# colmap/privacy_preserving_sfm

Measured on AMD Instinct MI355X. Metric: BA iterations/sec + RANSAC hypotheses/sec, 500 cams / 200k line obs, higher is better.
Workload: dtype f64; 1 GPU; configs[2]: 500 cams / 200k line obs full BA (K1+K2+K3, MFMA Schur solve) on 1xMI355X; cams=500, points=25000, obs=200000, camera_model=SIMPLE_RADIAL, reduced_system=3000, successful_steps=2561, lm_chunk=10, submodels=1, exchange=none (independent sub-models), linear_solver=cholesky (one launch: chain workgroup + task list), cholesky_fallbacks=0

## Files before the change

privacy_preserving_sfm_amd/csrc/ba_covariance.hip:

```cpp
#include <algorithm>
#include <cmath>
#include <cstring>
#include <vector>

#include "ba_impl.hpp"
#include "resource_pool.hpp"

namespace ppsfm {

typedef double cov_v4 __attribute__((ext_vector_type(4)));
constexpr int kTile = 64;

__device__ __forceinline__ cov_v4 CovMfma64(const double (&a)[16], const double (&b)[16], cov_v4 acc) {
  cov_v4 p1 = (cov_v4){0.0, 0.0, 0.0, 0.0}, p2 = p1, p3 = p1;
#pragma unroll
  for (int kk = 0; kk < 4; ++kk) {
    acc = __builtin_amdgcn_mfma_f64_16x16x4f64(a[kk], b[kk], acc, 0, 0, 0);
    p1 = __builtin_amdgcn_mfma_f64_16x16x4f64(a[4 + kk], b[4 + kk], p1, 0, 0, 0);
    p2 = __builtin_amdgcn_mfma_f64_16x16x4f64(a[8 + kk], b[8 + kk], p2, 0, 0, 0);
    p3 = __builtin_amdgcn_mfma_f64_16x16x4f64(a[12 + kk], b[12 + kk], p3, 0, 0, 0);
  }
  return (acc + p1) + (p2 + p3);
}
__device__ __forceinline__ void CovLoad16(const double* __restrict__ p, double (&v)[16]) {
  const double2* q = reinterpret_cast<const double2*>(p);
#pragma unroll
  for (int i = 0; i < 8; ++i) { const double2 t = q[i]; v[2 * i] = t.x; v[2 * i + 1] = t.y; }
}

__global__ __launch_bounds__(256) void k_tri_inverse(const double* __restrict__ L, int ld, int T, const double* __restrict__ Minv, const uint8_t* __restrict__ nz, double* Zt) {
  __shared__ double P[kTile * 17];
  const int j = (int)blockIdx.x >> 2, strip = (int)blockIdx.x & 3;
  const int tid = threadIdx.x, w = tid >> 6, l = tid & 63, lr = l & 15, g = l >> 4;
  double* zcol = Zt + ((size_t)j * kTile + 16 * strip) * ld;
  for (int idx = tid; idx < kTile * 16; idx += 256) {
    const int cc = idx >> 6, rr = idx & 63, gcol = 16 * strip + cc;
    zcol[(size_t)cc * ld + (size_t)j * kTile + rr] = rr >= gcol ? Minv[(size_t)j * kTile * kTile + rr * kTile + gcol] : 0.0;
  }
  __syncthreads();
  for (int k = j + 1; k < T; ++k) {
    cov_v4 acc = (cov_v4){0.0, 0.0, 0.0, 0.0};
    for (int m = j; m < k; ++m) {
      if (nz && !nz[(size_t)k * T + m]) continue;
      double av[16], bv[16];
      CovLoad16(L + ((size_t)k * kTile + 16 * w + lr) * ld + (size_t)m * kTile + 16 * g, av);
      CovLoad16(zcol + (size_t)lr * ld + (size_t)m * kTile + 16 * g, bv);
      acc = CovMfma64(av, bv, acc);
    }
#pragma unroll
    for (int i = 0; i < 4; ++i) P[(16 * w + g + 4 * i) * 17 + lr] = acc[i];
    __syncthreads();
    double av[16], bv[16];
    CovLoad16(Minv + (size_t)k * kTile * kTile + (size_t)(16 * w + lr) * kTile + 16 * g, av);
#pragma unroll
    for (int kk = 0; kk < 16; ++kk) {
      if (16 * g + kk > 16 * w + lr) av[kk] = 0.0;
      bv[kk] = P[(16 * g + kk) * 17 + lr];
    }
    const cov_v4 d = CovMfma64(av, bv, (cov_v4){0.0, 0.0, 0.0, 0.0});
#pragma unroll
    for (int i = 0; i < 4; ++i) zcol[(size_t)lr * ld + (size_t)k * kTile + 16 * w + g + 4 * i] = -d[i];
    __syncthreads();
  }
}

__global__ __launch_bounds__(256) void k_cov_pose_blocks(const int32_t* __restrict__ pairs, const int32_t* __restrict__ spos, const double* __restrict__ scale_c,
                                                         const double* __restrict__ Zt, int N, int n, double* __restrict__ out) {
  __shared__ double red[4][36];
  const int pr = blockIdx.x, tid = threadIdx.x;
  const int pi = pairs[2 * pr], pj = pairs[2 * pr + 1];
  const int ci = spos[6 * pi], cj = spos[6 * pj];
  const double* zi = Zt + (size_t)ci * N;
  const double* zj = Zt + (size_t)cj * N;
  double acc[36];
#pragma unroll
  for (int i = 0; i < 36; ++i) acc[i] = 0.0;
  for (int k = max(ci, cj) + tid; k < n; k += 256) {
    double a[6], b[6];
#pragma unroll
    for (int x = 0; x < 6; ++x) { a[x] = zi[(size_t)x * N + k]; b[x] = zj[(size_t)x * N + k]; }
#pragma unroll
    for (int x = 0; x < 6; ++x)
#pragma unroll
      for (int y = 0; y < 6; ++y) acc[6 * x + y] += a[x] * b[y];
  }
#pragma unroll
  for (int i = 0; i < 36; ++i) acc[i] = WaveSum(acc[i]);
  if ((tid & 63) == 0) {
#pragma unroll
    for (int i = 0; i < 36; ++i) red[tid >> 6][i] = acc[i];
  }
  __syncthreads();
  if (tid < 36) {
    const double v = ((red[0][tid] + red[1][tid]) + red[2][tid]) + red[3][tid];
    out[36 * (size_t)pr + tid] = scale_c[6 * pi + tid / 6] * scale_c[6 * pj + tid % 6] * v;
  }
}

struct CovPointArgs {
  int C, n, N;
  const int32_t *pt_start, *pt_obs, *obs_pose, *obs_cam, *spos, *intr_off, *intr_nv;
  const uint8_t* point_const;
  const double *rec, *JkS , *Vinv, *scale_p, *Zt;
};
constexpr int kCovChunk = 64;

__global__ __launch_bounds__(256) void k_cov_points(CovPointArgs a, const int32_t* __restrict__ ids, double* __restrict__ out) {
  __shared__ int s_kmin, s_col[kCovChunk], s_nv[kCovChunk], s_colI[kCovChunk][kCamStride];
  __shared__ double s_B[kCovChunk][18], s_BI[kCovChunk][3 * kCamStride], red[4][6];
  const int tid = threadIdx.x;
  const int p = ids[blockIdx.x];
  if (a.point_const[p]) {
    if (tid < 9) out[9 * (size_t)blockIdx.x + tid] = 0.0;
    return;
  }
  const int begin = a.pt_start[p], end = a.pt_start[p + 1];
  if (tid == 0) s_kmin = a.n;
  __syncthreads();
  for (int e = begin + tid; e < end; e += 256) {
    const int o = a.pt_obs[e];
    int kmin = a.spos[6 * a.obs_pose[o]];
    if (a.JkS) {
      const int cam = a.obs_cam[o] >> 4, off = a.intr_off[cam];
      if (off >= 0) for (int c = 0; c < a.intr_nv[cam]; ++c) kmin = min(kmin, a.spos[6 * a.C + off + c]);
    }
    atomicMin(&s_kmin, kmin);
  }
  __syncthreads();
  const int kmin = s_kmin;
  const int nchunks = (end - begin + kCovChunk - 1) / kCovChunk;
  double acc[6] = {0.0, 0.0, 0.0, 0.0, 0.0, 0.0};
  for (int k0 = kmin; k0 < a.n; k0 += 256) {
    const int k = k0 + tid;
    const bool live = k < a.n;
    double y0 = 0.0, y1 = 0.0, y2 = 0.0;
    for (int ch = 0; ch < nchunks; ++ch) {
      const int cnt = min(kCovChunk, end - begin - kCovChunk * ch);
      if (nchunks > 1 || k0 == kmin) {
        __syncthreads();
        if (tid < cnt) {
          const int o = a.pt_obs[begin + kCovChunk * ch + tid];
          const double* t = RecT(a.rec, (size_t)o);
          const double* jp = RecJ(a.rec, (size_t)o);
          s_col[tid] = a.spos[6 * a.obs_pose[o]];
#pragma unroll
          for (int x = 0; x < 6; ++x)
#pragma unroll
            for (int c = 0; c < 3; ++c) s_B[tid][3 * x + c] = jp[x] * t[c] + jp[6 + x] * t[3 + c];
          int nv = 0;
          if (a.JkS) {
            const int cam = a.obs_cam[o] >> 4, off = a.intr_off[cam];
            if (off >= 0) {
              nv = a.intr_nv[cam];
              const double* jk = a.JkS + (size_t)2 * kCamStride * o;
              for (int x = 0; x < nv; ++x) {
                s_colI[tid][x] = a.spos[6 * a.C + off + x];
#pragma unroll
                for (int c = 0; c < 3; ++c) s_BI[tid][3 * x + c] = jk[x] * t[c] + jk[kCamStride + x] * t[3 + c];
              }
            }
          }
          s_nv[tid] = nv;
        }
        __syncthreads();
      }
      if (live) {
        for (int q = 0; q < cnt; ++q) {
          const double* z = a.Zt + (size_t)s_col[q] * a.N + k;
#pragma unroll
          for (int x = 0; x < 6; ++x) {
            const double zz = z[(size_t)x * a.N];
            y0 += zz * s_B[q][3 * x]; y1 += zz * s_B[q][3 * x + 1]; y2 += zz * s_B[q][3 * x + 2];
          }
          const int nv = s_nv[q];
          for (int x = 0; x < nv; ++x) {
            const double zz = a.Zt[(size_t)s_colI[q][x] * a.N + k];
            y0 += zz * s_BI[q][3 * x]; y1 += zz * s_BI[q][3 * x + 1]; y2 += zz * s_BI[q][3 * x + 2];
          }
        }
      }
    }
    acc[0] += y0 * y0; acc[1] += y0 * y1; acc[2] += y0 * y2; acc[3] += y1 * y1; acc[4] += y1 * y2; acc[5] += y2 * y2;
  }
#pragma unroll
  for (int i = 0; i < 6; ++i) acc[i] = WaveSum(acc[i]);
  if ((tid & 63) == 0) {
#pragma unroll
    for (int i = 0; i < 6; ++i) red[tid >> 6][i] = acc[i];
  }
  __syncthreads();
  if (tid < 9) {
    const int r = tid / 3, c = tid % 3;
    const int lo = min(r, c), hi = max(r, c);
    const int sym = lo == 0 ? hi : (lo == 1 ? 2 + hi : 5);
    const double yy = ((red[0][sym] + red[1][sym]) + red[2][sym]) + red[3][sym];
    out[9 * (size_t)blockIdx.x + tid] = a.scale_p[3 * p + r] * a.scale_p[3 * p + c] * a.Vinv[6 * (size_t)p + sym] + yy;
  }
}

namespace {
struct CovBuffers {
  hipStream_t stream = nullptr;
  std::vector<void*> blocks;
  CholeskyState* chol = nullptr;
  template <typename T> int Alloc(T** p, size_t count) { const int rc = HandleAlloc(p, count); if (rc == PP_OK && *p) blocks.push_back(*p); return rc; }
  ~CovBuffers() {
    if (stream) (void)hipStreamSynchronize(stream);
    if (chol) CholeskyDestroy(chol);
    for (void* b : blocks) PoolDeviceFree(b);
  }
};
struct BufferSwap {
  pp_ba_impl* h;
  double *S, *scale_c, *scale_p, *diag_c, *diag_p, *Vinv, *vb;
  int32_t* d_flag;
  explicit BufferSwap(pp_ba_impl* hh) : h(hh), S(hh->S), scale_c(hh->scale_c), scale_p(hh->scale_p), diag_c(hh->diag_c), diag_p(hh->diag_p), Vinv(hh->Vinv), vb(hh->vb), d_flag(hh->d_flag) {}
  ~BufferSwap() { h->S = S; h->scale_c = scale_c; h->scale_p = scale_p; h->diag_c = diag_c; h->diag_p = diag_p; h->Vinv = Vinv; h->vb = vb; h->d_flag = d_flag; }
};
}

}

using namespace ppsfm;

extern "C" int pp_ba_covariance(pp_ba_handle h, const pp_ba_options* o, int32_t num_pose_pairs, const int32_t* pose_i, const int32_t* pose_j, double* pose_cov,
                                int32_t num_points, const int32_t* point_ids, double* point_cov, pp_ba_covariance_info* info) try {
  PP_REQUIRE(h && o, "pp_ba_covariance: null handle or options");
  PP_REQUIRE(num_pose_pairs >= 0 && num_points >= 0, "pp_ba_covariance: negative count");
  PP_REQUIRE(num_pose_pairs == 0 || (pose_i && pose_j && pose_cov), "pp_ba_covariance: %d pose pairs without their arrays", (int)num_pose_pairs);
  PP_REQUIRE(num_points == 0 || (point_ids && point_cov), "pp_ba_covariance: %d points without their arrays", (int)num_points);
  for (int32_t q = 0; q < num_pose_pairs; ++q)
    PP_REQUIRE(pose_i[q] >= 0 && pose_i[q] < h->C && pose_j[q] >= 0 && pose_j[q] < h->C, "pp_ba_covariance: pose pair %d = (%d, %d) is out of range (%d images)", (int)q,
               (int)pose_i[q], (int)pose_j[q], (int)h->C);
  for (int32_t q = 0; q < num_points; ++q)
    PP_REQUIRE(point_ids[q] >= 0 && point_ids[q] < h->P, "pp_ba_covariance: point %d = %d is out of range (%d points)", (int)q, (int)point_ids[q], (int)h->P);
  PP_REQUIRE(!h->iterative, "pp_ba_covariance: an iterative (ITERATIVE_SCHUR) handle never forms the reduced camera system the covariance is taken from - create "
             "the handle with pp_ba_problem_desc::linear_solver = PP_LINEAR_SOLVER_DIRECT (or PPSFM_BA_LINEAR_SOLVER=direct)");
  PP_REQUIRE(!BaInGroup(h), "pp_ba_covariance: the handle is attached to a group (pp_ba_set_allreduce / pp_ba_set_communicator) and holds one shard of the points - "
             "detach it, or take the covariance from a handle that holds the whole problem");
  if (info) std::memset(info, 0, sizeof(*info));
  PP_HIP_TRY(hipSetDevice(h->device));
  int rc;
  if ((rc = BaEnsureJacobianBuffers(h, 0, h->NI > 0 ? 1 : 0))) return rc;
  if ((rc = BaEnsureSolverBuffers(h))) return rc;
  hipStream_t s = h->stream;
  const int N = h->N, n = h->n_red, T = N / kTile;
  const size_t NN = (size_t)N * N;

  CovBuffers buf;
  buf.stream = s;
  double *S2 = nullptr, *Linv2 = nullptr, *Lfac2 = nullptr, *x2 = nullptr, *scale_c2 = nullptr, *scale_p2 = nullptr, *diag_c2 = nullptr, *diag_p2 = nullptr, *Vinv2 = nullptr,
         *vb2 = nullptr, *Zt = nullptr, *d_pose = nullptr, *d_point = nullptr;
  int32_t *flag2 = nullptr, *d_pairs = nullptr, *d_ids = nullptr;
  Switches sw = h->sw;
  sw.chol_small = false;
  {
    std::lock_guard<std::recursive_mutex> setup_lock(DeviceSetupMutex());
    if ((rc = buf.Alloc(&S2, NN)) || (rc = buf.Alloc(&Linv2, CholeskyWorkspaceDoubles(N))) || (rc = buf.Alloc(&x2, (size_t)N)) || (rc = buf.Alloc(&flag2, 4)) ||
        (rc = buf.Alloc(&scale_c2, (size_t)n)) || (rc = buf.Alloc(&scale_p2, 3 * (size_t)h->P)) || (rc = buf.Alloc(&diag_c2, (size_t)n)) ||
        (rc = buf.Alloc(&diag_p2, 3 * (size_t)h->P)) || (rc = buf.Alloc(&Vinv2, 6 * (size_t)h->P)) || (rc = buf.Alloc(&vb2, 3 * (size_t)h->P)) || (rc = buf.Alloc(&Zt, NN)) ||
        (rc = buf.Alloc(&d_pose, 36 * (size_t)num_pose_pairs)) || (rc = buf.Alloc(&d_point, 9 * (size_t)num_points)) || (rc = buf.Alloc(&d_pairs, 2 * (size_t)num_pose_pairs)) ||
        (rc = buf.Alloc(&d_ids, (size_t)num_points)))
      return rc;
    buf.chol = CholeskyCreate(sw);
    CholeskyDisableGraph(buf.chol);
    if (CholeskyNeedsFactorArray(buf.chol, N) && !CholeskyColumnsOnly(h->chol) && (rc = buf.Alloc(&Lfac2, NN))) return rc;
    PP_HIP_TRY(hipMemsetAsync(S2, 0, sizeof(double) * NN, s));
    if (Lfac2) PP_HIP_TRY(hipMemsetAsync(Lfac2, 0, sizeof(double) * NN, s));
    PP_HIP_TRY(hipMemsetAsync(Zt, 0, sizeof(double) * NN, s));
    PP_HIP_TRY(hipMemsetAsync(flag2, 0, 4 * sizeof(int32_t), s));
    const CholeskySystem sys{S2, N, n, Linv2, Lfac2, x2, flag2, s};
    const bool sparse = h->sparse_tiles && !h->tile_nz.empty();
    if ((rc = CholeskyBind(buf.chol, sys, sparse ? h->tile_nz.data() : nullptr))) return rc;
    if (CholeskyColumnsOnly(h->chol)) (void)CholeskyFallBackToColumns(buf.chol);
  }
  if (num_pose_pairs > 0) {
    std::vector<int32_t> pairs(2 * (size_t)num_pose_pairs);
    const bool perm = !h->pose_new_of_old.empty();
    for (int32_t q = 0; q < num_pose_pairs; ++q) {
      pairs[2 * (size_t)q] = perm ? h->pose_new_of_old[pose_i[q]] : pose_i[q];
      pairs[2 * (size_t)q + 1] = perm ? h->pose_new_of_old[pose_j[q]] : pose_j[q];
    }
    PP_HIP_TRY(hipMemcpyAsync(d_pairs, pairs.data(), sizeof(int32_t) * pairs.size(), hipMemcpyHostToDevice, s));
    PP_HIP_TRY(hipStreamSynchronize(s));
  }
  if (num_points > 0) PP_HIP_TRY(hipMemcpyAsync(d_ids, point_ids, sizeof(int32_t) * (size_t)num_points, hipMemcpyHostToDevice, s));
  PP_HIP_TRY(hipEventRecord(h->ev0, s));

  int32_t flag = 0;
  {
    BufferSwap swap(h);
    h->S = S2; h->scale_c = scale_c2; h->scale_p = scale_p2; h->diag_c = diag_c2; h->diag_p = diag_p2; h->Vinv = Vinv2; h->vb = vb2; h->d_flag = flag2;
    for (int attempt = 0; attempt < 2; ++attempt) {
      if ((rc = BaAssembleUndamped(h, o, attempt == 0))) return rc;
      if ((rc = CholeskySolve(buf.chol))) return rc;
      PP_HIP_TRY(hipMemcpyAsync(&flag, flag2, sizeof(int32_t), hipMemcpyDeviceToHost, s));
      PP_HIP_TRY(hipStreamSynchronize(s));
      if (!(flag & 4) || (flag & 3) || attempt == 1 || !CholeskyFallBackToColumns(buf.chol)) break;
      PP_HIP_TRY(hipMemsetAsync(flag2, 0, sizeof(int32_t), s));
      PP_HIP_TRY(hipMemsetAsync(S2, 0, sizeof(double) * NN, s));
    }
  }
  if (flag & 7) {
    SetLastError("pp_ba_covariance: the undamped reduced camera system is not positive definite (%s) - a free gauge, or a point seen along one direction only, has no covariance",
                 (flag & 2) ? "a point block is singular" : (flag & 1) ? "non-positive pivot" : "the factorisation did not finish");
    return PP_ERR_NUMERIC;
  }
  const double* Minv = nullptr;
  const uint8_t* nz = nullptr;
  const double* L = CholeskyFactor(buf.chol, &Minv, &nz);
  if (!L) { SetLastError("pp_ba_covariance: the factorisation left no factor in memory"); return PP_ERR_INTERNAL; }
  hipLaunchKernelGGL(k_tri_inverse, dim3(4 * T), dim3(256), 0, s, L, N, T, Minv, nz, Zt);
  if (num_pose_pairs > 0)
    hipLaunchKernelGGL(k_cov_pose_blocks, dim3(num_pose_pairs), dim3(256), 0, s, (const int32_t*)d_pairs, (const int32_t*)h->spos, (const double*)scale_c2, (const double*)Zt, N, n, d_pose);
  if (num_points > 0) {
    CovPointArgs a;
    a.C = h->C; a.n = n; a.N = N;
    a.pt_start = h->pt_start; a.pt_obs = h->pt_obs; a.obs_pose = h->obs_pose; a.obs_cam = h->obs_cam; a.spos = h->spos; a.intr_off = h->intr_off; a.intr_nv = h->intr_nv;
    a.point_const = h->point_const; a.rec = h->JpS; a.JkS = h->NI > 0 ? h->JkS_intr : nullptr; a.Vinv = Vinv2; a.scale_p = scale_p2; a.Zt = Zt;
    hipLaunchKernelGGL(k_cov_points, dim3(num_points), dim3(256), 0, s, a, (const int32_t*)d_ids, d_point);
  }
  PP_HIP_TRY(hipGetLastError());
  PP_HIP_TRY(hipEventRecord(h->ev1, s));
  if (num_pose_pairs > 0) PP_HIP_TRY(hipMemcpyAsync(pose_cov, d_pose, sizeof(double) * 36 * (size_t)num_pose_pairs, hipMemcpyDeviceToHost, s));
  if (num_points > 0) PP_HIP_TRY(hipMemcpyAsync(point_cov, d_point, sizeof(double) * 9 * (size_t)num_points, hipMemcpyDeviceToHost, s));
  PP_HIP_TRY(hipStreamSynchronize(s));
  if (info) {
    float ms = 0;
    PP_HIP_TRY(hipEventElapsedTime(&ms, h->ev0, h->ev1));
    info->n = n; info->path = CholeskyLinsolve(buf.chol); info->device_ms = ms;
  }
  return PP_OK;
} PP_API_CATCH("pp_ba_covariance")
```

privacy_preserving_sfm_amd/csrc/ba_eval.hip:

```cpp
#include <algorithm>
#include <chrono>
#include <cstdlib>
#include <cmath>
#include <cstring>
#include <numeric>
#include <thread>

#include "ba_impl.hpp"
#include "resource_pool.hpp"
#include "line_residual.hpp"

namespace ppsfm {

struct EvalArgs {
  int64_t M;
  const double *la, *lb, *lc;
  const int32_t *obs_pose, *obs_point, *obs_cam;
  const double *poses, *points, *intr;
  double *r, *Jpose, *Jpoint, *Jcam;
  const int32_t* cam_col;
  int cam_stride;
  double* partials;
  int loss_type;
  double loss_scale;
};

__device__ __forceinline__ void BlockPartialSum(double v, double* partials) {
  __shared__ double wsum[4];
  v = WaveSum(v);
  const int wave = threadIdx.x >> 6;
  if ((threadIdx.x & 63) == 0) wsum[wave] = v;
  __syncthreads();
  if (threadIdx.x == 0) partials[blockIdx.x] = (wsum[0] + wsum[1]) + (wsum[2] + wsum[3]);
}

template <int MODE, bool WANT_CAM, bool LOSS_CORRECT>
__global__ __launch_bounds__(256) void k_line_eval(EvalArgs a) {
  constexpr int JW = MODE == 2 ? 14 : 12;
  __shared__ __attribute__((aligned(16))) double sJp[MODE == 0 ? 2 : 256 * JW];
  __shared__ __attribute__((aligned(16))) double sJx[MODE == 0 ? 2 : 256 * 6];
  const int tid = threadIdx.x;
  const int64_t o0 = (int64_t)blockIdx.x * 256;
  const int64_t o = o0 + tid;
  double half_rho = 0.0;
  if (o < a.M) {
    const int c = a.obs_pose[o], p = a.obs_point[o], ck = a.obs_cam[o];
    const double la = a.la[o], lb = a.lb[o], lc = a.lc[o];
    const int model = ck & 15;
    const double* cam = a.intr + (size_t)kCamStride * (ck >> 4);
    const double* pose = a.poses + (size_t)7 * c;
    const double q[4] = {pose[0], pose[1], pose[2], pose[3]};
    const double t[3] = {pose[4], pose[5], pose[6]};
    const double X[3] = {a.points[3 * (size_t)p], a.points[3 * (size_t)p + 1], a.points[3 * (size_t)p + 2]};
    if (MODE == 0) {
      double r[2];
      LineResidualOnly(model, cam, q, t, X, la, lb, lc, r);
      double rho0, rho1;
      LossRho(a.loss_type, a.loss_scale, r[0] * r[0] + r[1] * r[1], &rho0, &rho1);
      half_rho = 0.5 * rho0;
      if (a.r) { a.r[2 * o] = r[0]; a.r[2 * o + 1] = r[1]; }
    } else {
      LineObsJac J;
      LineResidualJacobian<MODE == 2>(model, cam, q, t, X, la, lb, lc, &J);
      double rho0, rho1;
      LossRho(a.loss_type, a.loss_scale, J.r[0] * J.r[0] + J.r[1] * J.r[1], &rho0, &rho1);
      half_rho = 0.5 * rho0;
      const double sr = LOSS_CORRECT ? sqrt(rho1) : 1.0;
      double2* r2 = reinterpret_cast<double2*>(a.r);
      r2[o] = make_double2(sr * J.r[0], sr * J.r[1]);
      double2* jp = reinterpret_cast<double2*>(sJp + JW * tid);
      if (MODE == 1) {
        jp[0] = make_double2(sr * J.Jrot[0], sr * J.Jrot[1]);
        jp[1] = make_double2(sr * J.Jrot[2], sr * J.Jt[0]);
        jp[2] = make_double2(sr * J.Jt[1], sr * J.Jt[2]);
        jp[3] = make_double2(sr * J.Jrot[3], sr * J.Jrot[4]);
        jp[4] = make_double2(sr * J.Jrot[5], sr * J.Jt[3]);
        jp[5] = make_double2(sr * J.Jt[4], sr * J.Jt[5]);
      } else {
        jp[0] = make_double2(sr * J.Jq[0], sr * J.Jq[1]);
        jp[1] = make_double2(sr * J.Jq[2], sr * J.Jq[3]);
        jp[2] = make_double2(sr * J.Jt[0], sr * J.Jt[1]);
        jp[3] = make_double2(sr * J.Jt[2], sr * J.Jq[4]);
        jp[4] = make_double2(sr * J.Jq[5], sr * J.Jq[6]);
        jp[5] = make_double2(sr * J.Jq[7], sr * J.Jt[3]);
        jp[6] = make_double2(sr * J.Jt[4], sr * J.Jt[5]);
      }
      double2* jx = reinterpret_cast<double2*>(sJx + 6 * tid);
      jx[0] = make_double2(sr * J.JX[0], sr * J.JX[1]);
      jx[1] = make_double2(sr * J.JX[2], sr * J.JX[3]);
      jx[2] = make_double2(sr * J.JX[4], sr * J.JX[5]);
      if (WANT_CAM) {
        double jl[2 * kCamStride];
#pragma unroll
        for (int i = 0; i < 2 * kCamStride; ++i) jl[i] = 0.0;
        LineResidualCameraJacobian(model, cam, q, t, X, la, lb, lc, jl, kCamStride);
        if (LOSS_CORRECT) {
#pragma unroll
          for (int i = 0; i < 2 * kCamStride; ++i) jl[i] *= sr;
        }
        if (a.cam_col) {
          const int W = a.cam_stride;
          double* jc = a.Jcam + (size_t)2 * W * o;
          double2* z = reinterpret_cast<double2*>(jc);
          for (int i = 0; i < W; ++i) z[i] = make_double2(0.0, 0.0);
          const int32_t* col = a.cam_col + (size_t)kCamStride * (ck >> 4);
#pragma unroll
          for (int i = 0; i < kCamStride; ++i) { const int cc = col[i]; if (cc >= 0) { jc[cc] = jl[i]; jc[W + cc] = jl[kCamStride + i]; } }
        } else {
          double2* jc = reinterpret_cast<double2*>(a.Jcam + (size_t)2 * kCamStride * o);
#pragma unroll
          for (int i = 0; i < kCamStride; ++i) jc[i] = make_double2(jl[2 * i], jl[2 * i + 1]);
        }
      }
    }
  }
  if (MODE != 0) {
    __syncthreads();
    const int64_t left = a.M - o0;
    const int nobs = left < 256 ? (int)left : 256;
    {
      const int n2 = nobs * JW / 2;
      double2* dst = reinterpret_cast<double2*>(a.Jpose + (size_t)JW * o0);
      const double2* src = reinterpret_cast<const double2*>(sJp);
#pragma unroll
      for (int it = 0; it < (256 * JW / 2 + 255) / 256; ++it) {
        const int idx = it * 256 + tid;
        if (idx < n2) { const double2 v = src[idx]; __builtin_nontemporal_store(v.x, &dst[idx].x); __builtin_nontemporal_store(v.y, &dst[idx].y); }
      }
    }
    {
      const int n2 = nobs * 3;
      double2* dst = reinterpret_cast<double2*>(a.Jpoint + (size_t)6 * o0);
      const double2* src = reinterpret_cast<const double2*>(sJx);
#pragma unroll
      for (int it = 0; it < 3; ++it) {
        const int idx = it * 256 + tid;
        if (idx < n2) { const double2 v = src[idx]; __builtin_nontemporal_store(v.x, &dst[idx].x); __builtin_nontemporal_store(v.y, &dst[idx].y); }
      }
    }
  }
  BlockPartialSum(half_rho, a.partials);
}

__global__ __launch_bounds__(256) void k_sum_partials(const double* partials, int n, double* out) {
  __shared__ double sh[256];
  double acc = 0.0;
  for (int i = threadIdx.x; i < n; i += 256) acc += partials[i];
  sh[threadIdx.x] = acc;
  __syncthreads();
  for (int s = 128; s > 0; s >>= 1) {
    if ((int)threadIdx.x < s) sh[threadIdx.x] += sh[threadIdx.x + s];
    __syncthreads();
  }
  if (threadIdx.x == 0) *out = sh[0];
}

static EvalArgs MakeArgs(pp_ba_impl* h, const double* poses, const double* points, const double* intr = nullptr) {
  EvalArgs a;
  a.M = h->M; a.la = h->la; a.lb = h->lb; a.lc = h->lc;
  a.obs_pose = h->obs_pose; a.obs_point = h->obs_point; a.obs_cam = h->obs_cam;
  a.poses = poses; a.points = points; a.intr = intr ? intr : h->intr;
  a.r = h->r; a.Jpose = h->Jpose; a.Jpoint = h->Jpoint; a.Jcam = h->Jcam; a.cam_col = nullptr; a.cam_stride = kCamStride;
  a.partials = h->partials; a.loss_type = h->loss_type; a.loss_scale = h->loss_scale;
  return a;
}

int BaEnsureJacobianBuffers(pp_ba_impl* h, int jac_mode, int want_cam) {
  const int width = jac_mode == 1 ? 14 : 12;
  if (!h->Jpose || h->jpose_width < width) {
    if (h->Jpose) PoolDeviceFree(h->Jpose);
    h->Jpose = nullptr;
    int rc = HandleAlloc(&h->Jpose, (size_t)h->M * width);
    if (rc) return rc;
    h->jpose_width = width;
  }
  if (want_cam && !h->Jcam) {
    int rc = HandleAlloc(&h->Jcam, (size_t)h->M * 2 * kCamStride);
    if (rc) return rc;
  }
  return PP_OK;
}

int LaunchEval(pp_ba_impl* h, int jac_mode, int want_cam, bool loss_correct, const double* poses, const double* points,
               double* cost_slot, bool compact_cam) {
  EvalArgs a = MakeArgs(h, poses, points);
  if (want_cam) {
    h->jcam_compact = compact_cam && h->NI > 0;
    if (h->jcam_compact) { a.cam_col = h->intr_col; a.cam_stride = h->jcam_stride; }
  }
  const int grid = h->num_partials;
  hipStream_t s = h->stream;
  if (jac_mode == 0) {
    if (want_cam) { if (loss_correct) hipLaunchKernelGGL((k_line_eval<1, true, true>), dim3(grid), dim3(256), 0, s, a); else hipLaunchKernelGGL((k_line_eval<1, true, false>), dim3(grid), dim3(256), 0, s, a); }
    else { if (loss_correct) hipLaunchKernelGGL((k_line_eval<1, false, true>), dim3(grid), dim3(256), 0, s, a); else hipLaunchKernelGGL((k_line_eval<1, false, false>), dim3(grid), dim3(256), 0, s, a); }
  } else {
    if (want_cam) hipLaunchKernelGGL((k_line_eval<2, true, false>), dim3(grid), dim3(256), 0, s, a);
    else hipLaunchKernelGGL((k_line_eval<2, false, false>), dim3(grid), dim3(256), 0, s, a);
  }
  if (cost_slot) hipLaunchKernelGGL(k_sum_partials, dim3(1), dim3(256), 0, s, h->partials, grid, cost_slot);
  PP_HIP_TRY(hipGetLastError());
  return PP_OK;
}

int LaunchCostOnly(pp_ba_impl* h, const double* poses, const double* points, const double* intr, double* cost_slot) {
  EvalArgs a = MakeArgs(h, poses, points, intr);
  a.r = nullptr;
  const int grid = h->num_partials;
  hipLaunchKernelGGL((k_line_eval<0, false, false>), dim3(grid), dim3(256), 0, h->stream, a);
  if (cost_slot) hipLaunchKernelGGL(k_sum_partials, dim3(1), dim3(256), 0, h->stream, h->partials, grid, cost_slot);
  PP_HIP_TRY(hipGetLastError());
  return PP_OK;
}

static int LaunchResidualsOnly(pp_ba_impl* h, const double* poses, const double* points, double* cost_slot) {
  EvalArgs a = MakeArgs(h, poses, points);
  const int grid = h->num_partials;
  hipLaunchKernelGGL((k_line_eval<0, false, false>), dim3(grid), dim3(256), 0, h->stream, a);
  if (cost_slot) hipLaunchKernelGGL(k_sum_partials, dim3(1), dim3(256), 0, h->stream, h->partials, grid, cost_slot);
  PP_HIP_TRY(hipGetLastError());
  return PP_OK;
}

}

using namespace ppsfm;

extern "C" {

int pp_ba_destroy(pp_ba_handle h) try {
  if (!h) return PP_OK;
  (void)hipSetDevice(h->device);
  void* bufs[] = {h->la, h->lb, h->lc, h->obs_cam, h->obs_pose, h->obs_point, h->pose_camera, h->camera_model, h->pose_const,
                  h->tvec_mask, h->point_const, h->pt_start, h->pt_obs, h->pose_start, h->pose_obs, h->pair_start,
                  h->pair_ij, h->pair_entries, h->poses, h->points, h->intr, h->poses_c, h->points_c, h->r, h->Jpose,
                  h->Jpoint, h->Jcam, h->partials, h->U, h->gc, h->V, h->gp, h->Vinv, h->vb, h->scale_c, h->scale_p,
                  h->diag_c, h->diag_p, h->S, h->Linv, h->Lfac, h->step_c, h->step_p, h->scal, h->JpS, h->Q, h->norm_part,
                  h->intr_c, h->cam_np, h->intr_off, h->intr_nv, h->intr_col, h->cam_start, h->cam_obs, h->gen_pair, h->gen_pair_chunk, h->gen_chunk,
                  h->gen_multi, h->gen_grp_start, h->gen_grp_obs, h->gen_L, h->kk_entries, h->kk_pair, h->kk_pair_chunk, h->kk_chunk, h->kk_multi, h->kk_partial, h->gen_entries, h->isum_chunk, h->isum_cam_chunk, h->gen_partial, h->isum_partial, h->cnI, h->JkS_intr, h->Spack, h->nz_tile_list,
                  h->small_chunk, h->small_pair_chunk, h->small_partials, h->spos, h->step_s, h->attach_slot};
  if (h->stream) (void)hipStreamSynchronize(h->stream);
  for (void* b : bufs) if (b) PoolDeviceFree(b);
  CholeskyDestroy(h->chol);
  PcgFreeBuffers(h);
  for (int i = 0; i < 8; ++i) if (h->tev[i]) PoolEventRelease(h->tev[i], true);
  for (int i = 0; i < 2; ++i) if (h->tev_eval[i]) PoolEventRelease(h->tev_eval[i], true);
  if (h->h_scal) PoolPinnedFree(h->h_scal);
  { void* pins[] = {h->pin_r, h->pin_jpose, h->pin_jpoint, h->pin_jcam}; for (void* b : pins) if (b) (void)hipHostFree(b); }
  if (h->ev_readback) PoolEventRelease(h->ev_readback, false);
  if (h->ev0) PoolEventRelease(h->ev0, true);
  if (h->ev1) PoolEventRelease(h->ev1, true);
  if (h->stream) PoolStreamRelease(h->stream);
  delete h;
  return PP_OK;
} PP_API_CATCH("pp_ba_destroy")

int pp_ba_create(const pp_ba_problem_desc* d, int device, pp_ba_handle* out) try {
  PP_REQUIRE(d && out, "pp_ba_create: null argument");
  *out = nullptr;
  PP_REQUIRE(d->num_poses > 0 && d->num_points > 0 && d->num_cameras > 0 && d->num_obs > 0,
             "pp_ba_create: empty problem (poses %d, points %d, cameras %d, obs %lld)", d->num_poses, d->num_points,
             d->num_cameras, (long long)d->num_obs);
  PP_REQUIRE(d->lines && d->obs_pose && d->obs_point && d->pose_camera && d->camera_model, "pp_ba_create: null array");
  PP_REQUIRE(d->loss_type >= 0 && d->loss_type <= 2 && d->loss_scale >= 0, "pp_ba_create: bad loss");
  PP_REQUIRE(d->num_obs < (int64_t)1 << 31, "pp_ba_create: more than 2^31 observations");
  PP_REQUIRE(d->ordering >= PP_ORDERING_DEFAULT && d->ordering <= PP_ORDERING_AUTO, "pp_ba_create: unknown ordering %d", d->ordering);
  const int C = d->num_poses, P = d->num_points, K = d->num_cameras;
  const int64_t M = d->num_obs;
  PP_REQUIRE(K < (1 << 26), "pp_ba_create: too many intrinsics blocks");
  for (int k = 0; k < K; ++k) PP_REQUIRE(CameraNumParams(d->camera_model[k]) > 0, "pp_ba_create: unknown camera model %d", d->camera_model[k]);
  for (int c = 0; c < C; ++c) PP_REQUIRE(d->pose_camera[c] >= 0 && d->pose_camera[c] < K, "pp_ba_create: pose_camera[%d] out of range", c);
  for (int64_t o = 0; o < M; ++o) {
    PP_REQUIRE(d->obs_pose[o] >= 0 && d->obs_pose[o] < C && d->obs_point[o] >= 0 && d->obs_point[o] < P,
               "pp_ba_create: observation %lld indexes out of range", (long long)o);
    const double nrm = std::sqrt(d->lines[3 * o] * d->lines[3 * o] + d->lines[3 * o + 1] * d->lines[3 * o + 1]);
    PP_REQUIRE(std::fabs(nrm - 1.0) <= 1e-6, "pp_ba_create: line %lld is not normalised (|(a,b)| = %.9g)", (long long)o, nrm);
  }
  std::vector<int32_t> intr_off(K, -1), intr_nv(K, 0), intr_col((size_t)K * kCamStride, -1);
  int nv_widest = 0;
  int NI = 0;
  if (d->camera_const_mask) {
    std::vector<char> cam_used(K, 0);
    for (int c = 0; c < C; ++c) cam_used[d->pose_camera[c]] = 1;
    for (int k = 0; k < K; ++k) {
      if (!cam_used[k]) continue;
      const int np = CameraNumParams(d->camera_model[k]);
      int nv = 0;
      for (int j = 0; j < np; ++j) if (!((d->camera_const_mask[k] >> j) & 1)) intr_col[(size_t)k * kCamStride + j] = nv++;
      if (nv > 0) { intr_off[k] = NI; intr_nv[k] = nv; NI += nv; } nv_widest = std::max(nv_widest, nv);
    }
  }
  int ndev = 0;
  PP_HIP_TRY(hipGetDeviceCount(&ndev));
  PP_REQUIRE(device >= 0 && device < ndev, "pp_ba_create: device %d of %d", device, ndev);
  PP_HIP_TRY(hipSetDevice(device));

  const auto t_create0 = std::chrono::steady_clock::now();
  const ppsfm::Switches sw = ppsfm::ReadSwitches();
  const bool create_dbg = sw.create_debug;
  auto lap = [&, last = t_create0](const char* what) mutable {
    if (!create_dbg) return;
    const auto now = std::chrono::steady_clock::now();
    fprintf(stderr, "ppsfm: create %-34s %.3f ms\n", what, std::chrono::duration<double, std::milli>(now - last).count());
    last = now;
  };
  pp_ba_impl* h = new pp_ba_impl();
  OnUnwind unwind{[&] { pp_ba_destroy(h); }};
  h->sw = sw;
  h->chol = CholeskyCreate(sw);
  h->structure_from_covisibility = d->covisibility != nullptr;
  h->device = device; h->C = C; h->P = P; h->K = K; h->M = M;
  h->loss_type = d->loss_type; h->loss_scale = d->loss_scale;
  h->NI = NI; h->n_red = 6 * C + NI; h->intrinsics_variable = NI > 0;
  h->jcam_stride = std::max(2, (nv_widest + 1) & ~1);
  h->iterative = ppsfm::WillIterate(d, sw.ba_linear_solver);
  const bool iterative = h->iterative;
  int rc = PP_OK;
#define TRY(x) do { rc = (x); if (rc) { pp_ba_destroy(h); return rc; } } while (0)
#define TRYH(x) do { hipError_t e_ = (x); if (e_ != hipSuccess) { SetLastError("%s: %s", #x, hipGetErrorString(e_)); pp_ba_destroy(h); return PP_ERR_HIP; } } while (0)
  TRY(PoolStreamAcquire(&h->stream));
  TRY(PoolEventAcquire(&h->ev0, true));
  TRY(PoolEventAcquire(&h->ev1, true));
  hipStream_t s = h->stream;
  lap("handle, stream, events");

  std::vector<uint8_t> point_const(P, 0);
  if (d->point_const) std::memcpy(point_const.data(), d->point_const, P);
  std::vector<int32_t> pt_start(P + 1, 0), pt_obs(M);
  for (int64_t o = 0; o < M; ++o) pt_start[d->obs_point[o] + 1]++;
  for (int p = 0; p < P; ++p) pt_start[p + 1] += pt_start[p];
  {
    std::vector<int32_t> fp(pt_start.begin(), pt_start.end() - 1);
    for (int64_t o = 0; o < M; ++o) pt_obs[fp[d->obs_point[o]]++] = (int32_t)o;
  }
  lap("CSR by point");
  bool lists_on_device = !iterative && PairListsOnDeviceEligible(C, M, sw.ba_pair_lists);
  std::vector<uint64_t> graph_bits;
  double graph_ms = 0;
  if (lists_on_device) {
// ... 309 lines not shown
          size_t b = a;
          while (b < ko.size() && ko[b].first == ko[a].first) ++b;
          grps.push_back({ko[a].first, p, (int32_t)flat.size(), (int32_t)(flat.size() + (b - a))});
          for (size_t t = a; t < b; ++t) flat.push_back(ko[t].second);
          a = b;
        }
      }
      std::stable_sort(grps.begin(), grps.end(), [](const Grp& a, const Grp& b) { return a.k < b.k; });
      const size_t G = grps.size();
      dl.entries.assign(G + 1 + flat.size(), 0);
      { size_t pos = 0; for (size_t g = 0; g < G; ++g) { dl.entries[g] = (int32_t)pos; for (int32_t e = grps[g].e0; e < grps[g].e1; ++e) dl.entries[G + 1 + pos++] = flat[e]; } dl.entries[G] = (int32_t)pos; }
      dl.num_groups = (int64_t)G;
      dl.pair_chunk.push_back(0);
      size_t g = 0;
      for (int k = 0; k < K; ++k) {
        if (intr_off[k] < 0) continue;
        const int pair_id = (int)(dl.pair.size() / 4);
        dl.pair.push_back(6 * C + intr_off[k]); dl.pair.push_back(intr_nv[k]); dl.pair.push_back(6 * C + intr_off[k]); dl.pair.push_back(intr_nv[k] | (1 << 8));
        while (g < G && grps[g].k < k) ++g;
        size_t g0 = g; int64_t nobs = 0;
        for (; g < G && grps[g].k == k; ++g) {
          nobs += grps[g].e1 - grps[g].e0;
          if (nobs >= 320) { dl.chunk.push_back(pair_id); dl.chunk.push_back((int32_t)g0); dl.chunk.push_back((int32_t)(g + 1)); g0 = g + 1; nobs = 0; }
        }
        if (g0 < g) { dl.chunk.push_back(pair_id); dl.chunk.push_back((int32_t)g0); dl.chunk.push_back((int32_t)g); }
        dl.pair_chunk.push_back((int32_t)(dl.chunk.size() / 3));
      }
    };
    auto finish_diag = [&](DiagLists& dl) {
      const int64_t np = (int64_t)(dl.pair.size() / 4);
      for (int64_t pr = 0; pr < np; ++pr) if (dl.pair_chunk[pr + 1] - dl.pair_chunk[pr] != 1) dl.multi.push_back((int32_t)pr);
    };
    if (iterative) {
      DiagLists dl;
      build_diag(dl);
      gen_entries = dl.entries; gen_pair = dl.pair; gen_pair_chunk = dl.pair_chunk; gen_chunk = dl.chunk; h->gen_num_groups = dl.num_groups;
    } else if (h->intr_wide_nv > 0) {
      gen_pair_chunk.push_back(0);
    } else {
    struct GEntry { int64_t key; int32_t oi, oj; };
    std::vector<GEntry> ge;
    std::vector<int32_t> grp_start(1, 0), grp_obs;
    std::vector<int32_t> grp_cam;
    {
      std::vector<std::pair<int32_t, int32_t>> ko;
      for (int p = 0; p < P; ++p) {
        ko.clear();
        for (int e = pt_start[p]; e < pt_start[p + 1]; ++e) {
          const int32_t o = pt_obs[e]; const int k = in_pose_camera[in_obs_pose[o]];
          if (intr_off[k] >= 0) ko.push_back({k, o});
        }
        std::stable_sort(ko.begin(), ko.end(), [](const auto& a, const auto& b) { return a.first < b.first; });
        const size_t first_group = grp_cam.size();
        for (size_t a = 0; a < ko.size();) {
          size_t b = a;
          while (b < ko.size() && ko[b].first == ko[a].first) ++b;
          grp_cam.push_back(ko[a].first);
          for (size_t t = a; t < b; ++t) grp_obs.push_back(ko[t].second);
          grp_start.push_back((int32_t)grp_obs.size());
          a = b;
        }
        for (size_t g = first_group; g < grp_cam.size(); ++g) {
          const int ka = grp_cam[g];
          for (int f = pt_start[p]; f < pt_start[p + 1]; ++f) {
            const int32_t oj = pt_obs[f]; const int cj = in_obs_pose[oj]; const int kb = in_pose_camera[cj];
            const bool same = kb == ka;
            if (point_const[p] && !same) continue;
            const int32_t code = oj | (same ? (int32_t)0x80000000 : 0);
            if (!pose_const[cj]) ge.push_back({((int64_t)ka * 2 + 0) * (int64_t)(C + K) + cj, (int32_t)g, code});
            if (intr_off[kb] >= 0 && kb < ka) ge.push_back({((int64_t)ka * 2 + 1) * (int64_t)(C + K) + kb, (int32_t)g, code});
          }
        }
      }
    }
    h->gen_num_groups = (int64_t)grp_cam.size();
    gen_grp_start = grp_start; gen_grp_obs = grp_obs;
    build_diag(kk); finish_diag(kk);
    std::sort(ge.begin(), ge.end(), [](const GEntry& a, const GEntry& b) {
      if (a.key != b.key) return a.key < b.key;
      if (a.oi != b.oi) return a.oi < b.oi;
      return (a.oj & 0x7fffffff) < (b.oj & 0x7fffffff);
    });
    {
      std::vector<char> has_obs(K, 0);
      for (int64_t o = 0; o < M; ++o) has_obs[in_pose_camera[in_obs_pose[o]]] = 1;
      (void)has_obs;
      std::sort(ge.begin(), ge.end(), [](const GEntry& a, const GEntry& b) {
        if (a.key != b.key) return a.key < b.key;
        if (a.oi != b.oi) return a.oi < b.oi;
        return a.oj < b.oj;
      });
    }
    gen_entries.resize(2 * ge.size());
    gen_pair_chunk.push_back(0);
    size_t e = 0;
    while (e < ge.size()) {
      size_t f = e;
      while (f < ge.size() && ge[f].key == ge[e].key) ++f;
      const int64_t key = ge[e].key;
      const int col = (int)(key % (C + K)), kind = (int)((key / (C + K)) & 1), ka = (int)(key / (C + K) / 2);
      const int pair_id = (int)(gen_pair.size() / 4);
      gen_pair.push_back(6 * C + intr_off[ka]); gen_pair.push_back(intr_nv[ka]);
      if (kind == 0) { gen_pair.push_back(6 * col); gen_pair.push_back(6); }
      else { gen_pair.push_back(6 * C + intr_off[col]); gen_pair.push_back(intr_nv[col] | (1 << 8)); }
      if (ge[e].oi >= 0)
        for (size_t c0 = e; c0 < f; c0 += kGenChunk) { gen_chunk.push_back(pair_id); gen_chunk.push_back((int32_t)c0); gen_chunk.push_back((int32_t)std::min(c0 + kGenChunk, f)); }
      gen_pair_chunk.push_back((int32_t)(gen_chunk.size() / 3));
      for (size_t g = e; g < f; ++g) { gen_entries[2 * g] = ge[g].oi; gen_entries[2 * g + 1] = ge[g].oj; }
      e = f;
    }
    }
    h->gen_num_pairs = (int64_t)(gen_pair.size() / 4); h->gen_num_chunks = (int64_t)(gen_chunk.size() / 3);
    for (int64_t pr = 0; pr < h->gen_num_pairs; ++pr) if (gen_pair_chunk[pr + 1] - gen_pair_chunk[pr] != 1) gen_multi.push_back((int32_t)pr);
    h->gen_num_multi = (int64_t)gen_multi.size();
    h->isum_num_chunks = (int64_t)(isum_chunk.size() / 3);
  }

  lap("chunks, intrinsics lists");
  const auto t_create3 = std::chrono::steady_clock::now();
  TRY(HandleAlloc(&h->la, M)); TRY(HandleAlloc(&h->lb, M)); TRY(HandleAlloc(&h->lc, M));
  if (!arrays_on_device) { TRY(HandleAlloc(&h->obs_pose, M)); TRY(HandleAlloc(&h->obs_point, M)); }
  TRY(HandleAlloc(&h->obs_cam, M));
  TRY(HandleAlloc(&h->pose_camera, C)); TRY(HandleAlloc(&h->camera_model, K));
  if (!arrays_on_device) { TRY(HandleAlloc(&h->pose_const, C)); TRY(HandleAlloc(&h->point_const, P)); TRY(HandleAlloc(&h->pt_start, P + 1)); TRY(HandleAlloc(&h->pt_obs, M)); }
  TRY(HandleAlloc(&h->tvec_mask, C));
  TRY(HandleAlloc(&h->pose_start, C + 1)); TRY(HandleAlloc(&h->pose_obs, M));
  TRY(HandleAlloc(&h->pair_start, pair_start.size())); TRY(HandleAlloc(&h->pair_ij, std::max<size_t>(pair_ij.size(), 2)));
  if (!h->pair_entries) TRY(HandleAlloc(&h->pair_entries, std::max<size_t>(pair_entries.size(), 2)));
  TRY(HandleAlloc(&h->poses, (size_t)7 * C)); TRY(HandleAlloc(&h->points, (size_t)3 * P)); TRY(HandleAlloc(&h->intr, (size_t)kCamStride * K));
  TRY(HandleAlloc(&h->poses_c, (size_t)7 * C)); TRY(HandleAlloc(&h->points_c, (size_t)3 * P)); TRY(HandleAlloc(&h->intr_c, (size_t)kCamStride * K));
  TRY(HandleAlloc(&h->cam_np, K));
  TRY(HandleAlloc(&h->intr_off, K)); TRY(HandleAlloc(&h->intr_nv, K)); TRY(HandleAlloc(&h->intr_col, (size_t)K * kCamStride));
  if (NI > 0) {
    TRY(HandleAlloc(&h->cam_start, K + 1)); TRY(HandleAlloc(&h->cam_obs, M));
    TRY(HandleAlloc(&h->gen_pair, std::max<size_t>(gen_pair.size(), 4))); TRY(HandleAlloc(&h->gen_pair_chunk, gen_pair_chunk.size()));
    TRY(HandleAlloc(&h->gen_chunk, gen_chunk.size())); TRY(HandleAlloc(&h->gen_entries, std::max<size_t>(gen_entries.size(), 2)));
    TRY(HandleAlloc(&h->gen_multi, std::max<size_t>(gen_multi.size(), 1)));
    if (!iterative) {
      h->kk_num_groups = kk.num_groups; h->kk_num_pairs = (int64_t)(kk.pair.size() / 4); h->kk_num_chunks = (int64_t)(kk.chunk.size() / 3); h->kk_num_multi = (int64_t)kk.multi.size();
      TRY(HandleAlloc(&h->kk_entries, std::max<size_t>(kk.entries.size(), 1))); TRY(HandleAlloc(&h->kk_pair, std::max<size_t>(kk.pair.size(), 1)));
      TRY(HandleAlloc(&h->kk_pair_chunk, std::max<size_t>(kk.pair_chunk.size(), 1))); TRY(HandleAlloc(&h->kk_chunk, std::max<size_t>(kk.chunk.size(), 1)));
      TRY(HandleAlloc(&h->kk_multi, std::max<size_t>(kk.multi.size(), 1))); TRY(HandleAlloc(&h->kk_partial, 144 * std::max<size_t>((size_t)h->kk_num_chunks, 1)));
      TRY(Upload(h->kk_entries, kk.entries.data(), kk.entries.size(), s)); TRY(Upload(h->kk_pair, kk.pair.data(), kk.pair.size(), s));
      TRY(Upload(h->kk_pair_chunk, kk.pair_chunk.data(), kk.pair_chunk.size(), s)); TRY(Upload(h->kk_chunk, kk.chunk.data(), kk.chunk.size(), s));
      TRY(Upload(h->kk_multi, kk.multi.data(), kk.multi.size(), s));
      TRY(HandleAlloc(&h->gen_grp_start, std::max<size_t>(gen_grp_start.size(), 1))); TRY(HandleAlloc(&h->gen_grp_obs, std::max<size_t>(gen_grp_obs.size(), 1)));
      TRY(HandleAlloc(&h->gen_L, 36 * std::max<size_t>((size_t)h->gen_num_groups, 1)));
    }
    TRY(HandleAlloc(&h->isum_chunk, isum_chunk.size())); TRY(HandleAlloc(&h->isum_cam_chunk, isum_cam_chunk.size()));
    TRY(HandleAlloc(&h->gen_partial, (size_t)std::max<int64_t>(h->gen_num_chunks, 1) * 144)); TRY(HandleAlloc(&h->isum_partial, (size_t)std::max<int64_t>(h->isum_num_chunks, 1) * 24));
    TRY(HandleAlloc(&h->cnI, (size_t)NI)); TRY(HandleAlloc(&h->JkS_intr, (size_t)M * 2 * kCamStride));
    TRYH(hipMemsetAsync(h->JkS_intr, 0, sizeof(double) * (size_t)M * 2 * kCamStride, s));
  }
  TRY(HandleAlloc(&h->r, (size_t)2 * M)); TRY(HandleAlloc(&h->Jpoint, (size_t)6 * M));
  h->num_partials = CeilDiv(M, 256);
  h->partials_stride = std::max(std::max(h->num_partials, 4096), CeilDiv(4 * (int64_t)P, 256));
  TRY(HandleAlloc(&h->partials, 2 * (size_t)h->partials_stride));
  TRY(HandleAlloc(&h->scal, kNumScalars + 1));
  h->d_flag = reinterpret_cast<int32_t*>(h->scal + kNumScalars - 1);
  TRY(PoolPinnedAlloc(reinterpret_cast<void**>(&h->h_scal), sizeof(double) * 3 * kNumScalars));
  std::memset(h->h_scal, 0, sizeof(double) * 3 * kNumScalars);
  if (hipHostGetDevicePointer(reinterpret_cast<void**>(&h->h_scal_dev), h->h_scal, 0) != hipSuccess) { h->h_scal_dev = nullptr; (void)hipGetLastError(); }
  TRYH(hipMemsetAsync(h->scal, 0, sizeof(double) * (kNumScalars + 1), s));

  TRY(Upload(h->la, la.data(), M, s)); TRY(Upload(h->lb, lb.data(), M, s)); TRY(Upload(h->lc, lc.data(), M, s));
  if (!arrays_on_device) { TRY(Upload(h->obs_pose, in_obs_pose, M, s)); TRY(Upload(h->obs_point, d->obs_point, M, s)); }
  TRY(Upload(h->obs_cam, obs_cam.data(), M, s));
  TRY(Upload(h->pose_camera, in_pose_camera, C, s)); TRY(Upload(h->camera_model, d->camera_model, K, s));
  if (!arrays_on_device) { TRY(Upload(h->pose_const, pose_const.data(), C, s)); TRY(Upload(h->point_const, point_const.data(), P, s)); }
  TRY(Upload(h->tvec_mask, tvec_mask.data(), C, s));
  {
    int neff = 0;
    for (int c = 0; c < C; ++c) if (!pose_const[c]) neff += 6 - __builtin_popcount(tvec_mask[c] & 7);
    for (int p = 0; p < P; ++p) if (!point_const[p]) neff += 3;
    h->num_effective_pose_point = neff;
  }
  if (!arrays_on_device) { TRY(Upload(h->pt_start, pt_start.data(), P + 1, s)); TRY(Upload(h->pt_obs, pt_obs.data(), M, s)); }
  TRY(Upload(h->pose_start, pose_start.data(), C + 1, s)); TRY(Upload(h->pose_obs, pose_obs.data(), M, s));
  TRY(Upload(h->pair_start, pair_start.data(), pair_start.size(), s));
  TRY(Upload(h->pair_ij, pair_ij.data(), pair_ij.size(), s));
  if (!lists_on_device) TRY(Upload(h->pair_entries, pair_entries.data(), pair_entries.size(), s));
  { std::vector<int32_t> np(K); for (int k = 0; k < K; ++k) np[k] = CameraNumParams(d->camera_model[k]); TRY(Upload(h->cam_np, np.data(), K, s)); TRYH(hipStreamSynchronize(s)); }
  TRY(HandleAlloc(&h->spos, std::max<size_t>(h->spos_host.size(), 1))); TRY(Upload(h->spos, h->spos_host.data(), h->spos_host.size(), s));
  TRY(Upload(h->intr_off, intr_off.data(), K, s)); TRY(Upload(h->intr_nv, intr_nv.data(), K, s)); TRY(Upload(h->intr_col, intr_col.data(), intr_col.size(), s));
  if (NI > 0) {
    TRY(Upload(h->cam_start, cam_start.data(), K + 1, s)); TRY(Upload(h->cam_obs, cam_obs.data(), M, s));
    TRY(Upload(h->gen_pair, gen_pair.data(), gen_pair.size(), s)); TRY(Upload(h->gen_pair_chunk, gen_pair_chunk.data(), gen_pair_chunk.size(), s));
    TRY(Upload(h->gen_chunk, gen_chunk.data(), gen_chunk.size(), s)); TRY(Upload(h->gen_entries, gen_entries.data(), gen_entries.size(), s));
    TRY(Upload(h->gen_multi, gen_multi.data(), gen_multi.size(), s));
    if (!iterative) { TRY(Upload(h->gen_grp_start, gen_grp_start.data(), gen_grp_start.size(), s)); TRY(Upload(h->gen_grp_obs, gen_grp_obs.data(), gen_grp_obs.size(), s)); }
    TRY(Upload(h->isum_chunk, isum_chunk.data(), isum_chunk.size(), s)); TRY(Upload(h->isum_cam_chunk, isum_cam_chunk.data(), isum_cam_chunk.size(), s));
  }
  if (want_chunks) {
    TRY(HandleAlloc(&h->small_chunk, std::max<size_t>(small_chunk.size(), 3))); TRY(HandleAlloc(&h->small_pair_chunk, small_pair_chunk.size()));
    TRY(HandleAlloc(&h->small_partials, 36 * std::max<size_t>((size_t)h->small_num_chunks, 1)));
    TRY(Upload(h->small_chunk, small_chunk.data(), small_chunk.size(), s)); TRY(Upload(h->small_pair_chunk, small_pair_chunk.data(), small_pair_chunk.size(), s));
  }
  TRYH(hipStreamSynchronize(s));
#undef TRY
#undef TRYH
  {
    const auto t_create4 = std::chrono::steady_clock::now();
    auto ms = [](std::chrono::steady_clock::time_point a, std::chrono::steady_clock::time_point b) { return std::chrono::duration<double, std::milli>(b - a).count(); };
    h->create_ms[0] = ordering_ms; h->create_ms[1] = ms(t_create0, t_create2) - ordering_ms; h->create_ms[2] = ms(t_create2, t_create3);
    h->create_ms[3] = ms(t_create3, t_create4); h->create_ms[4] = 0; h->create_ms[5] = ms(t_create0, t_create4);
  }
  *out = h;
  return PP_OK;
} PP_API_CATCH("pp_ba_create")

int pp_ba_get_create_profile(pp_ba_handle h, double* ms) try {
  PP_REQUIRE(h && ms, "pp_ba_get_create_profile: null argument");
  for (int i = 0; i < 6; ++i) ms[i] = h->create_ms[i];
  ms[4] = CholeskyPlanMs(h->chol);
  return PP_OK;
} PP_API_CATCH("pp_ba_get_create_profile")

int pp_ba_covisibility(const pp_ba_problem_desc* d, uint8_t* out) try {
  PP_REQUIRE(d && out && d->obs_pose && d->obs_point, "pp_ba_covisibility: null argument");
  const int C = d->num_poses, P = d->num_points;
  const int64_t M = d->num_obs;
  PP_REQUIRE(C > 0 && P > 0 && M >= 0, "pp_ba_covisibility: empty problem");
  if (d->camera_const_mask) {
    PP_REQUIRE(d->pose_camera && d->camera_model && d->num_cameras > 0, "pp_ba_covisibility: camera_const_mask without pose_camera / camera_model");
    for (int k = 0; k < d->num_cameras; ++k) PP_REQUIRE(CameraNumParams(d->camera_model[k]) > 0, "pp_ba_covisibility: unknown camera model %d", d->camera_model[k]);
    for (int c = 0; c < C; ++c) PP_REQUIRE(d->pose_camera[c] >= 0 && d->pose_camera[c] < d->num_cameras, "pp_ba_covisibility: pose_camera[%d] out of range", c);
  }
  for (int64_t o = 0; o < M; ++o)
    PP_REQUIRE(d->obs_pose[o] >= 0 && d->obs_pose[o] < C && d->obs_point[o] >= 0 && d->obs_point[o] < P, "pp_ba_covisibility: observation %lld indexes out of range", (long long)o);
  std::memset(out, 0, (size_t)C * C);
  std::vector<int32_t> ps(P + 1, 0), po(M);
  for (int64_t o = 0; o < M; ++o) ps[d->obs_point[o] + 1]++;
  for (int p = 0; p < P; ++p) ps[p + 1] += ps[p];
  { std::vector<int32_t> f(ps.begin(), ps.end() - 1); for (int64_t o = 0; o < M; ++o) po[f[d->obs_point[o]]++] = d->obs_pose[o]; }
  const uint8_t* fixed = (d->camera_const_mask && ppsfm::PrivateIntrinsicsColumns(d, ppsfm::ReadSwitches().ba_intr_layout) > 0) ? nullptr : d->pose_const;
  for (int p = 0; p < P; ++p) {
    if (d->point_const && d->point_const[p]) continue;
    for (int a = ps[p]; a < ps[p + 1]; ++a) {
      const int ca = po[a];
      if (fixed && fixed[ca]) continue;
      for (int b = ps[p]; b < a; ++b) {
        const int cb = po[b];
        if (cb == ca || (fixed && fixed[cb])) continue;
        out[(size_t)ca * C + cb] = 1; out[(size_t)cb * C + ca] = 1;
      }
    }
  }
  return PP_OK;
} PP_API_CATCH("pp_ba_covisibility")

int pp_ba_set_parameters(pp_ba_handle h, const double* poses, const double* points, const double* intr) try {
  PP_REQUIRE(h, "pp_ba_set_parameters: null handle");
  PP_HIP_TRY(hipSetDevice(h->device));
  std::vector<double> staged;
  if (poses && !h->pose_new_of_old.empty()) {
    staged.resize((size_t)7 * h->C);
    for (int c = 0; c < h->C; ++c) std::memcpy(&staged[(size_t)7 * h->pose_new_of_old[c]], poses + (size_t)7 * c, 7 * sizeof(double));
    poses = staged.data();
  }
  if (poses && (int)h->host_pose_const.size() == h->C)
    for (int c = 0; c < h->C; ++c) {
      const double* q = poses + (size_t)7 * c;
      const double n2 = q[0] * q[0] + q[1] * q[1] + q[2] * q[2] + q[3] * q[3];
      PP_REQUIRE(h->host_pose_const[c] || !(std::fabs(n2 - 1.0) > 1e-6),
                 "pp_ba_set_parameters: the quaternion of a variable pose is not of unit length (|q|^2 = %.9g at internal image %d); normalise it as "
                 "BundleAdjuster::AddImageToProblem does (Image::NormalizeQvec)", n2, c);
    }
  if (poses) { int rc = Upload(h->poses, poses, (size_t)7 * h->C, h->stream); if (rc) return rc; }
  if (points) { int rc = Upload(h->points, points, (size_t)3 * h->P, h->stream); if (rc) return rc; }
  if (intr) { int rc = Upload(h->intr, intr, (size_t)kCamStride * h->K, h->stream); if (rc) return rc; }
  PP_HIP_TRY(hipStreamSynchronize(h->stream));
  return PP_OK;
} PP_API_CATCH("pp_ba_set_parameters")

int pp_ba_get_parameters(pp_ba_handle h, double* poses, double* points, double* intr) try {
  PP_REQUIRE(h, "pp_ba_get_parameters: null handle");
  PP_HIP_TRY(hipSetDevice(h->device));
  std::vector<double> staged;
  const bool perm = poses && !h->pose_new_of_old.empty();
  if (perm) staged.resize((size_t)7 * h->C);
  if (poses) { int rc = Download(perm ? staged.data() : poses, h->poses, (size_t)7 * h->C, h->stream); if (rc) return rc; }
  if (points) { int rc = Download(points, h->points, (size_t)3 * h->P, h->stream); if (rc) return rc; }
  if (intr) { int rc = Download(intr, h->intr, (size_t)kCamStride * h->K, h->stream); if (rc) return rc; }
  PP_HIP_TRY(hipStreamSynchronize(h->stream));
  if (perm) for (int c = 0; c < h->C; ++c) std::memcpy(poses + (size_t)7 * c, &staged[(size_t)7 * h->pose_new_of_old[c]], 7 * sizeof(double));
  return PP_OK;
} PP_API_CATCH("pp_ba_get_parameters")

int pp_ba_eval(pp_ba_handle h, int jac_mode, int want_cam, double* residuals_out, double* jpose_out, double* jpoint_out,
               double* jcam_out, double* cost_out) try {
  PP_REQUIRE(h, "pp_ba_eval: null handle");
  PP_REQUIRE(jac_mode == 0 || jac_mode == 1, "pp_ba_eval: jac_mode must be 0 (tangent) or 1 (ambient)");
  PP_HIP_TRY(hipSetDevice(h->device));
  int rc = BaEnsureJacobianBuffers(h, jac_mode, want_cam || jcam_out != nullptr);
  if (rc) return rc;
  const int cam = (want_cam || jcam_out) ? 1 : 0;
  rc = LaunchEval(h, jac_mode, cam, false, h->poses, h->points, h->scal + kCost);
  if (rc) return rc;
  const int width = jac_mode == 1 ? 14 : 12;
  if (residuals_out) { rc = Download(residuals_out, h->r, (size_t)2 * h->M, h->stream); if (rc) return rc; }
  if (jpose_out) { rc = Download(jpose_out, h->Jpose, (size_t)width * h->M, h->stream); if (rc) return rc; }
  if (jpoint_out) { rc = Download(jpoint_out, h->Jpoint, (size_t)6 * h->M, h->stream); if (rc) return rc; }
  if (jcam_out) { rc = Download(jcam_out, h->Jcam, (size_t)2 * kCamStride * h->M, h->stream); if (rc) return rc; }
  if (cost_out) { rc = Download(cost_out, h->scal + kCost, 1, h->stream); if (rc) return rc; }
  PP_HIP_TRY(hipStreamSynchronize(h->stream));
  return PP_OK;
} PP_API_CATCH("pp_ba_eval")

int pp_ba_eval_host_view(pp_ba_handle h, int jac_mode, int want_cam, int want_jacobians, const double** residuals, const double** jpose,
                         const double** jpoint, const double** jcam, double* cost_out) try {
  PP_REQUIRE(h && residuals, "pp_ba_eval_host_view: null argument");
  PP_REQUIRE(jac_mode == 0 || jac_mode == 1, "pp_ba_eval_host_view: jac_mode must be 0 (tangent) or 1 (ambient)");
  PP_HIP_TRY(hipSetDevice(h->device));
  const int cam = want_cam ? 1 : 0, width = jac_mode == 1 ? 14 : 12;
  int rc = BaEnsureJacobianBuffers(h, jac_mode, cam);
  if (rc) return rc;
  const size_t M = (size_t)h->M;
  if (!h->pin_r) PP_HIP_TRY(hipHostMalloc(reinterpret_cast<void**>(&h->pin_r), sizeof(double) * 2 * M));
  if (want_jacobians) {
    if (h->pin_jpose && h->pin_width < width) { (void)hipHostFree(h->pin_jpose); h->pin_jpose = nullptr; }
    if (!h->pin_jpose) { PP_HIP_TRY(hipHostMalloc(reinterpret_cast<void**>(&h->pin_jpose), sizeof(double) * width * M)); h->pin_width = width; }
    if (!h->pin_jpoint) PP_HIP_TRY(hipHostMalloc(reinterpret_cast<void**>(&h->pin_jpoint), sizeof(double) * 6 * M));
    if (cam && !h->pin_jcam) PP_HIP_TRY(hipHostMalloc(reinterpret_cast<void**>(&h->pin_jcam), sizeof(double) * 2 * kCamStride * M));
  }
  if (want_jacobians) rc = LaunchEval(h, jac_mode, cam, false, h->poses, h->points, h->scal + kCost);
  else rc = LaunchResidualsOnly(h, h->poses, h->points, h->scal + kCost);
  if (rc) return rc;
  rc = Download(h->pin_r, h->r, 2 * M, h->stream); if (rc) return rc;
  if (want_jacobians) {
    rc = Download(h->pin_jpose, h->Jpose, (size_t)width * M, h->stream); if (rc) return rc;
    rc = Download(h->pin_jpoint, h->Jpoint, 6 * M, h->stream); if (rc) return rc;
    if (cam) { rc = Download(h->pin_jcam, h->Jcam, (size_t)2 * kCamStride * M, h->stream); if (rc) return rc; }
  }
  if (cost_out) { rc = Download(cost_out, h->scal + kCost, 1, h->stream); if (rc) return rc; }
  PP_HIP_TRY(hipStreamSynchronize(h->stream));
  *residuals = h->pin_r;
  if (jpose) *jpose = want_jacobians ? h->pin_jpose : nullptr;
  if (jpoint) *jpoint = want_jacobians ? h->pin_jpoint : nullptr;
  if (jcam) *jcam = (want_jacobians && cam) ? h->pin_jcam : nullptr;
  return PP_OK;
} PP_API_CATCH("pp_ba_eval_host_view")

int pp_ba_eval_device(pp_ba_handle h, int jac_mode, int want_cam, int repeat, float* ms_per_launch) try {
  PP_REQUIRE(h && repeat > 0, "pp_ba_eval_device: bad argument");
  PP_REQUIRE(jac_mode == 0 || jac_mode == 1, "pp_ba_eval_device: jac_mode must be 0 or 1");
  PP_HIP_TRY(hipSetDevice(h->device));
  int rc = BaEnsureJacobianBuffers(h, jac_mode, want_cam);
  if (rc) return rc;
  PP_HIP_TRY(hipEventRecord(h->ev0, h->stream));
  for (int i = 0; i < repeat; ++i) {
    rc = LaunchEval(h, jac_mode, want_cam, false, h->poses, h->points, nullptr);
    if (rc) return rc;
  }
  PP_HIP_TRY(hipEventRecord(h->ev1, h->stream));
  PP_HIP_TRY(hipEventSynchronize(h->ev1));
  float ms = 0;
  PP_HIP_TRY(hipEventElapsedTime(&ms, h->ev0, h->ev1));
  if (ms_per_launch) *ms_per_launch = ms / repeat;
  return PP_OK;
} PP_API_CATCH("pp_ba_eval_device")

}
```

privacy_preserving_sfm_amd/csrc/ba_impl.hpp:

```cpp
#pragma once
#include <mutex>
#include <functional>
#include <vector>

#include "common.hpp"
#include "switches.hpp"

namespace ppsfm {

constexpr int kRecStride = 24;
#ifdef __HIPCC__
__device__ __forceinline__ const double* RecT(const double* rec, size_t o) { return rec + kRecStride * o; }
__device__ __forceinline__ const double* RecJ(const double* rec, size_t o) { return rec + kRecStride * o + 6; }
__device__ __forceinline__ const double* RecX(const double* rec, size_t o) { return rec + kRecStride * o + 18; }
#endif
int SymbolicTileFill(int T, uint8_t* nz);
int CholeskyChainSteps(int T, const uint8_t* nz, const Switches& sw, int* chains = nullptr);
int CholeskyPlanSteps(int T, const uint8_t* nz, const Switches& sw, int* chains = nullptr);
struct ImageOrdering { std::vector<int32_t> old_of_new, new_of_old; int nnz_natural = -1, nnz_ordered = -1, chains = 0, chain_steps = 0; bool dense_exit = false; double plan_ms = 0; };
ImageOrdering ChooseImageOrdering(const pp_ba_problem_desc* d, int NI, const Switches& sw, const uint64_t* graph_bits = nullptr);
bool OrderingReadsObservations(const pp_ba_problem_desc* d, int NI, const Switches& sw);
bool WillIterate(const pp_ba_problem_desc* d, LinearSolverSwitch sw);
int CountVariableIntrinsics(const pp_ba_problem_desc* d);
bool PairListsOnDeviceEligible(int C, int64_t M, PairListsSwitch sw);
int BuildPairListsOnDevice(int C, int64_t M, const int32_t* d_pt_start, const int32_t* d_pt_obs, const int32_t* d_obs_pose, const int32_t* d_obs_point,
                           const uint8_t* d_pose_const, const uint8_t* d_point_const, hipStream_t s, int32_t** entries_out, int64_t* num_entries,
                           std::vector<int32_t>* pair_start, std::vector<int32_t>* pair_ij, bool* fallback);
void BuildPairListsOnHost(int C, int P, int64_t M, const int32_t* pt_start, const int32_t* pt_obs, const int32_t* obs_pose, const uint8_t* list_const,
                          const uint8_t* point_const, int threads, const std::function<void(const char*)>& lap, int64_t* total_entries,
                          std::vector<int32_t>* pair_start, std::vector<int32_t>* pair_ij, std::vector<int32_t>* pair_entries);
int CoVisibilityOnDevice(int C, int64_t M, const int32_t* d_pt_start, const int32_t* d_pt_obs, const int32_t* d_obs_pose, const int32_t* d_obs_point,
                         const uint8_t* d_pose_const, const uint8_t* d_point_const, hipStream_t s, std::vector<uint64_t>* bits);
int PrivateIntrinsicsColumns(const pp_ba_problem_desc* d, IntrLayout layout);
}

namespace ppsfm {
struct PcgState { double rho, Q0, norm_b, alpha; int32_t iter, done, status, pad_; };
struct CholeskyState;
}

struct pp_ba_impl {
  ppsfm::Switches sw;
  int device = 0;
  hipStream_t stream = nullptr;
  hipEvent_t ev0 = nullptr, ev1 = nullptr;

  int32_t C = 0, P = 0, K = 0;
  int64_t M = 0;
  int32_t loss_type = 0;
  double loss_scale = 1.0;
  bool intrinsics_variable = false;

  double *la = nullptr, *lb = nullptr, *lc = nullptr;
  int32_t *obs_pose = nullptr, *obs_point = nullptr, *obs_cam = nullptr, *pose_camera = nullptr, *camera_model = nullptr;
  uint8_t *pose_const = nullptr, *tvec_mask = nullptr, *point_const = nullptr;
  std::vector<uint8_t> host_pose_const;
  int32_t *pt_start = nullptr, *pt_obs = nullptr, *pose_start = nullptr, *pose_obs = nullptr;
  int64_t num_pairs = 0, num_entries = 0;
  bool pairs_complete = false;
  std::vector<uint8_t> tile_nz;
  int num_nz_tiles = 0;
  bool sparse_tiles = false;
  int32_t* nz_tile_list = nullptr;
  std::vector<int32_t> pose_old_of_new, pose_new_of_old;
  int nnz_tiles_natural = -1, nnz_tiles_ordered = -1;
  int32_t* spos = nullptr;
  std::vector<int32_t> spos_host;
  bool spos_identity = true;
  int jcam_stride = 2;
  bool jcam_compact = false;
  int intr_wide_nv = 0;
  double* step_s = nullptr;
  double* attach_slot = nullptr;
  bool structure_from_covisibility = false;
  int structure_chains = -1, structure_steps = -1;
  double create_ms[6] = {0, 0, 0, 0, 0, 0};
  int32_t *pair_start = nullptr, *pair_ij = nullptr, *pair_entries = nullptr;

  int32_t NI = 0;
  int32_t n_red = 0;
  int32_t *intr_off = nullptr, *intr_nv = nullptr;
  int32_t* intr_col = nullptr;
  int32_t *cam_start = nullptr, *cam_obs = nullptr;
  int32_t* cam_np = nullptr;
  int64_t gen_num_pairs = 0, gen_num_chunks = 0, isum_num_chunks = 0;
  int32_t *gen_pair = nullptr, *gen_pair_chunk = nullptr, *gen_chunk = nullptr, *gen_entries = nullptr;
  int32_t *gen_grp_start = nullptr, *gen_grp_obs = nullptr; double* gen_L = nullptr;
  int32_t *kk_entries = nullptr, *kk_pair = nullptr, *kk_pair_chunk = nullptr, *kk_chunk = nullptr, *kk_multi = nullptr; double* kk_partial = nullptr;
  int64_t kk_num_groups = 0, kk_num_pairs = 0, kk_num_chunks = 0, kk_num_multi = 0;
  int32_t* gen_multi = nullptr; int64_t gen_num_multi = 0;
  int64_t gen_num_groups = 0;
  int32_t *isum_chunk = nullptr, *isum_cam_chunk = nullptr;
  double *gen_partial = nullptr, *isum_partial = nullptr, *cnI = nullptr, *JkS_intr = nullptr;

  double *poses = nullptr, *points = nullptr, *intr = nullptr;
  double *poses_c = nullptr, *points_c = nullptr, *intr_c = nullptr;

  double *r = nullptr, *Jpose = nullptr, *Jpoint = nullptr, *Jcam = nullptr;
  int jpose_width = 0;
  double* partials = nullptr;
  int num_partials = 0, partials_stride = 0, trial_partials = 0;
  double *pin_r = nullptr, *pin_jpose = nullptr, *pin_jpoint = nullptr, *pin_jcam = nullptr;
  int pin_width = 0;

  double *U = nullptr, *gc = nullptr, *V = nullptr, *gp = nullptr, *Vinv = nullptr, *vb = nullptr;
  double *scale_c = nullptr, *scale_p = nullptr, *diag_c = nullptr, *diag_p = nullptr;
  double *S = nullptr, *Linv = nullptr, *Lfac = nullptr, *step_c = nullptr, *step_p = nullptr;
  double *JpS = nullptr, *Q = nullptr, *norm_part = nullptr;
  int32_t N = 0;
  double* scal = nullptr;
  double* h_scal = nullptr;
  int num_effective_pose_point = 0;
  unsigned long long ticket_seq = 0;
  double* h_scal_dev = nullptr;
  hipEvent_t ev_readback = nullptr;
  int32_t* d_flag = nullptr;

  std::vector<double> trace;
  double timings_ms[PP_BA_T_COUNT] = {0};
  int32_t timing_calls[PP_BA_T_COUNT] = {0};

  bool iterative = false;
  double *pcg_Sd = nullptr, *pcg_binv = nullptr, *pcg_b = nullptr, *pcg_r = nullptr, *pcg_z = nullptr, *pcg_p = nullptr, *pcg_q = nullptr, *pcg_a = nullptr,
         *pcg_dot = nullptr, *pcg_part = nullptr;
  ppsfm::PcgState *pcg_state = nullptr, *pcg_state_host = nullptr;
  double *pcg_tk = nullptr, *pcg_w = nullptr, *pcg_Scomp = nullptr, *pcg_binvI = nullptr;
  void *pcg_pt_entry = nullptr, *pcg_pose_entry = nullptr;
  int linear_solver_iterations = 0;
  int32_t pcg_ticket = 0;
  int pcg_last_iterations = 0;

  bool pairs_chunked = false;
  int32_t *small_chunk = nullptr, *small_pair_chunk = nullptr;
  int small_num_chunks = 0;
  double* small_partials = nullptr;

  pp_allreduce_fn allreduce = nullptr;
  void* allreduce_ctx = nullptr;
  int32_t group_rank = 0, group_size = 1;
  struct pp_comm_impl* comm = nullptr;
  int64_t Spack_cap = 0;
  double* Spack = nullptr;
  hipEvent_t tev[8] = {nullptr};
  hipEvent_t tev_eval[2] = {nullptr, nullptr};
  ppsfm::CholeskyState* chol = nullptr;
};

namespace ppsfm {
enum Scalar { kCost = 0, kCostCand = 1, kModelChange = 2, kGradMax = 3, kStepNorm2 = 4, kXNorm2 = 5, kTicketSlot = 6 , kNumScalars = 8 };

int BaEnsureJacobianBuffers(pp_ba_impl* h, int jac_mode, int want_cam);
int LaunchEval(pp_ba_impl* h, int jac_mode, int want_cam, bool loss_correct, const double* poses, const double* points,
               double* cost_slot, bool compact_cam = false);
int LaunchCostOnly(pp_ba_impl* h, const double* poses, const double* points, const double* intr, double* cost_slot);
constexpr int kGenChunk = 32;
constexpr int kIsumChunk = 2048;
int IntrSumsAfterEval(pp_ba_impl* h);
int IntrScale(pp_ba_impl* h, int jacobi);
int IntrDiagonal(pp_ba_impl* h, double dmin, double dmax);
int IntrScaledJacobians(pp_ba_impl* h);
int IntrAssemble(pp_ba_impl* h, double inv_radius, int add_diagonal);
inline size_t CholeskyWorkspaceDoubles(int N) { return (size_t)(4 * (N / 64) + 3) * 64 * 64 + 8192 + (size_t)(N / 128 + 1) * 5 * 64 * 64; }
std::recursive_mutex& DeviceSetupMutex();
struct CholeskySystem { double* S; int N, rhs_row; double *Linv_ws, *Lfac, *x; int32_t* flag; hipStream_t stream; };
CholeskyState* CholeskyCreate(const Switches& sw);
void CholeskyDestroy(CholeskyState* st);
bool CholeskyNeedsFactorArray(const CholeskyState* st, int N);
int CholeskyBind(CholeskyState* st, const CholeskySystem& sys, const uint8_t* tile_nz, bool* map_changed = nullptr);
int CholeskySolve(CholeskyState* st);
bool CholeskyFallBackToColumns(CholeskyState* st);
void CholeskyDisableGraph(CholeskyState* st);
int CholeskyLinsolve(const CholeskyState* st);
int CholeskyFallbacks(const CholeskyState* st);
double CholeskyPlanMs(const CholeskyState* st);
bool CholeskyColumnsOnly(const CholeskyState* st);
const double* CholeskyFactor(const CholeskyState* st, const double** diag_inverses, const uint8_t** tile_map);
int BaEnsureSolverBuffers(pp_ba_impl* h);
int BaAssembleUndamped(pp_ba_impl* h, const pp_ba_options* o, bool evaluate);
bool BaInGroup(const pp_ba_impl* h);
int BaGroupReduce(pp_ba_impl* h, double* ptr, int64_t count, int op);
int PcgEnsureBuffers(pp_ba_impl* h);
void PcgFreeBuffers(pp_ba_impl* h);
int PcgSolve(pp_ba_impl* h, double radius, int max_iterations, double eta, int* iterations);
#ifdef __HIPCC__
__device__ __forceinline__ void LossRho(int type, double scale, double s, double* rho0, double* rho1) {
  if (type == PP_LOSS_TRIVIAL) { *rho0 = s; *rho1 = 1.0; return; }
  const double b = scale * scale, c = 1.0 / b;
  const double sum = 1.0 + s * c;
  if (type == PP_LOSS_SOFT_L1) {
    const double tmp = sqrt(sum);
    *rho0 = 2.0 * b * (tmp - 1.0);
    *rho1 = fmax(2.2250738585072014e-308, 1.0 / tmp);
  } else {
    *rho0 = b * log(sum);
    *rho1 = fmax(2.2250738585072014e-308, 1.0 / sum);
  }
}

#endif

}
```

privacy_preserving_sfm_amd/csrc/ba_solver.hip:

```cpp
#include <atomic>
#include <chrono>
#include <cmath>
#include <cstdlib>
#include <cstring>
#include <thread>

#include "ba_impl.hpp"
#include "lm_policy.hpp"
#include "resource_pool.hpp"
#include "line_residual.hpp"
#include "rccl_comm.hpp"

namespace ppsfm {

constexpr double kBig = 1e100;

struct Jrow {
  double jp[12];
  double jx[6];
};

__device__ __forceinline__ void LoadJp(const double* __restrict__ Jpose, int o, double jp[12]) {
  const double2* p = reinterpret_cast<const double2*>(Jpose + (size_t)12 * o);
#pragma unroll
  for (int i = 0; i < 6; ++i) { const double2 v = p[i]; jp[2 * i] = v.x; jp[2 * i + 1] = v.y; }
}
__device__ __forceinline__ void LoadJx(const double* __restrict__ Jpoint, int o, double jx[6]) {
  const double2* p = reinterpret_cast<const double2*>(Jpoint + (size_t)6 * o);
#pragma unroll
  for (int i = 0; i < 3; ++i) { const double2 v = p[i]; jx[2 * i] = v.x; jx[2 * i + 1] = v.y; }
}

__device__ __forceinline__ void PoseReduceBody(int c, const int32_t* __restrict__ pose_start, const int32_t* __restrict__ pose_obs,
                                               const double* __restrict__ Jpose, const double* __restrict__ r,
                                               double* __restrict__ U, double* __restrict__ gc) {
  __shared__ double red[4][27];
  const int lane = threadIdx.x & 63, wv = threadIdx.x >> 6;
  double u[21], g[6];
#pragma unroll
  for (int i = 0; i < 21; ++i) u[i] = 0.0;
#pragma unroll
  for (int i = 0; i < 6; ++i) g[i] = 0.0;
  auto add = [&](const double (&jp)[12], double r0, double r1) {
    int idx = 0;
#pragma unroll
    for (int a = 0; a < 6; ++a) {
      g[a] += jp[a] * r0 + jp[6 + a] * r1;
#pragma unroll
      for (int b = a; b < 6; ++b) u[idx++] += jp[a] * jp[b] + jp[6 + a] * jp[6 + b];
    }
  };
  const int begin = pose_start[c], end = pose_start[c + 1];
  if (end - begin <= 256) {
    const int e = begin + (int)threadIdx.x;
    if (e < end) {
      const int o = pose_obs[e];
      double jp[12];
      LoadJp(Jpose, o, jp);
      add(jp, r[2 * (size_t)o], r[2 * (size_t)o + 1]);
    }
  } else {
    for (int e = begin + (int)threadIdx.x; e < end; e += 512) {
      const bool two = e + 256 < end;
      const int o = pose_obs[e], o2 = pose_obs[two ? e + 256 : e];
      double jp[12], jq[12];
      LoadJp(Jpose, o, jp);
      LoadJp(Jpose, o2, jq);
      const double r0 = r[2 * (size_t)o], r1 = r[2 * (size_t)o + 1];
      const double w = two ? 1.0 : 0.0;
      const double q0 = w * r[2 * (size_t)o2], q1 = w * r[2 * (size_t)o2 + 1];
#pragma unroll
      for (int i = 0; i < 12; ++i) jq[i] *= w;
      add(jp, r0, r1);
      add(jq, q0, q1);
    }
  }
#pragma unroll
  for (int i = 0; i < 21; ++i) u[i] = WaveSumDpp(u[i]);
#pragma unroll
  for (int i = 0; i < 6; ++i) g[i] = WaveSumDpp(g[i]);
  if (lane == 0) {
#pragma unroll
    for (int i = 0; i < 21; ++i) red[wv][i] = u[i];
#pragma unroll
    for (int i = 0; i < 6; ++i) red[wv][21 + i] = g[i];
  }
  __syncthreads();
  if (threadIdx.x < 27) {
    const int i = threadIdx.x;
    const double v = ((red[0][i] + red[1][i]) + red[2][i]) + red[3][i];
    if (i >= 21) {
      gc[6 * (size_t)c + (i - 21)] = v;
    } else {
      int a = 0, rem = i;
      while (rem >= 6 - a) { rem -= 6 - a; ++a; }
      const int b = a + rem;
      U[36 * (size_t)c + 6 * a + b] = v; U[36 * (size_t)c + 6 * b + a] = v;
    }
  }
}

__device__ __forceinline__ void PointReduceBody(int gid, int P, const int32_t* __restrict__ pt_start, const int32_t* __restrict__ pt_obs,
                                                const double* __restrict__ Jpoint, const double* __restrict__ r,
                                                double* __restrict__ V, double* __restrict__ gp) {
  const int p = gid >> 2, q = gid & 3;
  double v[6] = {0, 0, 0, 0, 0, 0}, g[3] = {0, 0, 0};
  if (p < P) {
    for (int e = pt_start[p] + q; e < pt_start[p + 1]; e += 4) {
      const int o = pt_obs[e];
      double jx[6];
      LoadJx(Jpoint, o, jx);
      const double r0 = r[2 * (size_t)o], r1 = r[2 * (size_t)o + 1];
      v[0] += jx[0] * jx[0] + jx[3] * jx[3]; v[1] += jx[0] * jx[1] + jx[3] * jx[4]; v[2] += jx[0] * jx[2] + jx[3] * jx[5];
      v[3] += jx[1] * jx[1] + jx[4] * jx[4]; v[4] += jx[1] * jx[2] + jx[4] * jx[5]; v[5] += jx[2] * jx[2] + jx[5] * jx[5];
      g[0] += jx[0] * r0 + jx[3] * r1; g[1] += jx[1] * r0 + jx[4] * r1; g[2] += jx[2] * r0 + jx[5] * r1;
    }
  }
#pragma unroll
  for (int i = 0; i < 6; ++i) { v[i] += __shfl_xor(v[i], 1, 64); v[i] += __shfl_xor(v[i], 2, 64); }
#pragma unroll
  for (int i = 0; i < 3; ++i) { g[i] += __shfl_xor(g[i], 1, 64); g[i] += __shfl_xor(g[i], 2, 64); }
  if (p >= P || q != 0) return;
#pragma unroll
  for (int i = 0; i < 6; ++i) V[6 * (size_t)p + i] = v[i];
#pragma unroll
  for (int i = 0; i < 3; ++i) gp[3 * (size_t)p + i] = g[i];
}

__global__ __launch_bounds__(256) void k_reduce(int C, int P, const int32_t* __restrict__ pose_start, const int32_t* __restrict__ pose_obs,
                                                const int32_t* __restrict__ pt_start, const int32_t* __restrict__ pt_obs, const double* __restrict__ Jpose,
                                                const double* __restrict__ Jpoint, const double* __restrict__ r, double* __restrict__ U,
                                                double* __restrict__ gc, double* __restrict__ V, double* __restrict__ gp) {
  if ((int)blockIdx.x < C) PoseReduceBody(blockIdx.x, pose_start, pose_obs, Jpose, r, U, gc);
  else PointReduceBody(((int)blockIdx.x - C) * 256 + threadIdx.x, P, pt_start, pt_obs, Jpoint, r, V, gp);
}

__global__ __launch_bounds__(256) void k_jacobi_scale(int C, int P, const double* __restrict__ U, const double* __restrict__ V,
                                                      const uint8_t* __restrict__ pose_const, const uint8_t* __restrict__ tvec_mask,
                                                      const uint8_t* __restrict__ point_const, int jacobi, double* __restrict__ scale_c,
                                                      double* __restrict__ scale_p) {
  const int i = blockIdx.x * 256 + threadIdx.x;
  if (i < 6 * C) {
    const int c = i / 6, j = i % 6;
    const bool fixed = pose_const[c] || (j >= 3 && ((tvec_mask[c] >> (j - 3)) & 1));
    const double n2 = U[36 * (size_t)c + 7 * j];
    scale_c[i] = fixed ? 0.0 : (jacobi ? 1.0 / (1.0 + sqrt(n2)) : 1.0);
  }
  if (i < 3 * P) {
    const int p = i / 3, j = i % 3;
    const int di = j == 0 ? 0 : (j == 1 ? 3 : 5);
    const double n2 = V[6 * (size_t)p + di];
    scale_p[i] = point_const[p] ? 0.0 : (jacobi ? 1.0 / (1.0 + sqrt(n2)) : 1.0);
  }
}

__global__ __launch_bounds__(256) void k_lm_diagonal(int C, int P, const double* __restrict__ U, const double* __restrict__ V,
                                                     const double* __restrict__ scale_c, const double* __restrict__ scale_p, double dmin,
                                                     double dmax, double* __restrict__ diag_c, double* __restrict__ diag_p) {
  const int i = blockIdx.x * 256 + threadIdx.x;
  if (i < 6 * C) {
    const int c = i / 6, j = i % 6;
    const double s = scale_c[i];
    diag_c[i] = fmin(fmax(s * s * U[36 * (size_t)c + 7 * j], dmin), dmax);
  }
  if (i < 3 * P) {
    const int p = i / 3, j = i % 3;
    const int di = j == 0 ? 0 : (j == 1 ? 3 : 5);
    const double s = scale_p[i];
    diag_p[i] = fmin(fmax(s * s * V[6 * (size_t)p + di], dmin), dmax);
  }
}

__device__ __forceinline__ double PointBlockInverse(const double* __restrict__ v, double s0, double s1, double s2, double d0, double d1, double d2,
                                                    double inv_radius, double (&vi)[6]) {
  const double a = s0 * s0 * v[0] + d0 * inv_radius, b = s0 * s1 * v[1], c = s0 * s2 * v[2];
  const double d = s1 * s1 * v[3] + d1 * inv_radius, e = s1 * s2 * v[4];
  const double f = s2 * s2 * v[5] + d2 * inv_radius;
  const double c00 = d * f - e * e, c01 = c * e - b * f, c02 = b * e - c * d;
  const double det = a * c00 + b * c01 + c * c02;
  const double id = 1.0 / det;
  vi[0] = c00 * id; vi[1] = c01 * id; vi[2] = c02 * id;
  vi[3] = (a * f - c * c) * id; vi[4] = (b * c - a * e) * id; vi[5] = (a * d - b * b) * id;
  return det;
}
__device__ __forceinline__ double LmDiagonalEntry(double scale, double jtj, double dmin, double dmax) { return fmin(fmax(scale * scale * jtj, dmin), dmax); }

template <bool kWithDiagonal>
__device__ __forceinline__ void PointPrepareBody(int block, int P, const double* __restrict__ V, const double* __restrict__ gp,
                                                 const double* __restrict__ scale_p, double* __restrict__ diag_p,
                                                 const uint8_t* __restrict__ point_const, double inv_radius,
                                                 double* __restrict__ Vinv, double* __restrict__ vb, int32_t* __restrict__ flag,
                                                 int C, const double* __restrict__ U, const double* __restrict__ scale_c, double dmin, double dmax,
                                                 double* __restrict__ diag_c) {
  const int p = block * 256 + threadIdx.x;
  if (kWithDiagonal) {
    if (p < 6 * C) {
      const int c = p / 6, j = p % 6;
      diag_c[p] = LmDiagonalEntry(scale_c[p], U[36 * (size_t)c + 7 * j], dmin, dmax);
    }
    if (p < P) {
#pragma unroll
      for (int j = 0; j < 3; ++j) {
        const int di = j == 0 ? 0 : (j == 1 ? 3 : 5);
        diag_p[3 * p + j] = LmDiagonalEntry(scale_p[3 * p + j], V[6 * (size_t)p + di], dmin, dmax);
      }
    }
  }
  if (p >= P) return;
  double* vi = Vinv + 6 * (size_t)p;
  double* vbp = vb + 3 * (size_t)p;
  if (point_const[p]) {
#pragma unroll
    for (int i = 0; i < 6; ++i) vi[i] = 0.0;
    vbp[0] = vbp[1] = vbp[2] = 0.0;
    return;
  }
  const double s0 = scale_p[3 * p], s1 = scale_p[3 * p + 1], s2 = scale_p[3 * p + 2];
  double w[6];
  const double det = PointBlockInverse(V + 6 * (size_t)p, s0, s1, s2, diag_p[3 * p], diag_p[3 * p + 1], diag_p[3 * p + 2], inv_radius, w);
  if (!(det > 0.0) || !isfinite(det)) { atomicOr(flag, 2); }
#pragma unroll
  for (int i = 0; i < 6; ++i) vi[i] = w[i];
  const double b0 = -s0 * gp[3 * p], b1 = -s1 * gp[3 * p + 1], b2 = -s2 * gp[3 * p + 2];
  vbp[0] = w[0] * b0 + w[1] * b1 + w[2] * b2;
  vbp[1] = w[1] * b0 + w[3] * b1 + w[4] * b2;
  vbp[2] = w[2] * b0 + w[4] * b1 + w[5] * b2;
}

struct SchurArgs {
  int C, N, rhs_row;
  const int32_t *pose_start, *pose_obs, *obs_point;
  const double *Jpose, *Jpoint, *U, *gc, *Vinv, *vb, *scale_c, *scale_p, *diag_c;
  double inv_radius;
  double* S;
  int add_diagonal;
  double* Sd = nullptr;
  double* rhs_out = nullptr;
  const int32_t* spos = nullptr;
};

template <bool kWithDiagonal>
__device__ __forceinline__ void ObsPrepareBody(int block, int64_t M, const int32_t* __restrict__ obs_pose, const int32_t* __restrict__ obs_point,
                                               const double* __restrict__ Jpose, const double* __restrict__ Jpoint,
                                               const double* __restrict__ V, const double* __restrict__ diag_p, const uint8_t* __restrict__ point_const,
                                               double inv_radius, double dmin, double dmax, const double* __restrict__ scale_c,
                                               const double* __restrict__ scale_p, double* __restrict__ rec) {
  __shared__ __attribute__((aligned(16))) double sR[256 * kRecStride];
  const int tid = threadIdx.x;
  const int64_t o0 = (int64_t)block * 256, o = o0 + tid;
  if (o < M) {
    const int c = obs_pose[o], p = obs_point[o];
    double jp[12], jx[6];
    LoadJp(Jpose, (int)o, jp);
    LoadJx(Jpoint, (int)o, jx);
    double2* jo = reinterpret_cast<double2*>(sR + kRecStride * tid + 6);
#pragma unroll
    for (int i = 0; i < 6; ++i) {
      const int j0 = (2 * i) % 6, j1 = (2 * i + 1) % 6;
      jo[i] = make_double2(jp[2 * i] * scale_c[6 * c + j0], jp[2 * i + 1] * scale_c[6 * c + j1]);
    }
    const double s0 = scale_p[3 * p], s1 = scale_p[3 * p + 1], s2 = scale_p[3 * p + 2];
    double vi[6] = {0.0, 0.0, 0.0, 0.0, 0.0, 0.0};
    if (!point_const[p]) {
      const double* v = V + 6 * (size_t)p;
      double d0, d1, d2;
      if (kWithDiagonal) { d0 = LmDiagonalEntry(s0, v[0], dmin, dmax); d1 = LmDiagonalEntry(s1, v[3], dmin, dmax); d2 = LmDiagonalEntry(s2, v[5], dmin, dmax); }
      else { d0 = diag_p[3 * p]; d1 = diag_p[3 * p + 1]; d2 = diag_p[3 * p + 2]; }
      (void)PointBlockInverse(v, s0, s1, s2, d0, d1, d2, inv_radius, vi);
    }
    const double v00 = vi[0] * s0 * s0, v01 = vi[1] * s0 * s1, v02 = vi[2] * s0 * s2, v11 = vi[3] * s1 * s1, v12 = vi[4] * s1 * s2,
                 v22 = vi[5] * s2 * s2;
    double t[6];
#pragma unroll
    for (int r = 0; r < 2; ++r) {
      t[3 * r + 0] = jx[3 * r] * v00 + jx[3 * r + 1] * v01 + jx[3 * r + 2] * v02;
      t[3 * r + 1] = jx[3 * r] * v01 + jx[3 * r + 1] * v11 + jx[3 * r + 2] * v12;
      t[3 * r + 2] = jx[3 * r] * v02 + jx[3 * r + 1] * v12 + jx[3 * r + 2] * v22;
    }
    double2* to = reinterpret_cast<double2*>(sR + kRecStride * tid);
    double2* xo = reinterpret_cast<double2*>(sR + kRecStride * tid + 18);
    to[0] = make_double2(t[0], t[1]); to[1] = make_double2(t[2], t[3]); to[2] = make_double2(t[4], t[5]);
    xo[0] = make_double2(jx[0], jx[1]); xo[1] = make_double2(jx[2], jx[3]); xo[2] = make_double2(jx[4], jx[5]);
  }
  __syncthreads();
  const int64_t left = M - o0;
  const int n2 = (left < 256 ? (int)left : 256) * (kRecStride / 2);
  double2* dr = reinterpret_cast<double2*>(rec + (size_t)kRecStride * o0);
  const double2* sr = reinterpret_cast<const double2*>(sR);
#pragma unroll
  for (int it = 0; it < kRecStride / 2; ++it) {
    const int idx = it * 256 + tid;
    if (idx < n2) dr[idx] = sr[idx];
  }
}

template <bool kWithDiagonal>
__global__ __launch_bounds__(256) void k_prepare(int point_blocks, int P, const double* __restrict__ V, const double* __restrict__ gp, const double* __restrict__ scale_p,
                                                 double* __restrict__ diag_p, const uint8_t* __restrict__ point_const, double inv_radius, double* __restrict__ Vinv,
                                                 double* __restrict__ vb, int32_t* __restrict__ flag, int C, const double* __restrict__ U,
                                                 const double* __restrict__ scale_c, double dmin, double dmax, double* __restrict__ diag_c, int64_t M,
                                                 const int32_t* __restrict__ obs_pose, const int32_t* __restrict__ obs_point, const double* __restrict__ Jpose,
                                                 const double* __restrict__ Jpoint, double* __restrict__ rec, int obs_blocks, double* __restrict__ zS, int zN,
                                                 const int32_t* __restrict__ ztiles) {
  if ((int)blockIdx.x < point_blocks)
    PointPrepareBody<kWithDiagonal>(blockIdx.x, P, V, gp, scale_p, diag_p, point_const, inv_radius, Vinv, vb, flag, C, U, scale_c, dmin, dmax, diag_c);
  else if ((int)blockIdx.x < point_blocks + obs_blocks)
    ObsPrepareBody<kWithDiagonal>((int)blockIdx.x - point_blocks, M, obs_pose, obs_point, Jpose, Jpoint, V, diag_p, point_const, inv_radius, dmin, dmax, scale_c, scale_p, rec);
  else {
    const int zt = (int)blockIdx.x - point_blocks - obs_blocks;
    const int ti = ztiles[2 * zt], tj = ztiles[2 * zt + 1];
    double2* base = reinterpret_cast<double2*>(zS + (size_t)ti * 64 * zN + (size_t)tj * 64);
    for (int idx = threadIdx.x; idx < 64 * 32; idx += 256) base[(size_t)(idx >> 5) * (zN / 2) + (idx & 31)] = make_double2(0.0, 0.0);
  }
}

__device__ __forceinline__ void SchurSelfRhsBody(const SchurArgs& a, const double* __restrict__ rec, int c) {
  __shared__ double red[4][27];
  const int lane = threadIdx.x & 63, wv = threadIdx.x >> 6;
  if (c == 0 && threadIdx.x < 64 && !a.Sd) {
    const int j = a.rhs_row + threadIdx.x;
    if (j < a.N) {
      if (threadIdx.x > 0) a.S[(size_t)j * a.N + j] = 1.0;
      else if (a.add_diagonal) a.S[(size_t)j * a.N + j] = kBig;
    }
  }
  double u[21], acc[6];
#pragma unroll
  for (int i = 0; i < 21; ++i) u[i] = 0.0;
#pragma unroll
  for (int i = 0; i < 6; ++i) acc[i] = 0.0;
  for (int e = a.pose_start[c] + (int)threadIdx.x; e < a.pose_start[c + 1]; e += 256) {
    const int o = a.pose_obs[e];
    const int p = a.obs_point[o];
    double jp[12], q[12];
    {
      const double2* p = reinterpret_cast<const double2*>(RecT(rec, (size_t)o));
#pragma unroll
      for (int i = 0; i < 3; ++i) { const double2 v = p[i]; q[2 * i] = v.x; q[2 * i + 1] = v.y; }
#pragma unroll
      for (int i = 0; i < 6; ++i) { const double2 v = p[3 + i]; jp[2 * i] = v.x; jp[2 * i + 1] = v.y; }
#pragma unroll
      for (int i = 0; i < 3; ++i) { const double2 v = p[9 + i]; q[6 + 2 * i] = v.x; q[6 + 2 * i + 1] = v.y; }
    }
    const double g00 = q[0] * q[6] + q[1] * q[7] + q[2] * q[8], g01 = q[0] * q[9] + q[1] * q[10] + q[2] * q[11];
    const double g10 = q[3] * q[6] + q[4] * q[7] + q[5] * q[8], g11 = q[3] * q[9] + q[4] * q[10] + q[5] * q[11];
    int idx = 0;
#pragma unroll
    for (int x = 0; x < 6; ++x) {
      const double h0 = jp[x] * g00 + jp[6 + x] * g10, h1 = jp[x] * g01 + jp[6 + x] * g11;
#pragma unroll
      for (int y = x; y < 6; ++y) u[idx++] += h0 * jp[y] + h1 * jp[6 + y];
    }
    const double w0 = a.scale_p[3 * p] * a.vb[3 * (size_t)p], w1 = a.scale_p[3 * p + 1] * a.vb[3 * (size_t)p + 1],
                 w2 = a.scale_p[3 * p + 2] * a.vb[3 * (size_t)p + 2];
    const double t0 = q[6] * w0 + q[7] * w1 + q[8] * w2, t1 = q[9] * w0 + q[10] * w1 + q[11] * w2;
#pragma unroll
    for (int j = 0; j < 6; ++j) acc[j] += jp[j] * t0 + jp[6 + j] * t1;
  }
#pragma unroll
  for (int i = 0; i < 21; ++i) u[i] = WaveSumDpp(u[i]);
#pragma unroll
  for (int i = 0; i < 6; ++i) acc[i] = WaveSumDpp(acc[i]);
  if (lane == 0) {
#pragma unroll
    for (int i = 0; i < 21; ++i) red[wv][i] = u[i];
#pragma unroll
    for (int i = 0; i < 6; ++i) red[wv][21 + i] = acc[i];
  }
  __syncthreads();
  if (threadIdx.x < 27) {
    const int i = threadIdx.x;
    const double sum = ((red[0][i] + red[1][i]) + red[2][i]) + red[3][i];
    if (i >= 21) {
      const int j = i - 21;
      const double s = a.scale_c[6 * c + j];
      const double own = a.add_diagonal ? -s * a.gc[6 * (size_t)c + j] : 0.0;
      if (a.Sd) a.rhs_out[6 * (size_t)c + j] = own - sum;
      else a.S[(size_t)a.rhs_row * a.N + a.spos[6 * c] + j] = own - sum;
    } else {
      int x = 0, rem = i;
      while (rem >= 6 - x) { rem -= 6 - x; ++x; }
      const int y = x + rem;
      const double sa = a.scale_c[6 * c + x], sb = a.scale_c[6 * c + y];
      double v = 0.0;
      if (a.add_diagonal) {
        v = sa * sb * a.U[36 * (size_t)c + 6 * x + y];
        if (x == y) v = (sa == 0.0) ? 1.0 : v + a.diag_c[6 * c + x] * a.inv_radius;
      }
      v -= sum;
      if (a.Sd) { a.Sd[36 * (size_t)c + 6 * x + y] = v; a.Sd[36 * (size_t)c + 6 * y + x] = v; }
      else {
        const int sp = a.spos[6 * c];
        a.S[(size_t)(sp + x) * a.N + sp + y] = v;
        a.S[(size_t)(sp + y) * a.N + sp + x] = v;
      }
    }
  }
}

template <bool kStore>
__device__ __forceinline__ void SchurPairsBody(const SchurArgs& a, const double* __restrict__ rec,
                                               int64_t num_pairs, const int32_t* __restrict__ pair_start,
                                               const int32_t* __restrict__ pair_ij, const int32_t* __restrict__ pair_entries, int64_t block) {
  const int lane = threadIdx.x & 63;
  const int slot = lane / 6, ar = lane % 6;
  const int64_t wave = block * 4 + (threadIdx.x >> 6);
  const int64_t pr = wave * 10 + slot;
  if (slot >= 10 || pr >= num_pairs) return;
  const int bi = pair_ij[2 * pr], bj = pair_ij[2 * pr + 1];
  const int e0 = pair_start[2 * pr], e1 = pair_start[2 * pr + 1];
  double acc[6] = {0, 0, 0, 0, 0, 0};
  int2 next = e0 < e1 ? *reinterpret_cast<const int2*>(pair_entries + 2 * (size_t)e0) : make_int2(0, 0);
  for (int e = e0; e < e1; ++e) {
    const int2 oo = next;
    if (e + 1 < e1) next = *reinterpret_cast<const int2*>(pair_entries + 2 * (size_t)(e + 1));
    const double2* qi = reinterpret_cast<const double2*>(RecT(rec, (size_t)oo.x));
    const double2* qj = reinterpret_cast<const double2*>(RecX(rec, (size_t)oo.y));
    const double2* pj = reinterpret_cast<const double2*>(RecJ(rec, (size_t)oo.y));
    const double2 t0 = qi[0], t1 = qi[1], t2 = qi[2];
    const double2 x0 = qj[0], x1 = qj[1], x2 = qj[2];
    const double pi0 = RecJ(rec, (size_t)oo.x)[ar], pi1 = RecJ(rec, (size_t)oo.x)[6 + ar];
    const double g00 = t0.x * x0.x + t0.y * x0.y + t1.x * x1.x, g01 = t0.x * x1.y + t0.y * x2.x + t1.x * x2.y;
    const double g10 = t1.y * x0.x + t2.x * x0.y + t2.y * x1.x, g11 = t1.y * x1.y + t2.x * x2.x + t2.y * x2.y;
    const double h0 = pi0 * g00 + pi1 * g10, h1 = pi0 * g01 + pi1 * g11;
    const double2 j0 = pj[0], j1 = pj[1], j2 = pj[2], j3 = pj[3], j4 = pj[4], j5 = pj[5];
    acc[0] += h0 * j0.x + h1 * j3.x; acc[1] += h0 * j0.y + h1 * j3.y;
    acc[2] += h0 * j1.x + h1 * j4.x; acc[3] += h0 * j1.y + h1 * j4.y;
    acc[4] += h0 * j2.x + h1 * j5.x; acc[5] += h0 * j2.y + h1 * j5.y;
  }
  double2* dst = reinterpret_cast<double2*>(a.S + (size_t)(a.spos[6 * bi] + ar) * a.N + a.spos[6 * bj]);
  double2 d0 = make_double2(0.0, 0.0), d1 = d0, d2 = d0;
  if (!kStore) { d0 = dst[0]; d1 = dst[1]; d2 = dst[2]; }
  d0.x -= acc[0]; d0.y -= acc[1]; d1.x -= acc[2]; d1.y -= acc[3]; d2.x -= acc[4]; d2.y -= acc[5];
  dst[0] = d0; dst[1] = d1; dst[2] = d2;
}

__global__ __launch_bounds__(256) void k_schur_self_rhs(SchurArgs a, const double* __restrict__ rec) {
  SchurSelfRhsBody(a, rec, blockIdx.x);
}
template <bool kStore>
__global__ __launch_bounds__(256) void k_schur_pairs(SchurArgs a, const double* __restrict__ rec, int64_t num_pairs,
                                                     const int32_t* __restrict__ pair_start, const int32_t* __restrict__ pair_ij,
                                                     const int32_t* __restrict__ pair_entries) {
  SchurPairsBody<kStore>(a, rec, num_pairs, pair_start, pair_ij, pair_entries, blockIdx.x);
}
__global__ __launch_bounds__(256) void k_schur_blocks(SchurArgs a, const double* __restrict__ rec, int64_t num_pairs,
                                                      const int32_t* __restrict__ pair_start, const int32_t* __restrict__ pair_ij,
                                                      const int32_t* __restrict__ pair_entries) {
  if ((int)blockIdx.x < a.C) SchurSelfRhsBody(a, rec, blockIdx.x);
  else SchurPairsBody<true>(a, rec, num_pairs, pair_start, pair_ij, pair_entries, (int64_t)blockIdx.x - a.C);
}

template <int NV>
__global__ __launch_bounds__(256) void k_schur_wide_self(SchurArgs a, const double* __restrict__ rec, const double* __restrict__ JkS,
                                                         const int32_t* __restrict__ pose_camera, const int32_t* __restrict__ intr_off) {
  constexpr int W = 6 + NV, NU = W * (W + 1) / 2;
  __shared__ double red[4][NU + W];
  const int c = blockIdx.x;
  const int lane = threadIdx.x & 63, wv = threadIdx.x >> 6;
  if (c == 0 && threadIdx.x < 64) {
    const int j = a.rhs_row + threadIdx.x;
    if (j < a.N) {
      if (threadIdx.x > 0) a.S[(size_t)j * a.N + j] = 1.0;
      else if (a.add_diagonal) a.S[(size_t)j * a.N + j] = kBig;
    }
  }
  double u[NU], acc[W];
#pragma unroll
  for (int i = 0; i < NU; ++i) u[i] = 0.0;
#pragma unroll
  for (int i = 0; i < W; ++i) acc[i] = 0.0;
  for (int e = a.pose_start[c] + (int)threadIdx.x; e < a.pose_start[c + 1]; e += 256) {
    const int o = a.pose_obs[e];
    const int p = a.obs_point[o];
    double j0[W], j1[W], q[12];
    {
      const double2* r2 = reinterpret_cast<const double2*>(RecT(rec, (size_t)o));
#pragma unroll
      for (int i = 0; i < 3; ++i) { const double2 v = r2[i]; q[2 * i] = v.x; q[2 * i + 1] = v.y; }
#pragma unroll
      for (int i = 0; i < 3; ++i) { const double2 v = r2[3 + i]; j0[2 * i] = v.x; j0[2 * i + 1] = v.y; }
#pragma unroll
      for (int i = 0; i < 3; ++i) { const double2 v = r2[6 + i]; j1[2 * i] = v.x; j1[2 * i + 1] = v.y; }
#pragma unroll
      for (int i = 0; i < 3; ++i) { const double2 v = r2[9 + i]; q[6 + 2 * i] = v.x; q[6 + 2 * i + 1] = v.y; }
      const double2* k2 = reinterpret_cast<const double2*>(JkS + (size_t)2 * kCamStride * o);
#pragma unroll
      for (int i = 0; i < NV / 2; ++i) { const double2 v0 = k2[i], v1 = k2[kCamStride / 2 + i]; j0[6 + 2 * i] = v0.x; j0[7 + 2 * i] = v0.y; j1[6 + 2 * i] = v1.x; j1[7 + 2 * i] = v1.y; }
    }
    const double g00 = q[0] * q[6] + q[1] * q[7] + q[2] * q[8], g01 = q[0] * q[9] + q[1] * q[10] + q[2] * q[11];
    const double g10 = q[3] * q[6] + q[4] * q[7] + q[5] * q[8], g11 = q[3] * q[9] + q[4] * q[10] + q[5] * q[11];
    int idx = 0;
#pragma unroll
    for (int x = 0; x < W; ++x) {
      const double h0 = j0[x] * g00 + j1[x] * g10, h1 = j0[x] * g01 + j1[x] * g11;
      const double d0 = h0 - j0[x], d1 = h1 - j1[x];
#pragma unroll
      for (int y = x; y < W; ++y) u[idx++] += (y < 6) ? h0 * j0[y] + h1 * j1[y] : d0 * j0[y] + d1 * j1[y];
    }
    const double w0 = a.scale_p[3 * p] * a.vb[3 * (size_t)p], w1 = a.scale_p[3 * p + 1] * a.vb[3 * (size_t)p + 1],
                 w2 = a.scale_p[3 * p + 2] * a.vb[3 * (size_t)p + 2];
    const double t0 = q[6] * w0 + q[7] * w1 + q[8] * w2, t1 = q[9] * w0 + q[10] * w1 + q[11] * w2;
#pragma unroll
    for (int j = 0; j < W; ++j) acc[j] += j0[j] * t0 + j1[j] * t1;
  }
#pragma unroll
  for (int i = 0; i < NU; ++i) u[i] = WaveSumDpp(u[i]);
#pragma unroll
  for (int i = 0; i < W; ++i) acc[i] = WaveSumDpp(acc[i]);
  if (lane == 0) {
#pragma unroll
    for (int i = 0; i < NU; ++i) red[wv][i] = u[i];
#pragma unroll
    for (int i = 0; i < W; ++i) red[wv][NU + i] = acc[i];
  }
  __syncthreads();
  if (threadIdx.x < NU + W) {
    const int i = threadIdx.x;
    const double sum = ((red[0][i] + red[1][i]) + red[2][i]) + red[3][i];
    const int sp = a.spos[6 * c];
    const int ioff = 6 * a.C + intr_off[pose_camera[c]];
    if (i >= NU) {
      const int j = i - NU;
      const int v = j < 6 ? 6 * c + j : ioff + j - 6;
      const double own = a.add_diagonal ? -a.scale_c[v] * a.gc[v] : 0.0;
      a.S[(size_t)a.rhs_row * a.N + sp + j] = own - sum;
    } else {
      int x = 0, rem = i;
      while (rem >= W - x) { rem -= W - x; ++x; }
      const int y = x + rem;
      double v = 0.0;
      if (a.add_diagonal) {
        if (y < 6) {
          const double sa = a.scale_c[6 * c + x], sb = a.scale_c[6 * c + y];
          v = sa * sb * a.U[36 * (size_t)c + 6 * x + y];
          if (x == y) v = (sa == 0.0) ? 1.0 : v + a.diag_c[6 * c + x] * a.inv_radius;
        } else if (x == y) v = a.diag_c[ioff + x - 6] * a.inv_radius;
      }
      v -= sum;
      a.S[(size_t)(sp + x) * a.N + sp + y] = v;
      a.S[(size_t)(sp + y) * a.N + sp + x] = v;
    }
  }
}
template <int NV, bool kStore>
__global__ __launch_bounds__(256) void k_schur_wide_pairs(SchurArgs a, const double* __restrict__ rec, const double* __restrict__ JkS, int64_t num_pairs,
                                                          const int32_t* __restrict__ pair_start, const int32_t* __restrict__ pair_ij,
                                                          const int32_t* __restrict__ pair_entries) {
  constexpr int W = 6 + NV, kSlots = 64 / W;
  const int lane = threadIdx.x & 63;
  const int slot = lane / W, ar = lane % W;
  const int64_t wave = (int64_t)blockIdx.x * 4 + (threadIdx.x >> 6);
  const int64_t pr = wave * kSlots + slot;
  if (slot >= kSlots || pr >= num_pairs) return;
  const int bi = pair_ij[2 * pr], bj = pair_ij[2 * pr + 1];
  const int e0 = pair_start[2 * pr], e1 = pair_start[2 * pr + 1];
  double acc[W];
#pragma unroll
  for (int i = 0; i < W; ++i) acc[i] = 0.0;
  int2 next = e0 < e1 ? *reinterpret_cast<const int2*>(pair_entries + 2 * (size_t)e0) : make_int2(0, 0);
  for (int e = e0; e < e1; ++e) {
    const int2 oo = next;
    if (e + 1 < e1) next = *reinterpret_cast<const int2*>(pair_entries + 2 * (size_t)(e + 1));
    const double2* qi = reinterpret_cast<const double2*>(RecT(rec, (size_t)oo.x));
    const double2* qj = reinterpret_cast<const double2*>(RecX(rec, (size_t)oo.y));
    const double2* pj = reinterpret_cast<const double2*>(RecJ(rec, (size_t)oo.y));
    const double2* kj = reinterpret_cast<const double2*>(JkS + (size_t)2 * kCamStride * oo.y);
    const double2 t0 = qi[0], t1 = qi[1], t2 = qi[2];
    const double2 x0 = qj[0], x1 = qj[1], x2 = qj[2];
    const double* ri = ar < 6 ? RecJ(rec, (size_t)oo.x) + ar : JkS + (size_t)2 * kCamStride * oo.x + (ar - 6);
    const double pi0 = ri[0], pi1 = ri[ar < 6 ? 6 : kCamStride];
    const double g00 = t0.x * x0.x + t0.y * x0.y + t1.x * x1.x, g01 = t0.x * x1.y + t0.y * x2.x + t1.x * x2.y;
    const double g10 = t1.y * x0.x + t2.x * x0.y + t2.y * x1.x, g11 = t1.y * x1.y + t2.x * x2.x + t2.y * x2.y;
    const double h0 = pi0 * g00 + pi1 * g10, h1 = pi0 * g01 + pi1 * g11;
    const double2 j0 = pj[0], j1 = pj[1], j2 = pj[2], j3 = pj[3], j4 = pj[4], j5 = pj[5];
    acc[0] += h0 * j0.x + h1 * j3.x; acc[1] += h0 * j0.y + h1 * j3.y;
    acc[2] += h0 * j1.x + h1 * j4.x; acc[3] += h0 * j1.y + h1 * j4.y;
    acc[4] += h0 * j2.x + h1 * j5.x; acc[5] += h0 * j2.y + h1 * j5.y;
#pragma unroll
    for (int b = 0; b < NV / 2; ++b) {
      const double2 k0 = kj[b], k1 = kj[kCamStride / 2 + b];
      acc[6 + 2 * b] += h0 * k0.x + h1 * k1.x; acc[7 + 2 * b] += h0 * k0.y + h1 * k1.y;
    }
  }
  double2* dst = reinterpret_cast<double2*>(a.S + (size_t)(a.spos[6 * bi] + ar) * a.N + a.spos[6 * bj]);
#pragma unroll
  for (int b = 0; b < W / 2; ++b) { double2 d = kStore ? make_double2(0.0, 0.0) : dst[b]; d.x -= acc[2 * b]; d.y -= acc[2 * b + 1]; dst[b] = d; }
}

__device__ __forceinline__ void SchurChunksBody(const double* __restrict__ rec, int num_chunks, const int32_t* __restrict__ chunk, const int32_t* __restrict__ pair_entries,
                                                double* __restrict__ partials, int64_t block) {
  const int lane = threadIdx.x & 63;
  const int slot = lane / 6, ar = lane % 6;
  const int64_t ch = (block * 4 + (threadIdx.x >> 6)) * 10 + slot;
  if (slot >= 10 || ch >= num_chunks) return;
  const int e0 = chunk[3 * ch + 1], e1 = chunk[3 * ch + 2];
  double acc[6] = {0, 0, 0, 0, 0, 0};
  int2 next = e0 < e1 ? *reinterpret_cast<const int2*>(pair_entries + 2 * (size_t)e0) : make_int2(0, 0);
  for (int e = e0; e < e1; ++e) {
    const int2 oo = next;
    if (e + 1 < e1) next = *reinterpret_cast<const int2*>(pair_entries + 2 * (size_t)(e + 1));
    const double2* qi = reinterpret_cast<const double2*>(RecT(rec, (size_t)oo.x));
    const double2* qj = reinterpret_cast<const double2*>(RecX(rec, (size_t)oo.y));
    const double2* pj = reinterpret_cast<const double2*>(RecJ(rec, (size_t)oo.y));
    const double2 t0 = qi[0], t1 = qi[1], t2 = qi[2];
    const double2 x0 = qj[0], x1 = qj[1], x2 = qj[2];
    const double pi0 = RecJ(rec, (size_t)oo.x)[ar], pi1 = RecJ(rec, (size_t)oo.x)[6 + ar];
    const double g00 = t0.x * x0.x + t0.y * x0.y + t1.x * x1.x, g01 = t0.x * x1.y + t0.y * x2.x + t1.x * x2.y;
    const double g10 = t1.y * x0.x + t2.x * x0.y + t2.y * x1.x, g11 = t1.y * x1.y + t2.x * x2.x + t2.y * x2.y;
    const double h0 = pi0 * g00 + pi1 * g10, h1 = pi0 * g01 + pi1 * g11;
    const double2 j0 = pj[0], j1 = pj[1], j2 = pj[2], j3 = pj[3], j4 = pj[4], j5 = pj[5];
    acc[0] += h0 * j0.x + h1 * j3.x; acc[1] += h0 * j0.y + h1 * j3.y;
    acc[2] += h0 * j1.x + h1 * j4.x; acc[3] += h0 * j1.y + h1 * j4.y;
    acc[4] += h0 * j2.x + h1 * j5.x; acc[5] += h0 * j2.y + h1 * j5.y;
  }
  double2* dst = reinterpret_cast<double2*>(partials + 36 * (size_t)chunk[3 * ch] + 6 * ar);
  dst[0] = make_double2(acc[0], acc[1]); dst[1] = make_double2(acc[2], acc[3]); dst[2] = make_double2(acc[4], acc[5]);
}
__global__ __launch_bounds__(256) void k_schur_self_chunks(SchurArgs a, const double* __restrict__ rec, int num_chunks, const int32_t* __restrict__ chunk,
                                                           const int32_t* __restrict__ pair_entries, double* __restrict__ partials) {
  if ((int)blockIdx.x < a.C) SchurSelfRhsBody(a, rec, blockIdx.x);
  else SchurChunksBody(rec, num_chunks, chunk, pair_entries, partials, (int64_t)blockIdx.x - a.C);
}
template <bool kStore>
__global__ __launch_bounds__(256) void k_schur_chunk_reduce(SchurArgs a, int64_t num_pairs, const int32_t* __restrict__ pair_ij, const int32_t* __restrict__ pair_chunk,
                                                            const double* __restrict__ partials) {
  const int64_t it = (int64_t)blockIdx.x * 256 + threadIdx.x;
  if (it >= 36 * num_pairs) return;
  const int64_t pr = it / 36;
  const int el = (int)(it % 36);
  const int c0 = pair_chunk[pr], c1 = pair_chunk[pr + 1];
  if (c0 == c1 && !kStore) return;
  double sum = 0.0;
  int ch = c0;
  for (; ch + 8 <= c1; ch += 8) {
    double v[8];
#pragma unroll
    for (int u = 0; u < 8; ++u) v[u] = partials[36 * (size_t)(ch + u) + el];
#pragma unroll
    for (int u = 0; u < 8; ++u) sum += v[u];
  }
  for (; ch < c1; ++ch) sum += partials[36 * (size_t)ch + el];
  double* dst = a.S + (size_t)(a.spos[6 * pair_ij[2 * pr]] + el / 6) * a.N + a.spos[6 * pair_ij[2 * pr + 1]] + el % 6;
  *dst = (kStore ? 0.0 : *dst) - sum;
}

struct StepArgs {
  int C, P;
  int64_t M;
  const int32_t *pt_start, *pt_obs, *obs_pose, *obs_point;
  const double *Jpose, *Jpoint, *r, *Vinv, *vb, *scale_c, *scale_p, *step_c;
  double* step_p;
  double* partials;
  const double* JkS;
  const int32_t *obs_cam, *intr_off, *intr_nv;
  double* cand_partials = nullptr;
  const double *la = nullptr, *lb = nullptr, *lc = nullptr, *poses = nullptr, *points = nullptr, *intr = nullptr;
  int loss_type = 0;
  double loss_scale = 1.0;
};

__device__ __forceinline__ void IntrStepProduct(const StepArgs& a, int64_t o, double* m0, double* m1) {
  if (!a.JkS) return;
  const int k = a.obs_cam[o] >> 4;
  const int off = a.intr_off[k];
  if (off < 0) return;
  const int nv = a.intr_nv[k];
  const double* j = a.JkS + (size_t)2 * kCamStride * o;
  const double* d = a.step_c + 6 * a.C + off;
  for (int c = 0; c < nv; ++c) { *m0 += j[c] * d[c]; *m1 += j[kCamStride + c] * d[c]; }
}

__global__ __launch_bounds__(256) void k_backsub_points(StepArgs a) {
  const int gid = blockIdx.x * 256 + threadIdx.x;
  const int p = gid >> 2, q = gid & 3;
  double acc[3] = {0, 0, 0};
  if (p < a.P) {
    for (int e = a.pt_start[p] + q; e < a.pt_start[p + 1]; e += 4) {
      const int o = a.pt_obs[e];
      const int c = a.obs_pose[o];
      double jp[12], jx[6];
      LoadJp(a.Jpose, o, jp);
      LoadJx(a.Jpoint, o, jx);
      double m0 = 0.0, m1 = 0.0;
#pragma unroll
      for (int j = 0; j < 6; ++j) { const double d = a.scale_c[6 * c + j] * a.step_c[6 * c + j]; m0 += jp[j] * d; m1 += jp[6 + j] * d; }
      IntrStepProduct(a, o, &m0, &m1);
#pragma unroll
      for (int j = 0; j < 3; ++j) acc[j] += jx[j] * m0 + jx[3 + j] * m1;
    }
  }
#pragma unroll
  for (int j = 0; j < 3; ++j) { acc[j] += __shfl_xor(acc[j], 1, 64); acc[j] += __shfl_xor(acc[j], 2, 64); }
  if (p >= a.P || q != 0) return;
  const double s0 = a.scale_p[3 * p], s1 = a.scale_p[3 * p + 1], s2 = a.scale_p[3 * p + 2];
  const double w0 = s0 * acc[0], w1 = s1 * acc[1], w2 = s2 * acc[2];
  const double* vi = a.Vinv + 6 * (size_t)p;
  a.step_p[3 * (size_t)p + 0] = a.vb[3 * (size_t)p + 0] - (vi[0] * w0 + vi[1] * w1 + vi[2] * w2);
  a.step_p[3 * (size_t)p + 1] = a.vb[3 * (size_t)p + 1] - (vi[1] * w0 + vi[3] * w1 + vi[4] * w2);
  a.step_p[3 * (size_t)p + 2] = a.vb[3 * (size_t)p + 2] - (vi[2] * w0 + vi[4] * w1 + vi[5] * w2);
}

__device__ __forceinline__ bool LastBlockDone(int32_t* counter, int num_blocks) {
  __shared__ int s_last;
  __syncthreads();
  if (threadIdx.x == 0) {
    __threadfence();
    const int t = atomicAdd(counter, 1);
    s_last = (t == num_blocks - 1) ? 1 : 0;
    if (s_last) { *counter = 0; __threadfence(); }
  }
  __syncthreads();
  return s_last != 0;
}
__device__ __forceinline__ void BlockSumTo(const double* __restrict__ v, int n, double* __restrict__ out) {
  __shared__ double sh[256];
  double acc = 0.0;
  for (int i = threadIdx.x; i < n; i += 256) acc += v[i];
  sh[threadIdx.x] = acc;
  __syncthreads();
  for (int s = 128; s > 0; s >>= 1) {
    if ((int)threadIdx.x < s) sh[threadIdx.x] += sh[threadIdx.x + s];
    __syncthreads();
  }
  if (threadIdx.x == 0) *out = sh[0];
}

__device__ __forceinline__ void QuatPlus(const double* q, double d0, double d1, double d2, double* out);
__device__ __forceinline__ double ScaledStep(double scale, double step) {
#pragma clang fp contract(off)
  return scale * step;
}
__device__ __forceinline__ void ModelCostBody(const StepArgs& a, int block) {
  const int64_t o = (int64_t)block * 256 + threadIdx.x;
  double val = 0.0, half_rho = 0.0;
  if (o < a.M) {
    const int c = a.obs_pose[o], p = a.obs_point[o];
    double jp[12], jx[6];
    LoadJp(a.Jpose, (int)o, jp);
    LoadJx(a.Jpoint, (int)o, jx);
    double dc[6], dp[3];
#pragma unroll
    for (int j = 0; j < 6; ++j) dc[j] = ScaledStep(a.scale_c[6 * c + j], a.step_c[6 * c + j]);
#pragma unroll
    for (int j = 0; j < 3; ++j) dp[j] = ScaledStep(a.scale_p[3 * p + j], a.step_p[3 * (size_t)p + j]);
    double m0 = 0.0, m1 = 0.0;
#pragma unroll
    for (int j = 0; j < 6; ++j) { m0 += jp[j] * dc[j]; m1 += jp[6 + j] * dc[j]; }
    IntrStepProduct(a, o, &m0, &m1);
#pragma unroll
    for (int j = 0; j < 3; ++j) { m0 += jx[j] * dp[j]; m1 += jx[3 + j] * dp[j]; }
    val = -(m0 * (a.r[2 * o] + m0 / 2.0) + m1 * (a.r[2 * o + 1] + m1 / 2.0));
    if (a.cand_partials) {
      const double* pose = a.poses + 7 * (size_t)c;
      double qn[4];
      QuatPlus(pose, dc[0], dc[1], dc[2], qn);
      const double tn[3] = {pose[4] + dc[3], pose[5] + dc[4], pose[6] + dc[5]};
      const double Xn[3] = {a.points[3 * (size_t)p] + dp[0], a.points[3 * (size_t)p + 1] + dp[1], a.points[3 * (size_t)p + 2] + dp[2]};
      const int ck = a.obs_cam[o];
      double res[2];
      LineResidualOnly(ck & 15, a.intr + (size_t)kCamStride * (ck >> 4), qn, tn, Xn, a.la[o], a.lb[o], a.lc[o], res);
      double rho0, rho1;
      LossRho(a.loss_type, a.loss_scale, res[0] * res[0] + res[1] * res[1], &rho0, &rho1);
      half_rho = 0.5 * rho0;
    }
  }
  __shared__ double wsum[4], csum[4];
  val = WaveSum(val);
  if (a.cand_partials) half_rho = WaveSum(half_rho);
  if ((threadIdx.x & 63) == 0) { wsum[threadIdx.x >> 6] = val; csum[threadIdx.x >> 6] = half_rho; }
  __syncthreads();
  if (threadIdx.x == 0) {
    a.partials[block] = (wsum[0] + wsum[1]) + (wsum[2] + wsum[3]);
    if (a.cand_partials) a.cand_partials[block] = (csum[0] + csum[1]) + (csum[2] + csum[3]);
  }
}
__global__ __launch_bounds__(256) void k_sum(const double* __restrict__ partials, int n, double* __restrict__ out) { BlockSumTo(partials, n, out); }

__device__ __forceinline__ void QuatPlus(const double* q, double d0, double d1, double d2, double* out) {
  const double n = sqrt(d0 * d0 + d1 * d1 + d2 * d2);
  if (n > 0.0) {
    const double s = sin(n) / n, w1 = cos(n);
    const double x1 = s * d0, y1 = s * d1, z1 = s * d2;
    const double w2 = q[0], x2 = q[1], y2 = q[2], z2 = q[3];
    out[0] = w1 * w2 - x1 * x2 - y1 * y2 - z1 * z2;
    out[1] = w1 * x2 + x1 * w2 + y1 * z2 - z1 * y2;
    out[2] = w1 * y2 - x1 * z2 + y1 * w2 + z1 * x2;
    out[3] = w1 * z2 + x1 * y2 - y1 * x2 + z1 * w2;
  } else {
    out[0] = q[0]; out[1] = q[1]; out[2] = q[2]; out[3] = q[3];
  }
}

__device__ __forceinline__ void ApplyStepBody(int i, int C, int P, const double* __restrict__ poses, const double* __restrict__ points,
                                              const double* __restrict__ scale_c, const double* __restrict__ scale_p,
                                              const double* __restrict__ step_c, const double* __restrict__ step_p,
                                              double* __restrict__ poses_c, double* __restrict__ points_c) {
  if (i < C) {
    const double* q = poses + 7 * (size_t)i;
    double d[6];
#pragma unroll
    for (int j = 0; j < 6; ++j) d[j] = ScaledStep(scale_c[6 * i + j], step_c[6 * i + j]);
    double qn[4];
    QuatPlus(q, d[0], d[1], d[2], qn);
    double* o = poses_c + 7 * (size_t)i;
    o[0] = qn[0]; o[1] = qn[1]; o[2] = qn[2]; o[3] = qn[3];
    o[4] = q[4] + d[3]; o[5] = q[5] + d[4]; o[6] = q[6] + d[5];
  }
  if (i < P) {
#pragma unroll
    for (int j = 0; j < 3; ++j) points_c[3 * (size_t)i + j] = points[3 * (size_t)i + j] + ScaledStep(scale_p[3 * i + j], step_p[3 * (size_t)i + j]);
  }
}

__global__ __launch_bounds__(256) void k_model_cost_apply(StepArgs a, int obs_blocks, const double* __restrict__ poses, const double* __restrict__ points,
                                                          double* __restrict__ poses_c, double* __restrict__ points_c) {
  if ((int)blockIdx.x < obs_blocks) ModelCostBody(a, blockIdx.x);
  else ApplyStepBody(((int)blockIdx.x - obs_blocks) * 256 + threadIdx.x, a.C, a.P, poses, points, a.scale_c, a.scale_p, a.step_c, a.step_p, poses_c, points_c);
}

template <bool kIntr>
__global__ __launch_bounds__(256) void k_step_points(StepArgs a, int point_blocks, const double* __restrict__ poses, const double* __restrict__ points,
                                                     double* __restrict__ poses_c, double* __restrict__ points_c) {
  if ((int)blockIdx.x >= point_blocks) {
    const int i = ((int)blockIdx.x - point_blocks) * 256 + threadIdx.x;
    if (i < a.C) {
      const double* q = poses + 7 * (size_t)i;
      double d[6];
#pragma unroll
      for (int j = 0; j < 6; ++j) d[j] = ScaledStep(a.scale_c[6 * i + j], a.step_c[6 * i + j]);
      double qn[4];
      QuatPlus(q, d[0], d[1], d[2], qn);
      double* o = poses_c + 7 * (size_t)i;
      o[0] = qn[0]; o[1] = qn[1]; o[2] = qn[2]; o[3] = qn[3];
      o[4] = q[4] + d[3]; o[5] = q[5] + d[4]; o[6] = q[6] + d[5];
    }
    return;
  }
  const int gid = blockIdx.x * 256 + threadIdx.x;
  const int p = gid >> 2, q = gid & 3;
  const bool live = p < a.P;
  struct Row { double jp[12], jx[6], dc[6], u0, u1; int o, c; };
  Row R[2];
  auto load = [&](int o, Row& w) {
    w.o = o; w.c = a.obs_pose[o];
    LoadJp(a.Jpose, o, w.jp);
    LoadJx(a.Jpoint, o, w.jx);
    w.u0 = 0.0; w.u1 = 0.0;
#pragma unroll
    for (int j = 0; j < 6; ++j) { w.dc[j] = ScaledStep(a.scale_c[6 * w.c + j], a.step_c[6 * w.c + j]); w.u0 += w.jp[j] * w.dc[j]; w.u1 += w.jp[6 + j] * w.dc[j]; }
    if (kIntr) IntrStepProduct(a, o, &w.u0, &w.u1);
  };
  double acc[3] = {0.0, 0.0, 0.0};
  const int begin = live ? a.pt_start[p] + q : 0, end = live ? a.pt_start[p + 1] : 0;
  bool have[2] = {false, false};
  if (begin < end) {
    have[0] = true; have[1] = begin + 4 < end;
    const int o0 = a.pt_obs[begin], o1 = a.pt_obs[have[1] ? begin + 4 : begin];
    load(o0, R[0]);
    load(o1, R[1]);
#pragma unroll
    for (int j = 0; j < 3; ++j) acc[j] += R[0].jx[j] * R[0].u0 + R[0].jx[3 + j] * R[0].u1;
    if (have[1]) {
#pragma unroll
      for (int j = 0; j < 3; ++j) acc[j] += R[1].jx[j] * R[1].u0 + R[1].jx[3 + j] * R[1].u1;
    }
  }
  for (int e = begin + 8; e < end; e += 4) {
    Row w;
    load(a.pt_obs[e], w);
#pragma unroll
    for (int j = 0; j < 3; ++j) acc[j] += w.jx[j] * w.u0 + w.jx[3 + j] * w.u1;
  }
#pragma unroll
  for (int j = 0; j < 3; ++j) { acc[j] += __shfl_xor(acc[j], 1, 64); acc[j] += __shfl_xor(acc[j], 2, 64); }
  double dp[3] = {0.0, 0.0, 0.0}, Xn[3] = {0.0, 0.0, 0.0};
  if (live) {
    const double s0 = a.scale_p[3 * p], s1 = a.scale_p[3 * p + 1], s2 = a.scale_p[3 * p + 2];
    const double w0 = s0 * acc[0], w1 = s1 * acc[1], w2 = s2 * acc[2];
    const double* vi = a.Vinv + 6 * (size_t)p;
    const double e0 = a.vb[3 * (size_t)p + 0] - (vi[0] * w0 + vi[1] * w1 + vi[2] * w2);
    const double e1 = a.vb[3 * (size_t)p + 1] - (vi[1] * w0 + vi[3] * w1 + vi[4] * w2);
    const double e2 = a.vb[3 * (size_t)p + 2] - (vi[2] * w0 + vi[4] * w1 + vi[5] * w2);
    dp[0] = ScaledStep(s0, e0); dp[1] = ScaledStep(s1, e1); dp[2] = ScaledStep(s2, e2);
#pragma unroll
    for (int j = 0; j < 3; ++j) Xn[j] = points[3 * (size_t)p + j] + dp[j];
    if (q == 0) {
      a.step_p[3 * (size_t)p + 0] = e0; a.step_p[3 * (size_t)p + 1] = e1; a.step_p[3 * (size_t)p + 2] = e2;
#pragma unroll
      for (int j = 0; j < 3; ++j) points_c[3 * (size_t)p + j] = Xn[j];
    }
  }
  double val = 0.0, half_rho = 0.0;
  auto terms = [&](const Row& w) {
    double m0 = w.u0, m1 = w.u1;
#pragma unroll
    for (int j = 0; j < 3; ++j) { m0 += w.jx[j] * dp[j]; m1 += w.jx[3 + j] * dp[j]; }
    val -= m0 * (a.r[2 * (size_t)w.o] + m0 / 2.0) + m1 * (a.r[2 * (size_t)w.o + 1] + m1 / 2.0);
    const double* pose = poses + 7 * (size_t)w.c;
    double qn[4];
    QuatPlus(pose, w.dc[0], w.dc[1], w.dc[2], qn);
    const double tn[3] = {pose[4] + w.dc[3], pose[5] + w.dc[4], pose[6] + w.dc[5]};
    const int ck = a.obs_cam[w.o];
    double res[2];
    LineResidualOnly(ck & 15, a.intr + (size_t)kCamStride * (ck >> 4), qn, tn, Xn, a.la[w.o], a.lb[w.o], a.lc[w.o], res);
    double rho0, rho1;
    LossRho(a.loss_type, a.loss_scale, res[0] * res[0] + res[1] * res[1], &rho0, &rho1);
    half_rho += 0.5 * rho0;
  };
  if (have[0]) terms(R[0]);
  if (have[1]) terms(R[1]);
  for (int e = begin + 8; e < end; e += 4) {
    Row w;
    load(a.pt_obs[e], w);
    terms(w);
  }
  __shared__ double wsum[4], csum[4];
  val = WaveSum(val);
  half_rho = WaveSum(half_rho);
  if ((threadIdx.x & 63) == 0) { wsum[threadIdx.x >> 6] = val; csum[threadIdx.x >> 6] = half_rho; }
  __syncthreads();
  if (threadIdx.x == 0) {
    a.partials[blockIdx.x] = (wsum[0] + wsum[1]) + (wsum[2] + wsum[3]);
    a.cand_partials[blockIdx.x] = (csum[0] + csum[1]) + (csum[2] + csum[3]);
  }
}

__global__ __launch_bounds__(256) void k_apply_intr(int K, int C, const int32_t* __restrict__ intr_off, const int32_t* __restrict__ intr_col,
                                                    const double* __restrict__ intr, const double* __restrict__ scale_c, const double* __restrict__ step_c,
                                                    double* __restrict__ intr_c) {
  const int i = blockIdx.x * 256 + threadIdx.x;
  if (i >= K * kCamStride) return;
  const int k = i / kCamStride;
  const int col = intr_col[i], off = intr_off[k];
  double v = intr[i];
  if (off >= 0 && col >= 0) v += scale_c[6 * C + off + col] * step_c[6 * C + off + col];
  intr_c[i] = v;
}

constexpr int kNormsIntrThreads = 1024;
__global__ __launch_bounds__(kNormsIntrThreads) void k_norms_intr(int K, int C, const int32_t* __restrict__ intr_off, const int32_t* __restrict__ intr_nv,
                                                   const int32_t* __restrict__ camera_model_np, const double* __restrict__ intr, const double* __restrict__ gc,
                                                   const double* __restrict__ scale_c, const double* __restrict__ step_c, double* __restrict__ scal, int count_norms,
                                                   double* __restrict__ host_out, unsigned long long ticket) {
  __shared__ double wmax[kNormsIntrThreads / 64], wst[kNormsIntrThreads / 64], wxn[kNormsIntrThreads / 64];
  double gmax = 0.0, st = 0.0, xn = 0.0;
  for (int k = threadIdx.x; k < K; k += kNormsIntrThreads) {
    const int off = intr_off[k];
    if (off < 0) continue;
    for (int j = 0; j < intr_nv[k]; ++j) {
      gmax = fmax(gmax, fabs(gc[6 * C + off + j]));
      if (step_c && count_norms) { const double d = scale_c[6 * C + off + j] * step_c[6 * C + off + j]; st += d * d; }
    }
    if (count_norms) for (int j = 0; j < camera_model_np[k]; ++j) xn += intr[k * kCamStride + j] * intr[k * kCamStride + j];
  }
#pragma unroll
  for (int off = 32; off > 0; off >>= 1) gmax = fmax(gmax, __shfl_xor(gmax, off, 64));
  st = WaveSum(st); xn = WaveSum(xn);
  if ((threadIdx.x & 63) == 0) { wmax[threadIdx.x >> 6] = gmax; wst[threadIdx.x >> 6] = st; wxn[threadIdx.x >> 6] = xn; }
  __syncthreads();
  if (threadIdx.x == 0) {
    gmax = 0.0; st = 0.0; xn = 0.0;
    for (int w = 0; w < kNormsIntrThreads / 64; ++w) { gmax = fmax(gmax, wmax[w]); st += wst[w]; xn += wxn[w]; }
    scal[kGradMax] = fmax(scal[kGradMax], gmax); scal[kStepNorm2] += st; scal[kXNorm2] += xn; __threadfence();
  }
  __syncthreads();
  if (threadIdx.x >= 64) return;
  if (host_out) {
    const int b = threadIdx.x;
    if (b < kNumScalars && b != kTicketSlot) {
      const unsigned long long v = __hip_atomic_load(reinterpret_cast<const unsigned long long*>(scal) + b, __ATOMIC_RELAXED, __HIP_MEMORY_SCOPE_AGENT);
      __hip_atomic_store(reinterpret_cast<unsigned long long*>(host_out) + b, v, __ATOMIC_RELAXED, __HIP_MEMORY_SCOPE_SYSTEM);
    }
    if (ticket != 0) {
      __builtin_amdgcn_fence(__ATOMIC_RELEASE, "");
      if (b == 0) __hip_atomic_store(reinterpret_cast<unsigned long long*>(host_out) + kTicketSlot, ticket, __ATOMIC_RELEASE, __HIP_MEMORY_SCOPE_SYSTEM);
    }
  }
}

__global__ __launch_bounds__(256) void k_norms_partial(int C, int P, const double* __restrict__ poses, const double* __restrict__ points,
                                                       const double* __restrict__ gc, const double* __restrict__ gp, const double* __restrict__ scale_c,
                                                       const double* __restrict__ scale_p, const double* __restrict__ step_c,
                                                       const double* __restrict__ step_p, double* __restrict__ part, int32_t* __restrict__ done_counter,
                                                       double* __restrict__ scal, int norm_blocks, const double* __restrict__ sum0, int n0,
                                                       double* __restrict__ out0, const double* __restrict__ sum1, int n1, double* __restrict__ out1,
                                                       double* __restrict__ host_out, unsigned long long ticket, int count_pose_norms, int pose_blocks) {
  __shared__ double smax[256], sstep[256], sx[256];
  if ((int)blockIdx.x >= norm_blocks) {
    if ((int)blockIdx.x == norm_blocks) BlockSumTo(sum0, n0, out0);
    else BlockSumTo(sum1, n1, out1);
  } else {
    double gmax = 0.0, st = 0.0, xn = 0.0;
    const int point_blocks = norm_blocks - pose_blocks;
    const bool pose_role = (int)blockIdx.x >= point_blocks;
    const int stride = (pose_role ? pose_blocks : point_blocks) * 256, t0 = ((int)blockIdx.x - (pose_role ? point_blocks : 0)) * 256 + threadIdx.x;
    for (int c = t0; c < C && pose_role; c += stride) {
      const double* q = poses + 7 * (size_t)c;
      if (scale_c[6 * c] != 0.0) {
        double qn[4];
        QuatPlus(q, -gc[6 * (size_t)c], -gc[6 * (size_t)c + 1], -gc[6 * (size_t)c + 2], qn);
#pragma unroll
        for (int j = 0; j < 4; ++j) gmax = fmax(gmax, fabs(q[j] - qn[j]));
        if (count_pose_norms) {
#pragma unroll
          for (int j = 0; j < 7; ++j) xn += q[j] * q[j];
        }
      }
#pragma unroll
      for (int j = 3; j < 6; ++j) if (scale_c[6 * c + j] != 0.0) gmax = fmax(gmax, fabs(gc[6 * (size_t)c + j]));
      if (step_c && count_pose_norms) {
#pragma unroll
        for (int j = 0; j < 6; ++j) { const double d = scale_c[6 * c + j] * step_c[6 * c + j]; st += d * d; }
      }
    }
    for (int i = t0; i < 3 * P && !pose_role; i += stride) {
      const double sp = scale_p[i], gv = gp[i], xv = points[i], sv = step_p ? step_p[i] : 0.0;
      if (sp != 0.0) { gmax = fmax(gmax, fabs(gv)); xn += xv * xv; }
      const double d = sp * sv;
      st += d * d;
    }
    smax[threadIdx.x] = gmax; sstep[threadIdx.x] = st; sx[threadIdx.x] = xn;
    __syncthreads();
    for (int s = 128; s > 0; s >>= 1) {
      if ((int)threadIdx.x < s) {
        smax[threadIdx.x] = fmax(smax[threadIdx.x], smax[threadIdx.x + s]);
        sstep[threadIdx.x] += sstep[threadIdx.x + s];
        sx[threadIdx.x] += sx[threadIdx.x + s];
      }
      __syncthreads();
    }
    if (threadIdx.x == 0) { part[3 * blockIdx.x] = smax[0]; part[3 * blockIdx.x + 1] = sstep[0]; part[3 * blockIdx.x + 2] = sx[0]; }
  }
  if (LastBlockDone(done_counter, (int)gridDim.x)) {
    const int b = threadIdx.x;
    const bool in = b < norm_blocks;
    smax[b] = in ? __hip_atomic_load(part + 3 * b, __ATOMIC_RELAXED, __HIP_MEMORY_SCOPE_AGENT) : 0.0;
    sstep[b] = in ? __hip_atomic_load(part + 3 * b + 1, __ATOMIC_RELAXED, __HIP_MEMORY_SCOPE_AGENT) : 0.0;
    sx[b] = in ? __hip_atomic_load(part + 3 * b + 2, __ATOMIC_RELAXED, __HIP_MEMORY_SCOPE_AGENT) : 0.0;
    __syncthreads();
    for (int s = 128; s > 0; s >>= 1) {
      if (b < s) { smax[b] = fmax(smax[b], smax[b + s]); sstep[b] += sstep[b + s]; sx[b] += sx[b + s]; }
      __syncthreads();
    }
    if (b == 0) {
      __hip_atomic_store(scal + kGradMax, smax[0], __ATOMIC_RELAXED, __HIP_MEMORY_SCOPE_AGENT);
      __hip_atomic_store(scal + kStepNorm2, sstep[0], __ATOMIC_RELAXED, __HIP_MEMORY_SCOPE_AGENT);
      __hip_atomic_store(scal + kXNorm2, sx[0], __ATOMIC_RELAXED, __HIP_MEMORY_SCOPE_AGENT);
    }
    if (host_out) {
      __syncthreads();
      if (b < kNumScalars) {
        unsigned long long v;
        if (b == kGradMax) v = __double_as_longlong(smax[0]);
        else if (b == kStepNorm2) v = __double_as_longlong(sstep[0]);
        else if (b == kXNorm2) v = __double_as_longlong(sx[0]);
        else v = __hip_atomic_load(reinterpret_cast<const unsigned long long*>(scal) + b, __ATOMIC_RELAXED, __HIP_MEMORY_SCOPE_AGENT);
        if (b != kTicketSlot) __hip_atomic_store(reinterpret_cast<unsigned long long*>(host_out) + b, v, __ATOMIC_RELAXED, __HIP_MEMORY_SCOPE_SYSTEM);
      }
      if (ticket != 0 && b < 64) {
        __builtin_amdgcn_fence(__ATOMIC_RELEASE, "");
        if (b == 0) __hip_atomic_store(reinterpret_cast<unsigned long long*>(host_out) + kTicketSlot, ticket, __ATOMIC_RELEASE, __HIP_MEMORY_SCOPE_SYSTEM);
      }
    }
  }
}

static bool InGroup(const pp_ba_impl* h) { return h->comm != nullptr || h->allreduce != nullptr; }
static bool SparseActive(const pp_ba_impl* h) { return h->sparse_tiles && (!InGroup(h) || h->structure_from_covisibility); }
static int ApplyLinearSolverStructure(pp_ba_impl* h) {
  if (!h->S || h->iterative) return PP_OK;
  PP_HIP_TRY(hipSetDevice(h->device));
  std::lock_guard<std::recursive_mutex> setup_lock(DeviceSetupMutex());
  if (!h->Lfac && CholeskyNeedsFactorArray(h->chol, h->N)) { const int rc = HandleAlloc(&h->Lfac, (size_t)h->N * h->N); if (rc) return rc; }
  const CholeskySystem sys{h->S, h->N, h->n_red, h->Linv, h->Lfac, h->spos_identity ? h->step_c : h->step_s, h->d_flag, h->stream};
  bool new_map = false;
  { const int rc = CholeskyBind(h->chol, sys, SparseActive(h) ? h->tile_nz.data() : nullptr, &new_map); if (rc) return rc; }
  if (new_map) PP_HIP_TRY(hipMemsetAsync(h->S, 0, sizeof(double) * (size_t)h->N * h->N, h->stream));
  return PP_OK;
}

static int EnsureSolverBuffers(pp_ba_impl* h) {
  if (h->S || h->pcg_state) return PP_OK;
  std::lock_guard<std::recursive_mutex> setup_lock(DeviceSetupMutex());
  const int C = h->C, P = h->P;
  h->N = ((h->n_red + 1 + 63) / 64) * 64;
  int rc;
#define A(ptr, n) if ((rc = HandleAlloc(&h->ptr, (size_t)(n)))) return rc
  A(U, 36 * (size_t)C); A(gc, (size_t)h->n_red); A(V, 6 * (size_t)P); A(gp, 3 * (size_t)P); A(Vinv, 6 * (size_t)P); A(vb, 3 * (size_t)P);
  A(scale_c, (size_t)h->n_red); A(scale_p, 3 * (size_t)P); A(diag_c, (size_t)h->n_red); A(diag_p, 3 * (size_t)P);
  if (!h->iterative) { A(S, (size_t)h->N * h->N); A(Linv, CholeskyWorkspaceDoubles(h->N)); }
  A(JpS, kRecStride * (size_t)h->M); A(norm_part, 3 * 256); A(step_c, (size_t)h->N); A(step_p, 3 * (size_t)P);
  if (!h->spos_identity) { A(step_s, (size_t)h->N); }
#undef A
  for (int i = 0; i < 8; ++i) if ((rc = PoolEventAcquire(&h->tev[i], true))) return rc;
  for (int i = 0; i < 2; ++i) if ((rc = PoolEventAcquire(&h->tev_eval[i], true))) return rc;
  if ((rc = PoolEventAcquire(&h->ev_readback, false))) return rc;
  if (h->iterative) return PcgEnsureBuffers(h);
  PP_HIP_TRY(hipMemsetAsync(h->S, 0, sizeof(double) * (size_t)h->N * h->N, h->stream));
  if (h->sparse_tiles) {
    const int T = h->N / 64;
    std::vector<int32_t> list;
    for (int i = 0; i < T; ++i) for (int j = 0; j <= i; ++j) if (h->tile_nz[(size_t)i * T + j]) { list.push_back(i); list.push_back(j); }
    if ((rc = HandleAlloc(&h->nz_tile_list, list.size()))) return rc;
    PP_HIP_TRY(hipMemcpyAsync(h->nz_tile_list, list.data(), sizeof(int32_t) * list.size(), hipMemcpyHostToDevice, h->stream));
    PP_HIP_TRY(hipStreamSynchronize(h->stream));
  }
  return ApplyLinearSolverStructure(h);
}

__global__ __launch_bounds__(256) void k_gather_step(int n, const int32_t* __restrict__ spos, const double* __restrict__ x, double* __restrict__ step) {
  const int v = blockIdx.x * 256 + threadIdx.x;
  if (v < n) step[v] = x[spos[v]];
}

static SchurArgs MakeSchurArgs(pp_ba_impl* h, double radius) {
  SchurArgs a;
  a.C = h->C; a.N = h->N; a.rhs_row = h->n_red;
  a.pose_start = h->pose_start; a.pose_obs = h->pose_obs; a.obs_point = h->obs_point;
  a.Jpose = h->Jpose; a.Jpoint = h->Jpoint; a.U = h->U; a.gc = h->gc; a.Vinv = h->Vinv; a.vb = h->vb;
  a.scale_c = h->scale_c; a.scale_p = h->scale_p; a.diag_c = h->diag_c;
  a.inv_radius = 1.0 / radius; a.S = h->S; a.add_diagonal = h->group_rank == 0 ? 1 : 0;
  a.spos = h->spos;
  return a;
}
static StepArgs MakeStepArgs(pp_ba_impl* h) {
  StepArgs a;
  a.C = h->C; a.P = h->P; a.M = h->M;
  a.pt_start = h->pt_start; a.pt_obs = h->pt_obs; a.obs_pose = h->obs_pose; a.obs_point = h->obs_point;
  a.Jpose = h->Jpose; a.Jpoint = h->Jpoint; a.r = h->r; a.Vinv = h->Vinv; a.vb = h->vb;
  a.scale_c = h->scale_c; a.scale_p = h->scale_p; a.step_c = h->step_c; a.step_p = h->step_p; a.partials = h->partials + h->partials_stride;
  a.JkS = h->NI > 0 ? h->JkS_intr : nullptr; a.obs_cam = h->obs_cam; a.intr_off = h->intr_off; a.intr_nv = h->intr_nv;
  return a;
}

static int GroupReduce(pp_ba_impl* h, double* ptr, int64_t count, int op) {
  if (h->comm) return CommAllReduce(h->comm, ptr, count, op, h->stream);
  if (!h->allreduce) return PP_OK;
  PP_HIP_TRY(hipStreamSynchronize(h->stream));
  const int rc = h->allreduce(h->allreduce_ctx, ptr, count, op);
  if (rc) { SetLastError("allreduce callback returned %d", rc); return PP_ERR_INVALID; }
  return PP_OK;
}
bool BaInGroup(const pp_ba_impl* h) { return InGroup(h); }
int BaGroupReduce(pp_ba_impl* h, double* ptr, int64_t count, int op) { return GroupReduce(h, ptr, count, op); }
static int GroupBegin(pp_ba_impl* h) { return h->comm ? CommGroupStart() : PP_OK; }
static int GroupEnd(pp_ba_impl* h) { return h->comm ? CommGroupEnd() : PP_OK; }
struct GroupScope {
  pp_ba_impl* h; bool open = false;
  explicit GroupScope(pp_ba_impl* hh) : h(hh) {}
  int Begin() { const int rc = GroupBegin(h); open = rc == PP_OK; return rc; }
  int End() { open = false; return GroupEnd(h); }
  ~GroupScope() { if (open) (void)GroupEnd(h); }
};
__global__ void k_flag_to_scalar(const int32_t* __restrict__ flag, double* __restrict__ slot) { *slot = (double)(*flag & 7); }
__global__ void k_scalar_to_flag(const double* __restrict__ slot, int32_t* __restrict__ flag) { const int v = (int)*slot; if (v) atomicOr(flag, v); }

__global__ __launch_bounds__(256) void k_pack_lower(const double* __restrict__ S, int N, int rows, double* __restrict__ packed, int unpack, double* __restrict__ Sout) {
  const int r = blockIdx.y;
  const size_t base = (size_t)r * (r + 1) / 2;
  for (int c = blockIdx.x * 256 + threadIdx.x; c <= r && r < rows; c += gridDim.x * 256) {
    if (unpack) Sout[(size_t)r * N + c] = packed[base + c];
    else packed[base + c] = S[(size_t)r * N + c];
  }
}

__global__ __launch_bounds__(256) void k_pack_tiles(const double* __restrict__ S, int N, const int32_t* __restrict__ tiles, double* __restrict__ packed, int unpack, double* __restrict__ Sout) {
  const int ti = tiles[2 * blockIdx.x], tj = tiles[2 * blockIdx.x + 1];
  double2* pk = reinterpret_cast<double2*>(packed + (size_t)blockIdx.x * 64 * 64);
  for (int idx = threadIdx.x; idx < 64 * 32; idx += 256) {
    const size_t at = ((size_t)ti * 64 + (idx >> 5)) * N + (size_t)tj * 64 + 2 * (idx & 31);
    if (unpack) *reinterpret_cast<double2*>(Sout + at) = pk[idx];
    else pk[idx] = *reinterpret_cast<const double2*>(S + at);
  }
}

static int EvaluateAndReduce(pp_ba_impl* h, bool fold_cost = false) {
  hipStream_t s = h->stream;
  int rc = LaunchEval(h, 0, h->NI > 0 ? 1 : 0, true, h->poses, h->points, fold_cost ? nullptr : h->scal + kCost, true);
  if (rc) return rc;
  hipLaunchKernelGGL(k_reduce, dim3(h->C + CeilDiv(4 * (int64_t)h->P, 256)), dim3(256), 0, s, h->C, h->P, h->pose_start, h->pose_obs, h->pt_start, h->pt_obs, h->Jpose,
                     h->Jpoint, h->r, h->U, h->gc, h->V, h->gp);
  PP_HIP_TRY(hipGetLastError());
  if ((rc = IntrSumsAfterEval(h))) return rc;
  if (InGroup(h)) {
    GroupScope g(h);
    if ((rc = g.Begin())) return rc;
    if ((rc = GroupReduce(h, h->U, 36 * (int64_t)h->C, PP_REDUCE_SUM))) return rc;
    if ((rc = GroupReduce(h, h->gc, (int64_t)h->n_red, PP_REDUCE_SUM))) return rc;
    if (h->NI > 0 && (rc = GroupReduce(h, h->cnI, (int64_t)h->NI, PP_REDUCE_SUM))) return rc;
    if (!fold_cost && (rc = GroupReduce(h, h->scal + kCost, 1, PP_REDUCE_SUM))) return rc;
    if ((rc = g.End())) return rc;
  }
  return PP_OK;
}

static int LaunchNorms(pp_ba_impl* h, bool with_step, int fold = 0, double* host_slot = nullptr, unsigned long long ticket = 0) {
  const int pose_blocks = std::min(8, CeilDiv(h->C, 256));
  const int nblk = 64 + pose_blocks;
  const double* model_partials = h->partials + h->partials_stride;
  const int n_trial = fold == 2 && h->trial_partials > 0 ? h->trial_partials : h->num_partials;
  hipLaunchKernelGGL(k_norms_partial, dim3(nblk + fold), dim3(256), 0, h->stream, h->C, h->P, h->poses, h->points, h->gc, h->gp, h->scale_c,
                     h->scale_p, with_step ? h->step_c : nullptr, with_step ? h->step_p : nullptr, h->norm_part, h->d_flag + 2, h->scal, nblk,
                     fold ? h->partials : nullptr, fold == 2 ? n_trial : h->num_partials, fold == 2 ? h->scal + kCostCand : h->scal + kCost,
                     fold == 2 ? model_partials : nullptr, n_trial, h->scal + kModelChange, h->NI > 0 ? nullptr : host_slot, h->NI > 0 ? 0ull : ticket,
                     h->group_rank == 0 ? 1 : 0, pose_blocks);
  if (h->NI > 0)
    hipLaunchKernelGGL(k_norms_intr, dim3(1), dim3(kNormsIntrThreads), 0, h->stream, h->K, h->C, h->intr_off, h->intr_nv, h->cam_np, h->intr, h->gc, h->scale_c,
                       with_step ? h->step_c : nullptr, h->scal, h->group_rank == 0 ? 1 : 0, host_slot, ticket);
  PP_HIP_TRY(hipGetLastError());
  if (InGroup(h)) {
    int rc;
    if (with_step) hipLaunchKernelGGL(k_flag_to_scalar, dim3(1), dim3(1), 0, h->stream, h->d_flag, h->scal + kTicketSlot);
    {
      GroupScope g(h);
      if ((rc = g.Begin())) return rc;
      if ((rc = GroupReduce(h, h->scal + kGradMax, 1, PP_REDUCE_MAX))) return rc;
      if ((rc = GroupReduce(h, h->scal + kStepNorm2, 2, PP_REDUCE_SUM))) return rc;
      if (fold == 1 && (rc = GroupReduce(h, h->scal + kCost, 1, PP_REDUCE_SUM))) return rc;
      if (fold == 2 && (rc = GroupReduce(h, h->scal + kCostCand, 2, PP_REDUCE_SUM))) return rc;
      if (with_step && (rc = GroupReduce(h, h->scal + kTicketSlot, 1, PP_REDUCE_MAX))) return rc;
      if ((rc = g.End())) return rc;
    }
    if (with_step) hipLaunchKernelGGL(k_scalar_to_flag, dim3(1), dim3(1), 0, h->stream, h->scal + kTicketSlot, h->d_flag);
    PP_HIP_TRY(hipGetLastError());
  }
  return PP_OK;
}

static int EnsureSpack(pp_ba_impl* h, int64_t count) {
  if (h->Spack_cap >= count) return PP_OK;
  if (h->Spack) PoolDeviceFree(h->Spack);
  h->Spack = nullptr; h->Spack_cap = 0;
  const int rc = HandleAlloc(&h->Spack, (size_t)count);
  if (rc == PP_OK) h->Spack_cap = count;
  return rc;
}

static int AssembleReducedSystem(pp_ba_impl* h, double radius, bool refresh_diagonal = false, double dmin = 0.0, double dmax = 0.0) {
  hipStream_t s = h->stream;
  const bool store_blocks = h->pairs_complete && !h->iterative && !InGroup(h) && (h->NI == 0 || h->intr_wide_nv > 0 || h->spos_identity);
  const int zero_tiles = (!store_blocks && !h->iterative && SparseActive(h)) ? h->num_nz_tiles : 0;
  if (!store_blocks && !h->iterative && !zero_tiles) PP_HIP_TRY(hipMemsetAsync(h->S, 0, sizeof(double) * (size_t)h->N * h->N, s));
  if (store_blocks && h->NI > 0 && h->spos_identity) PP_HIP_TRY(hipMemsetAsync(h->S + (size_t)6 * h->C * h->N, 0, sizeof(double) * (size_t)h->NI * h->N, s));
  {
    const int point_blocks = CeilDiv(refresh_diagonal ? std::max(h->P, 6 * h->C) : h->P, 256);
    const dim3 grid(point_blocks + h->num_partials + zero_tiles);
    hipLaunchKernelGGL(refresh_diagonal ? k_prepare<true> : k_prepare<false>, grid, dim3(256), 0, s, point_blocks, h->P, h->V, h->gp, h->scale_p, h->diag_p, h->point_const,
                       1.0 / radius, h->Vinv, h->vb, h->d_flag, h->C, h->U, h->scale_c, dmin, dmax, h->diag_c, h->M, h->obs_pose, h->obs_point, h->Jpose, h->Jpoint, h->JpS,
                       h->num_partials, h->S, h->N, (const int32_t*)h->nz_tile_list);
  }
  SchurArgs a = MakeSchurArgs(h, radius);
  if (h->iterative) { a.Sd = h->pcg_Sd; a.rhs_out = h->pcg_b; }
  if (h->iterative) {
    hipLaunchKernelGGL(k_schur_self_rhs, dim3(h->C), dim3(256), 0, s, a, h->JpS);
    PP_HIP_TRY(hipGetLastError());
    if (InGroup(h)) {
      GroupScope g(h);
      int rc;
      if ((rc = g.Begin())) return rc;
      if ((rc = GroupReduce(h, h->pcg_Sd, 36 * (int64_t)h->C, PP_REDUCE_SUM))) return rc;
      if ((rc = GroupReduce(h, h->pcg_b, 6 * (int64_t)h->C, PP_REDUCE_SUM))) return rc;
      if ((rc = g.End())) return rc;
    }
    { const int rc = IntrAssemble(h, 1.0 / radius, a.add_diagonal); if (rc) return rc; }
    if (InGroup(h) && h->NI > 0) {
      GroupScope g(h);
      int rc;
      if ((rc = g.Begin())) return rc;
      if ((rc = GroupReduce(h, h->pcg_Scomp, 12 * (int64_t)h->NI, PP_REDUCE_SUM))) return rc;
      if ((rc = GroupReduce(h, h->pcg_b + 6 * (size_t)h->C, (int64_t)h->NI, PP_REDUCE_SUM))) return rc;
      if ((rc = g.End())) return rc;
    }
    return PP_OK;
  }
  if (h->pairs_chunked && h->num_pairs > 0) {
    hipLaunchKernelGGL(k_schur_self_chunks, dim3(h->C + CeilDiv(h->small_num_chunks, 40)), dim3(256), 0, s, a, h->JpS, h->small_num_chunks, h->small_chunk, h->pair_entries,
                       h->small_partials);
    const dim3 grid(CeilDiv(36 * h->num_pairs, 256));
    if (store_blocks) hipLaunchKernelGGL(k_schur_chunk_reduce<true>, grid, dim3(256), 0, s, a, h->num_pairs, h->pair_ij, h->small_pair_chunk, h->small_partials);
    else hipLaunchKernelGGL(k_schur_chunk_reduce<false>, grid, dim3(256), 0, s, a, h->num_pairs, h->pair_ij, h->small_pair_chunk, h->small_partials);
  } else if (h->intr_wide_nv > 0) {
    { const int rc = IntrScaledJacobians(h); if (rc) return rc; }
    const int W = 6 + h->intr_wide_nv;
    const dim3 gp((unsigned)CeilDiv(h->num_pairs, (int64_t)(4 * (64 / W))));
#define PP_WIDE(NV) do { \
      hipLaunchKernelGGL(k_schur_wide_self<NV>, dim3(h->C), dim3(256), 0, s, a, h->JpS, h->JkS_intr, h->pose_camera, h->intr_off); \
      if (h->num_pairs > 0) { \
        if (store_blocks) hipLaunchKernelGGL((k_schur_wide_pairs<NV, true>), gp, dim3(256), 0, s, a, h->JpS, h->JkS_intr, h->num_pairs, h->pair_start, h->pair_ij, h->pair_entries); \
        else hipLaunchKernelGGL((k_schur_wide_pairs<NV, false>), gp, dim3(256), 0, s, a, h->JpS, h->JkS_intr, h->num_pairs, h->pair_start, h->pair_ij, h->pair_entries); } } while (0)
    switch (h->intr_wide_nv) { case 2: PP_WIDE(2); break; case 4: PP_WIDE(4); break; case 6: PP_WIDE(6); break; default: PP_WIDE(8); break; }
#undef PP_WIDE
  } else if (store_blocks && h->num_pairs > 0) {
    hipLaunchKernelGGL(k_schur_blocks, dim3(h->C + CeilDiv(h->num_pairs, 40)), dim3(256), 0, s, a, h->JpS, h->num_pairs, h->pair_start, h->pair_ij,
                       h->pair_entries);
  } else {
    hipLaunchKernelGGL(k_schur_self_rhs, dim3(h->C), dim3(256), 0, s, a, h->JpS);
    if (h->num_pairs > 0)
      hipLaunchKernelGGL(k_schur_pairs<false>, dim3(CeilDiv(h->num_pairs, 40)), dim3(256), 0, s, a, h->JpS, h->num_pairs, h->pair_start, h->pair_ij,
                         h->pair_entries);
  }
  PP_HIP_TRY(hipGetLastError());
  { const int rc = IntrAssemble(h, 1.0 / radius, a.add_diagonal); if (rc) return rc; }
  if (InGroup(h) && SparseActive(h) && h->nz_tile_list && h->num_nz_tiles > 0) {
    const int64_t count = (int64_t)h->num_nz_tiles * 64 * 64;
    if (const int rc = EnsureSpack(h, count)) return rc;
    hipLaunchKernelGGL(k_pack_tiles, dim3(h->num_nz_tiles), dim3(256), 0, s, h->S, h->N, (const int32_t*)h->nz_tile_list, h->Spack, 0, (double*)nullptr);
    const int rc = GroupReduce(h, h->Spack, count, PP_REDUCE_SUM);
    if (rc) return rc;
    hipLaunchKernelGGL(k_pack_tiles, dim3(h->num_nz_tiles), dim3(256), 0, s, (const double*)nullptr, h->N, (const int32_t*)h->nz_tile_list, h->Spack, 1, h->S);
    PP_HIP_TRY(hipGetLastError());
  } else if (InGroup(h)) {
    const int rows = h->n_red + 1;
    const int64_t count = (int64_t)rows * (rows + 1) / 2;
    if (const int rc = EnsureSpack(h, count)) return rc;
    const dim3 grid(std::max(1, std::min(64, CeilDiv(rows, 256))), rows);
    hipLaunchKernelGGL(k_pack_lower, grid, dim3(256), 0, s, h->S, h->N, rows, h->Spack, 0, (double*)nullptr);
    const int rc = GroupReduce(h, h->Spack, count, PP_REDUCE_SUM);
    if (rc) return rc;
    hipLaunchKernelGGL(k_pack_lower, grid, dim3(256), 0, s, (const double*)nullptr, h->N, rows, h->Spack, 1, h->S);
    PP_HIP_TRY(hipGetLastError());
  }
  return PP_OK;
}

static int ReadScalars(pp_ba_impl* h) {
  PP_HIP_TRY(hipMemcpyAsync(h->h_scal, h->scal, sizeof(double) * kNumScalars, hipMemcpyDeviceToHost, h->stream));
  PP_HIP_TRY(hipStreamSynchronize(h->stream));
  return PP_OK;
}
static int WaitTicket(pp_ba_impl* h, unsigned long long ticket) {
  const long spin_us = h->sw.ticket_spin_us;
  const volatile unsigned long long* t = reinterpret_cast<const volatile unsigned long long*>(h->h_scal) + kTicketSlot;
  const auto t0 = std::chrono::steady_clock::now();
  bool synced = false;
  for (unsigned spins = 0; *t != ticket; ++spins) {
#if defined(__x86_64__) && !defined(__HIP_DEVICE_COMPILE__)
    __builtin_ia32_pause();
#endif
    if ((spins & 0xFF) != 0xFF) continue;
    const auto waited = std::chrono::steady_clock::now() - t0;
    if (waited > std::chrono::seconds(2) && !synced) {
      PP_HIP_TRY(hipStreamSynchronize(h->stream));
      synced = true;
      if (*t != ticket) { SetLastError("pp_ba_solve: the trial step's scalars never arrived"); return PP_ERR_HIP; }
      break;
    }
    if (waited > std::chrono::microseconds(spin_us)) std::this_thread::sleep_for(std::chrono::microseconds(50));
  }
  std::atomic_thread_fence(std::memory_order_acquire);
  return PP_OK;
}
static int32_t HostFlag(const pp_ba_impl* h) { int32_t f; std::memcpy(&f, h->h_scal + kNumScalars - 1, sizeof(f)); return f; }

struct PhaseTimer {
  pp_ba_impl* h; bool on; int n = 0; int phase[8];
  PhaseTimer(pp_ba_impl* hh, bool enabled) : h(hh), on(enabled) { if (on) (void)hipEventRecord(h->tev[0], h->stream); }
  void Mark(int ph) { if (on && n < 7) { phase[n] = ph; ++n; (void)hipEventRecord(h->tev[n], h->stream); } }
  void Collect() {
    if (!on) return;
    if (n > 0) (void)hipEventSynchronize(h->tev[n]);
    for (int i = 0; i < n; ++i) {
      float ms = 0;
      if (hipEventElapsedTime(&ms, h->tev[i], h->tev[i + 1]) == hipSuccess) { h->timings_ms[phase[i]] += ms; h->timing_calls[phase[i]] += 1; }
    }
    n = 0;
  }
};


static int EvaluateAndScale(pp_ba_impl* h, const pp_ba_options* o, bool fold, PhaseTimer& timer) {
  PP_HIP_TRY(hipMemsetAsync(h->d_flag, 0, 4 * sizeof(int32_t), h->stream));
  if (const int rc = EvaluateAndReduce(h, fold)) return rc;
  timer.Mark(PP_BA_T_EVAL);
  const int grid = CeilDiv(std::max<int64_t>(6 * (int64_t)h->C, 3 * (int64_t)h->P), 256);
  hipLaunchKernelGGL(k_jacobi_scale, dim3(grid), dim3(256), 0, h->stream, h->C, h->P, h->U, h->V, h->pose_const, h->tvec_mask, h->point_const,
                     o->jacobi_scaling, h->scale_c, h->scale_p);
  return IntrScale(h, o->jacobi_scaling);
}

struct StepPlan {
  bool fold;
  bool speculate;
  bool direct;
  bool fused_trial_cost;
  bool fused_step;
  bool phase_timings;
};
static StepPlan MakeStepPlan(const pp_ba_impl* h, const pp_ba_options* o) {
  StepPlan p;
  p.fold = h->allreduce == nullptr;
  p.speculate = h->allreduce == nullptr;
  p.direct = p.speculate && !InGroup(h) && h->h_scal_dev != nullptr;
  p.fused_trial_cost = p.fold && (h->NI == 0 || h->sw.ba_fused_step) && h->sw.ba_fused_trial_cost;
  p.fused_step = p.fused_trial_cost && h->sw.ba_fused_step;
  p.phase_timings = o->phase_timings != 0;
  return p;
}

static int EnqueueTrialStep(pp_ba_impl* h, const pp_ba_options* o, const StepPlan& plan, double radius, bool refresh_diagonal, PhaseTimer& timer, unsigned long long* ticket) {
  hipStream_t s = h->stream;
  const int grid_obs = h->num_partials;
// ... 390 lines not shown
```

Baseline: 1207 LM iterations/s.

## Write Jacobians directly into the per-observation record buffer to avoid separate arrays

When the system is dense, non-iterative and has no intrinsics, the eval kernel writes pose and point Jacobian rows straight into the strided JpS record buffer instead of separate Jpose/Jpoint arrays. The prepare kernel then only writes the T block and skips re-copying Jacobians, while the Schur and pair kernels apply the camera scaling on the fly from scale_c. This removes a read-then-rewrite of the Jacobians each iteration and saves memory, at the cost of strided stores in eval, extra scaling multiplies in the Schur kernels, and an unpack kernel when Jacobians are downloaded.

```diff
diff --git a/privacy_preserving_sfm_amd/csrc/ba_covariance.hip b/privacy_preserving_sfm_amd/csrc/ba_covariance.hip
--- a/privacy_preserving_sfm_amd/csrc/ba_covariance.hip
+++ b/privacy_preserving_sfm_amd/csrc/ba_covariance.hip
@@ -102,6 +102,7 @@
   const int32_t *pt_start, *pt_obs, *obs_pose, *obs_cam, *spos, *intr_off, *intr_nv;
   const uint8_t* point_const;
   const double *rec, *JkS , *Vinv, *scale_p, *Zt;
+  const double* rec_scale;
 };
 constexpr int kCovChunk = 64;
 
@@ -144,9 +145,12 @@
           const double* jp = RecJ(a.rec, (size_t)o);
           s_col[tid] = a.spos[6 * a.obs_pose[o]];
 #pragma unroll
-          for (int x = 0; x < 6; ++x)
-#pragma unroll
-            for (int c = 0; c < 3; ++c) s_B[tid][3 * x + c] = jp[x] * t[c] + jp[6 + x] * t[3 + c];
+          for (int x = 0; x < 6; ++x) {
+            const double sx = a.rec_scale ? a.rec_scale[6 * a.obs_pose[o] + x] : 1.0;
+            const double j0 = jp[x] * sx, j1 = jp[6 + x] * sx;
+#pragma unroll
+            for (int c = 0; c < 3; ++c) s_B[tid][3 * x + c] = j0 * t[c] + j1 * t[3 + c];
+          }
           int nv = 0;
           if (a.JkS) {
             const int cam = a.obs_cam[o] >> 4, off = a.intr_off[cam];
@@ -318,6 +322,7 @@
     a.C = h->C; a.n = n; a.N = N;
     a.pt_start = h->pt_start; a.pt_obs = h->pt_obs; a.obs_pose = h->obs_pose; a.obs_cam = h->obs_cam; a.spos = h->spos; a.intr_off = h->intr_off; a.intr_nv = h->intr_nv;
     a.point_const = h->point_const; a.rec = h->JpS; a.JkS = h->NI > 0 ? h->JkS_intr : nullptr; a.Vinv = Vinv2; a.scale_p = scale_p2; a.Zt = Zt;
+    a.rec_scale = h->jac_in_rec ? scale_c2 : nullptr;
     hipLaunchKernelGGL(k_cov_points, dim3(num_points), dim3(256), 0, s, a, (const int32_t*)d_ids, d_point);
   }
   PP_HIP_TRY(hipGetLastError());
diff --git a/privacy_preserving_sfm_amd/csrc/ba_eval.hip b/privacy_preserving_sfm_amd/csrc/ba_eval.hip
--- a/privacy_preserving_sfm_amd/csrc/ba_eval.hip
+++ b/privacy_preserving_sfm_amd/csrc/ba_eval.hip
@@ -17,7 +17,8 @@
   const double *la, *lb, *lc;
   const int32_t *obs_pose, *obs_point, *obs_cam;
   const double *poses, *points, *intr;
-  double *r, *Jpose, *Jpoint, *Jcam;
+  double *r, *Jcam;
+  JacRows jac;
   const int32_t* cam_col;
   int cam_stride;
   double* partials;
@@ -119,23 +120,32 @@
     const int64_t left = a.M - o0;
     const int nobs = left < 256 ? (int)left : 256;
     {
-      const int n2 = nobs * JW / 2;
-      double2* dst = reinterpret_cast<double2*>(a.Jpose + (size_t)JW * o0);
+      constexpr int H = JW / 2;
+      const int n2 = nobs * H;
+      double* dst = a.jac.jp + (size_t)a.jac.jp_stride * o0;
       const double2* src = reinterpret_cast<const double2*>(sJp);
 #pragma unroll
-      for (int it = 0; it < (256 * JW / 2 + 255) / 256; ++it) {
+      for (int it = 0; it < (256 * H + 255) / 256; ++it) {
         const int idx = it * 256 + tid;
-        if (idx < n2) { const double2 v = src[idx]; __builtin_nontemporal_store(v.x, &dst[idx].x); __builtin_nontemporal_store(v.y, &dst[idx].y); }
+        if (idx < n2) {
+          const int row = idx / H;
+          double* d = dst + (size_t)a.jac.jp_stride * row + 2 * (idx - row * H);
+          const double2 v = src[idx]; __builtin_nontemporal_store(v.x, d); __builtin_nontemporal_store(v.y, d + 1);
+        }
       }
     }
     {
       const int n2 = nobs * 3;
-      double2* dst = reinterpret_cast<double2*>(a.Jpoint + (size_t)6 * o0);
+      double* dst = a.jac.jx + (size_t)a.jac.jx_stride * o0;
       const double2* src = reinterpret_cast<const double2*>(sJx);
 #pragma unroll
       for (int it = 0; it < 3; ++it) {
         const int idx = it * 256 + tid;
-        if (idx < n2) { const double2 v = src[idx]; __builtin_nontemporal_store(v.x, &dst[idx].x); __builtin_nontemporal_store(v.y, &dst[idx].y); }
+        if (idx < n2) {
+          const int row = idx / 3;
+          double* d = dst + (size_t)a.jac.jx_stride * row + 2 * (idx - row * 3);
+          const double2 v = src[idx]; __builtin_nontemporal_store(v.x, d); __builtin_nontemporal_store(v.y, d + 1);
+        }
       }
     }
   }
@@ -160,14 +170,16 @@
   a.M = h->M; a.la = h->la; a.lb = h->lb; a.lc = h->lc;
   a.obs_pose = h->obs_pose; a.obs_point = h->obs_point; a.obs_cam = h->obs_cam;
   a.poses = poses; a.points = points; a.intr = intr ? intr : h->intr;
-  a.r = h->r; a.Jpose = h->Jpose; a.Jpoint = h->Jpoint; a.Jcam = h->Jcam; a.cam_col = nullptr; a.cam_stride = kCamStride;
+  a.r = h->r; a.jac = BaJacobianRows(h); a.Jcam = h->Jcam; a.cam_col = nullptr; a.cam_stride = kCamStride;
   a.partials = h->partials; a.loss_type = h->loss_type; a.loss_scale = h->loss_scale;
   return a;
 }
 
 int BaEnsureJacobianBuffers(pp_ba_impl* h, int jac_mode, int want_cam) {
   const int width = jac_mode == 1 ? 14 : 12;
-  if (!h->Jpose || h->jpose_width < width) {
+  const bool arrays = !h->jac_in_rec || jac_mode == 1;
+  if (arrays && !h->Jpoint) { int rc = HandleAlloc(&h->Jpoint, (size_t)6 * h->M); if (rc) return rc; }
+  if (arrays && (!h->Jpose || h->jpose_width < width)) {
     if (h->Jpose) PoolDeviceFree(h->Jpose);
     h->Jpose = nullptr;
     int rc = HandleAlloc(&h->Jpose, (size_t)h->M * width);
@@ -181,9 +193,29 @@
   return PP_OK;
 }
 
+__global__ __launch_bounds__(256) void k_unpack_jacobian(int64_t M, const double* __restrict__ rec, double* __restrict__ Jpose, double* __restrict__ Jpoint) {
+  const int64_t idx = (int64_t)blockIdx.x * 256 + threadIdx.x;
+  if (idx >= 9 * M) return;
+  const int64_t o = idx / 9;
+  const int k = (int)(idx - 9 * o);
+  const double2 v = reinterpret_cast<const double2*>(RecJ(rec, (size_t)o))[k];
+  if (k < 6) reinterpret_cast<double2*>(Jpose + 12 * o)[k] = v;
+  else reinterpret_cast<double2*>(Jpoint + 6 * o)[k - 6] = v;
+}
+
+static int BaUnpackJacobian(pp_ba_impl* h) {
+  if (!h->jac_in_rec) return PP_OK;
+  if (!h->Jpoint) { int rc = HandleAlloc(&h->Jpoint, (size_t)6 * h->M); if (rc) return rc; }
+  if (!h->Jpose) { int rc = HandleAlloc(&h->Jpose, (size_t)12 * h->M); if (rc) return rc; h->jpose_width = 12; }
+  hipLaunchKernelGGL(k_unpack_jacobian, dim3(CeilDiv(9 * h->M, (int64_t)256)), dim3(256), 0, h->stream, h->M, h->JpS, h->Jpose, h->Jpoint);
+  PP_HIP_TRY(hipGetLastError());
+  return PP_OK;
+}
+
 int LaunchEval(pp_ba_impl* h, int jac_mode, int want_cam, bool loss_correct, const double* poses, const double* points,
                double* cost_slot, bool compact_cam) {
   EvalArgs a = MakeArgs(h, poses, points);
+  if (jac_mode != 0) a.jac = JacRows{h->Jpose, h->Jpoint, 14, 6};
   if (want_cam) {
     h->jcam_compact = compact_cam && h->NI > 0;
     if (h->jcam_compact) { a.cam_col = h->intr_col; a.cam_stride = h->jcam_stride; }
@@ -799,7 +831,9 @@
     TRY(HandleAlloc(&h->cnI, (size_t)NI)); TRY(HandleAlloc(&h->JkS_intr, (size_t)M * 2 * kCamStride));
     TRYH(hipMemsetAsync(h->JkS_intr, 0, sizeof(double) * (size_t)M * 2 * kCamStride, s));
   }
-  TRY(HandleAlloc(&h->r, (size_t)2 * M)); TRY(HandleAlloc(&h->Jpoint, (size_t)6 * M));
+  h->jac_in_rec = !iterative && NI == 0 && !h->pairs_chunked;
+  TRY(HandleAlloc(&h->r, (size_t)2 * M));
+  if (h->jac_in_rec) TRY(HandleAlloc(&h->JpS, kRecStride * (size_t)M)); else TRY(HandleAlloc(&h->Jpoint, (size_t)6 * M));
   h->num_partials = CeilDiv(M, 256);
   h->partials_stride = std::max(std::max(h->num_partials, 4096), CeilDiv(4 * (int64_t)P, 256));
   TRY(HandleAlloc(&h->partials, 2 * (size_t)h->partials_stride));
@@ -946,6 +980,7 @@
   if (rc) return rc;
   const int width = jac_mode == 1 ? 14 : 12;
   if (residuals_out) { rc = Download(residuals_out, h->r, (size_t)2 * h->M, h->stream); if (rc) return rc; }
+  if (jac_mode == 0 && (jpose_out || jpoint_out) && (rc = BaUnpackJacobian(h))) return rc;
   if (jpose_out) { rc = Download(jpose_out, h->Jpose, (size_t)width * h->M, h->stream); if (rc) return rc; }
   if (jpoint_out) { rc = Download(jpoint_out, h->Jpoint, (size_t)6 * h->M, h->stream); if (rc) return rc; }
   if (jcam_out) { rc = Download(jcam_out, h->Jcam, (size_t)2 * kCamStride * h->M, h->stream); if (rc) return rc; }
@@ -975,6 +1010,7 @@
   if (rc) return rc;
   rc = Download(h->pin_r, h->r, 2 * M, h->stream); if (rc) return rc;
   if (want_jacobians) {
+    if (jac_mode == 0 && (rc = BaUnpackJacobian(h))) return rc;
     rc = Download(h->pin_jpose, h->Jpose, (size_t)width * M, h->stream); if (rc) return rc;
     rc = Download(h->pin_jpoint, h->Jpoint, 6 * M, h->stream); if (rc) return rc;
     if (cam) { rc = Download(h->pin_jcam, h->Jcam, (size_t)2 * kCamStride * M, h->stream); if (rc) return rc; }
diff --git a/privacy_preserving_sfm_amd/csrc/ba_impl.hpp b/privacy_preserving_sfm_amd/csrc/ba_impl.hpp
--- a/privacy_preserving_sfm_amd/csrc/ba_impl.hpp
+++ b/privacy_preserving_sfm_amd/csrc/ba_impl.hpp
@@ -14,6 +14,7 @@
 __device__ __forceinline__ const double* RecJ(const double* rec, size_t o) { return rec + kRecStride * o + 6; }
 __device__ __forceinline__ const double* RecX(const double* rec, size_t o) { return rec + kRecStride * o + 18; }
 #endif
+struct JacRows { double *jp, *jx; int jp_stride, jx_stride; };
 int SymbolicTileFill(int T, uint8_t* nz);
 int CholeskyChainSteps(int T, const uint8_t* nz, const Switches& sw, int* chains = nullptr);
 int CholeskyPlanSteps(int T, const uint8_t* nz, const Switches& sw, int* chains = nullptr);
@@ -98,6 +99,7 @@
 
   double *r = nullptr, *Jpose = nullptr, *Jpoint = nullptr, *Jcam = nullptr;
   int jpose_width = 0;
+  bool jac_in_rec = false;
   double* partials = nullptr;
   int num_partials = 0, partials_stride = 0, trial_partials = 0;
   double *pin_r = nullptr, *pin_jpose = nullptr, *pin_jpoint = nullptr, *pin_jcam = nullptr;
@@ -150,6 +152,10 @@
 enum Scalar { kCost = 0, kCostCand = 1, kModelChange = 2, kGradMax = 3, kStepNorm2 = 4, kXNorm2 = 5, kTicketSlot = 6 , kNumScalars = 8 };
 
 int BaEnsureJacobianBuffers(pp_ba_impl* h, int jac_mode, int want_cam);
+inline JacRows BaJacobianRows(const pp_ba_impl* h) {
+  if (h->jac_in_rec) return JacRows{h->JpS + 6, h->JpS + 18, kRecStride, kRecStride};
+  return JacRows{h->Jpose, h->Jpoint, 12, 6};
+}
 int LaunchEval(pp_ba_impl* h, int jac_mode, int want_cam, bool loss_correct, const double* poses, const double* points,
                double* cost_slot, bool compact_cam = false);
 int LaunchCostOnly(pp_ba_impl* h, const double* poses, const double* points, const double* intr, double* cost_slot);
diff --git a/privacy_preserving_sfm_amd/csrc/ba_solver.hip b/privacy_preserving_sfm_amd/csrc/ba_solver.hip
--- a/privacy_preserving_sfm_amd/csrc/ba_solver.hip
+++ b/privacy_preserving_sfm_amd/csrc/ba_solver.hip
@@ -20,19 +20,19 @@
   double jx[6];
 };
 
-__device__ __forceinline__ void LoadJp(const double* __restrict__ Jpose, int o, double jp[12]) {
-  const double2* p = reinterpret_cast<const double2*>(Jpose + (size_t)12 * o);
+__device__ __forceinline__ void LoadJp(const JacRows& j, int o, double jp[12]) {
+  const double2* p = reinterpret_cast<const double2*>(j.jp + (size_t)j.jp_stride * o);
 #pragma unroll
   for (int i = 0; i < 6; ++i) { const double2 v = p[i]; jp[2 * i] = v.x; jp[2 * i + 1] = v.y; }
 }
-__device__ __forceinline__ void LoadJx(const double* __restrict__ Jpoint, int o, double jx[6]) {
-  const double2* p = reinterpret_cast<const double2*>(Jpoint + (size_t)6 * o);
+__device__ __forceinline__ void LoadJx(const JacRows& j, int o, double jx[6]) {
+  const double2* p = reinterpret_cast<const double2*>(j.jx + (size_t)j.jx_stride * o);
 #pragma unroll
   for (int i = 0; i < 3; ++i) { const double2 v = p[i]; jx[2 * i] = v.x; jx[2 * i + 1] = v.y; }
 }
 
 __device__ __forceinline__ void PoseReduceBody(int c, const int32_t* __restrict__ pose_start, const int32_t* __restrict__ pose_obs,
-                                               const double* __restrict__ Jpose, const double* __restrict__ r,
+                                               const JacRows& Jpose, const double* __restrict__ r,
                                                double* __restrict__ U, double* __restrict__ gc) {
   __shared__ double red[4][27];
   const int lane = threadIdx.x & 63, wv = threadIdx.x >> 6;
@@ -101,7 +101,7 @@
 }
 
 __device__ __forceinline__ void PointReduceBody(int gid, int P, const int32_t* __restrict__ pt_start, const int32_t* __restrict__ pt_obs,
-                                                const double* __restrict__ Jpoint, const double* __restrict__ r,
+                                                const JacRows& Jpoint, const double* __restrict__ r,
                                                 double* __restrict__ V, double* __restrict__ gp) {
   const int p = gid >> 2, q = gid & 3;
   double v[6] = {0, 0, 0, 0, 0, 0}, g[3] = {0, 0, 0};
@@ -128,11 +128,11 @@
 }
 
 __global__ __launch_bounds__(256) void k_reduce(int C, int P, const int32_t* __restrict__ pose_start, const int32_t* __restrict__ pose_obs,
-                                                const int32_t* __restrict__ pt_start, const int32_t* __restrict__ pt_obs, const double* __restrict__ Jpose,
-                                                const double* __restrict__ Jpoint, const double* __restrict__ r, double* __restrict__ U,
+                                                const int32_t* __restrict__ pt_start, const int32_t* __restrict__ pt_obs, JacRows jac,
+                                                const double* __restrict__ r, double* __restrict__ U,
                                                 double* __restrict__ gc, double* __restrict__ V, double* __restrict__ gp) {
-  if ((int)blockIdx.x < C) PoseReduceBody(blockIdx.x, pose_start, pose_obs, Jpose, r, U, gc);
-  else PointReduceBody(((int)blockIdx.x - C) * 256 + threadIdx.x, P, pt_start, pt_obs, Jpoint, r, V, gp);
+  if ((int)blockIdx.x < C) PoseReduceBody(blockIdx.x, pose_start, pose_obs, jac, r, U, gc);
+  else PointReduceBody(((int)blockIdx.x - C) * 256 + threadIdx.x, P, pt_start, pt_obs, jac, r, V, gp);
 }
 
 __global__ __launch_bounds__(256) void k_jacobi_scale(int C, int P, const double* __restrict__ U, const double* __restrict__ V,
@@ -230,7 +230,8 @@
 struct SchurArgs {
   int C, N, rhs_row;
   const int32_t *pose_start, *pose_obs, *obs_point;
-  const double *Jpose, *Jpoint, *U, *gc, *Vinv, *vb, *scale_c, *scale_p, *diag_c;
+  const double *U, *gc, *Vinv, *vb, *scale_c, *scale_p, *diag_c;
+  const double* rec_scale = nullptr;
   double inv_radius;
   double* S;
   int add_diagonal;
@@ -241,23 +242,29 @@
 
 template <bool kWithDiagonal>
 __device__ __forceinline__ void ObsPrepareBody(int block, int64_t M, const int32_t* __restrict__ obs_pose, const int32_t* __restrict__ obs_point,
-                                               const double* __restrict__ Jpose, const double* __restrict__ Jpoint,
+                                               const JacRows& jac,
                                                const double* __restrict__ V, const double* __restrict__ diag_p, const uint8_t* __restrict__ point_const,
                                                double inv_radius, double dmin, double dmax, const double* __restrict__ scale_c,
                                                const double* __restrict__ scale_p, double* __restrict__ rec) {
   __shared__ __attribute__((aligned(16))) double sR[256 * kRecStride];
   const int tid = threadIdx.x;
   const int64_t o0 = (int64_t)block * 256, o = o0 + tid;
+  const bool home = jac.jx == rec + 18;
+  const int W = home ? 6 : kRecStride;
   if (o < M) {
-    const int c = obs_pose[o], p = obs_point[o];
-    double jp[12], jx[6];
-    LoadJp(Jpose, (int)o, jp);
-    LoadJx(Jpoint, (int)o, jx);
-    double2* jo = reinterpret_cast<double2*>(sR + kRecStride * tid + 6);
-#pragma unroll
-    for (int i = 0; i < 6; ++i) {
-      const int j0 = (2 * i) % 6, j1 = (2 * i + 1) % 6;
-      jo[i] = make_double2(jp[2 * i] * scale_c[6 * c + j0], jp[2 * i + 1] * scale_c[6 * c + j1]);
+    const int p = obs_point[o];
+    double jx[6];
+    LoadJx(jac, (int)o, jx);
+    if (!home) {
+      const int c = obs_pose[o];
+      double jp[12];
+      LoadJp(jac, (int)o, jp);
+      double2* jo = reinterpret_cast<double2*>(sR + kRecStride * tid + 6);
+#pragma unroll
+      for (int i = 0; i < 6; ++i) {
+        const int j0 = (2 * i) % 6, j1 = (2 * i + 1) % 6;
+        jo[i] = make_double2(jp[2 * i] * scale_c[6 * c + j0], jp[2 * i + 1] * scale_c[6 * c + j1]);
+      }
     }
     const double s0 = scale_p[3 * p], s1 = scale_p[3 * p + 1], s2 = scale_p[3 * p + 2];
     double vi[6] = {0.0, 0.0, 0.0, 0.0, 0.0, 0.0};
@@ -277,16 +284,27 @@
       t[3 * r + 1] = jx[3 * r] * v01 + jx[3 * r + 1] * v11 + jx[3 * r + 2] * v12;
       t[3 * r + 2] = jx[3 * r] * v02 + jx[3 * r + 1] * v12 + jx[3 * r + 2] * v22;
     }
-    double2* to = reinterpret_cast<double2*>(sR + kRecStride * tid);
-    double2* xo = reinterpret_cast<double2*>(sR + kRecStride * tid + 18);
+    double2* to = reinterpret_cast<double2*>(sR + W * tid);
     to[0] = make_double2(t[0], t[1]); to[1] = make_double2(t[2], t[3]); to[2] = make_double2(t[4], t[5]);
-    xo[0] = make_double2(jx[0], jx[1]); xo[1] = make_double2(jx[2], jx[3]); xo[2] = make_double2(jx[4], jx[5]);
+    if (!home) {
+      double2* xo = reinterpret_cast<double2*>(sR + kRecStride * tid + 18);
+      xo[0] = make_double2(jx[0], jx[1]); xo[1] = make_double2(jx[2], jx[3]); xo[2] = make_double2(jx[4], jx[5]);
+    }
   }
   __syncthreads();
   const int64_t left = M - o0;
-  const int n2 = (left < 256 ? (int)left : 256) * (kRecStride / 2);
+  const int nobs = left < 256 ? (int)left : 256;
   double2* dr = reinterpret_cast<double2*>(rec + (size_t)kRecStride * o0);
   const double2* sr = reinterpret_cast<const double2*>(sR);
+  if (home) {
+#pragma unroll
+    for (int it = 0; it < 3; ++it) {
+      const int idx = it * 256 + tid;
+      if (idx < 3 * nobs) { const int row = idx / 3; dr[(kRecStride / 2) * row + (idx - 3 * row)] = sr[idx]; }
+    }
+    return;
+  }
+  const int n2 = nobs * (kRecStride / 2);
 #pragma unroll
   for (int it = 0; it < kRecStride / 2; ++it) {
     const int idx = it * 256 + tid;
@@ -299,13 +317,13 @@
                                                  double* __restrict__ diag_p, const uint8_t* __restrict__ point_const, double inv_radius, double* __restrict__ Vinv,
                                                  double* __restrict__ vb, int32_t* __restrict__ flag, int C, const double* __restrict__ U,
                                                  const double* __restrict__ scale_c, double dmin, double dmax, double* __restrict__ diag_c, int64_t M,
-                                                 const int32_t* __restrict__ obs_pose, const int32_t* __restrict__ obs_point, const double* __restrict__ Jpose,
-                                                 const double* __restrict__ Jpoint, double* __restrict__ rec, int obs_blocks, double* __restrict__ zS, int zN,
+                                                 const int32_t* __restrict__ obs_pose, const int32_t* __restrict__ obs_point, JacRows jac,
+                                                 double* __restrict__ rec, int obs_blocks, double* __restrict__ zS, int zN,
                                                  const int32_t* __restrict__ ztiles) {
   if ((int)blockIdx.x < point_blocks)
     PointPrepareBody<kWithDiagonal>(blockIdx.x, P, V, gp, scale_p, diag_p, point_const, inv_radius, Vinv, vb, flag, C, U, scale_c, dmin, dmax, diag_c);
   else if ((int)blockIdx.x < point_blocks + obs_blocks)
-    ObsPrepareBody<kWithDiagonal>((int)blockIdx.x - point_blocks, M, obs_pose, obs_point, Jpose, Jpoint, V, diag_p, point_const, inv_radius, dmin, dmax, scale_c, scale_p, rec);
+    ObsPrepareBody<kWithDiagonal>((int)blockIdx.x - point_blocks, M, obs_pose, obs_point, jac, V, diag_p, point_const, inv_radius, dmin, dmax, scale_c, scale_p, rec);
   else {
     const int zt = (int)blockIdx.x - point_blocks - obs_blocks;
     const int ti = ztiles[2 * zt], tj = ztiles[2 * zt + 1];
@@ -324,11 +342,13 @@
       else if (a.add_diagonal) a.S[(size_t)j * a.N + j] = kBig;
     }
   }
-  double u[21], acc[6];
+  double u[21], acc[6], sc[6];
 #pragma unroll
   for (int i = 0; i < 21; ++i) u[i] = 0.0;
 #pragma unroll
   for (int i = 0; i < 6; ++i) acc[i] = 0.0;
+#pragma unroll
+  for (int i = 0; i < 6; ++i) sc[i] = a.rec_scale ? a.rec_scale[6 * c + i] : 1.0;
   for (int e = a.pose_start[c] + (int)threadIdx.x; e < a.pose_start[c + 1]; e += 256) {
     const int o = a.pose_obs[e];
     const int p = a.obs_point[o];
@@ -341,6 +361,8 @@
       for (int i = 0; i < 6; ++i) { const double2 v = p[3 + i]; jp[2 * i] = v.x; jp[2 * i + 1] = v.y; }
 #pragma unroll
       for (int i = 0; i < 3; ++i) { const double2 v = p[9 + i]; q[6 + 2 * i] = v.x; q[6 + 2 * i + 1] = v.y; }
+#pragma unroll
+      for (int i = 0; i < 6; ++i) { jp[i] *= sc[i]; jp[6 + i] *= sc[i]; }
     }
     const double g00 = q[0] * q[6] + q[1] * q[7] + q[2] * q[8], g01 = q[0] * q[9] + q[1] * q[10] + q[2] * q[11];
     const double g10 = q[3] * q[6] + q[4] * q[7] + q[5] * q[8], g11 = q[3] * q[9] + q[4] * q[10] + q[5] * q[11];
@@ -409,6 +431,10 @@
   if (slot >= 10 || pr >= num_pairs) return;
   const int bi = pair_ij[2 * pr], bj = pair_ij[2 * pr + 1];
   const int e0 = pair_start[2 * pr], e1 = pair_start[2 * pr + 1];
+  const double si = a.rec_scale ? a.rec_scale[6 * bi + ar] : 1.0;
+  double sj[6];
+#pragma unroll
+  for (int i = 0; i < 6; ++i) sj[i] = a.rec_scale ? a.rec_scale[6 * bj + i] : 1.0;
   double acc[6] = {0, 0, 0, 0, 0, 0};
   int2 next = e0 < e1 ? *reinterpret_cast<const int2*>(pair_entries + 2 * (size_t)e0) : make_int2(0, 0);
   for (int e = e0; e < e1; ++e) {
@@ -419,11 +445,13 @@
     const double2* pj = reinterpret_cast<const double2*>(RecJ(rec, (size_t)oo.y));
     const double2 t0 = qi[0], t1 = qi[1], t2 = qi[2];
     const double2 x0 = qj[0], x1 = qj[1], x2 = qj[2];
-    const double pi0 = RecJ(rec, (size_t)oo.x)[ar], pi1 = RecJ(rec, (size_t)oo.x)[6 + ar];
+    const double pi0 = RecJ(rec, (size_t)oo.x)[ar] * si, pi1 = RecJ(rec, (size_t)oo.x)[6 + ar] * si;
     const double g00 = t0.x * x0.x + t0.y * x0.y + t1.x * x1.x, g01 = t0.x * x1.y + t0.y * x2.x + t1.x * x2.y;
     const double g10 = t1.y * x0.x + t2.x * x0.y + t2.y * x1.x, g11 = t1.y * x1.y + t2.x * x2.x + t2.y * x2.y;
     const double h0 = pi0 * g00 + pi1 * g10, h1 = pi0 * g01 + pi1 * g11;
-    const double2 j0 = pj[0], j1 = pj[1], j2 = pj[2], j3 = pj[3], j4 = pj[4], j5 = pj[5];
+    double2 j0 = pj[0], j1 = pj[1], j2 = pj[2], j3 = pj[3], j4 = pj[4], j5 = pj[5];
+    j0.x *= sj[0]; j0.y *= sj[1]; j1.x *= sj[2]; j1.y *= sj[3]; j2.x *= sj[4]; j2.y *= sj[5];
+    j3.x *= sj[0]; j3.y *= sj[1]; j4.x *= sj[2]; j4.y *= sj[3]; j5.x *= sj[4]; j5.y *= sj[5];
     acc[0] += h0 * j0.x + h1 * j3.x; acc[1] += h0 * j0.y + h1 * j3.y;
     acc[2] += h0 * j1.x + h1 * j4.x; acc[3] += h0 * j1.y + h1 * j4.y;
     acc[4] += h0 * j2.x + h1 * j5.x; acc[5] += h0 * j2.y + h1 * j5.y;
@@ -649,7 +677,8 @@
   int C, P;
   int64_t M;
   const int32_t *pt_start, *pt_obs, *obs_pose, *obs_point;
-  const double *Jpose, *Jpoint, *r, *Vinv, *vb, *scale_c, *scale_p, *step_c;
+  JacRows jac;
+  const double *r, *Vinv, *vb, *scale_c, *scale_p, *step_c;
   double* step_p;
   double* partials;
   const double* JkS;
@@ -680,8 +709,8 @@
       const int o = a.pt_obs[e];
       const int c = a.obs_pose[o];
       double jp[12], jx[6];
-      LoadJp(a.Jpose, o, jp);
-      LoadJx(a.Jpoint, o, jx);
+      LoadJp(a.jac, o, jp);
+      LoadJx(a.jac, o, jx);
       double m0 = 0.0, m1 = 0.0;
 #pragma unroll
       for (int j = 0; j < 6; ++j) { const double d = a.scale_c[6 * c + j] * a.step_c[6 * c + j]; m0 += jp[j] * d; m1 += jp[6 + j] * d; }
@@ -737,8 +766,8 @@
   if (o < a.M) {
     const int c = a.obs_pose[o], p = a.obs_point[o];
     double jp[12], jx[6];
-    LoadJp(a.Jpose, (int)o, jp);
-    LoadJx(a.Jpoint, (int)o, jx);
+    LoadJp(a.jac, (int)o, jp);
+    LoadJx(a.jac, (int)o, jx);
     double dc[6], dp[3];
 #pragma unroll
     for (int j = 0; j < 6; ++j) dc[j] = ScaledStep(a.scale_c[6 * c + j], a.step_c[6 * c + j]);
@@ -844,8 +873,8 @@
   Row R[2];
   auto load = [&](int o, Row& w) {
     w.o = o; w.c = a.obs_pose[o];
-    LoadJp(a.Jpose, o, w.jp);
-    LoadJx(a.Jpoint, o, w.jx);
+    LoadJp(a.jac, o, w.jp);
+    LoadJx(a.jac, o, w.jx);
     w.u0 = 0.0; w.u1 = 0.0;
 #pragma unroll
     for (int j = 0; j < 6; ++j) { w.dc[j] = ScaledStep(a.scale_c[6 * w.c + j], a.step_c[6 * w.c + j]); w.u0 += w.jp[j] * w.dc[j]; w.u1 += w.jp[6 + j] * w.dc[j]; }
@@ -1090,7 +1119,8 @@
   A(U, 36 * (size_t)C); A(gc, (size_t)h->n_red); A(V, 6 * (size_t)P); A(gp, 3 * (size_t)P); A(Vinv, 6 * (size_t)P); A(vb, 3 * (size_t)P);
   A(scale_c, (size_t)h->n_red); A(scale_p, 3 * (size_t)P); A(diag_c, (size_t)h->n_red); A(diag_p, 3 * (size_t)P);
   if (!h->iterative) { A(S, (size_t)h->N * h->N); A(Linv, CholeskyWorkspaceDoubles(h->N)); }
-  A(JpS, kRecStride * (size_t)h->M); A(norm_part, 3 * 256); A(step_c, (size_t)h->N); A(step_p, 3 * (size_t)P);
+  if (!h->JpS) { A(JpS, kRecStride * (size_t)h->M); }
+  A(norm_part, 3 * 256); A(step_c, (size_t)h->N); A(step_p, 3 * (size_t)P);
   if (!h->spos_identity) { A(step_s, (size_t)h->N); }
 #undef A
   for (int i = 0; i < 8; ++i) if ((rc = PoolEventAcquire(&h->tev[i], true))) return rc;
@@ -1118,8 +1148,8 @@
   SchurArgs a;
   a.C = h->C; a.N = h->N; a.rhs_row = h->n_red;
   a.pose_start = h->pose_start; a.pose_obs = h->pose_obs; a.obs_point = h->obs_point;
-  a.Jpose = h->Jpose; a.Jpoint = h->Jpoint; a.U = h->U; a.gc = h->gc; a.Vinv = h->Vinv; a.vb = h->vb;
-  a.scale_c = h->scale_c; a.scale_p = h->scale_p; a.diag_c = h->diag_c;
+  a.U = h->U; a.gc = h->gc; a.Vinv = h->Vinv; a.vb = h->vb;
+  a.scale_c = h->scale_c; a.scale_p = h->scale_p; a.diag_c = h->diag_c; a.rec_scale = h->jac_in_rec ? h->scale_c : nullptr;
   a.inv_radius = 1.0 / radius; a.S = h->S; a.add_diagonal = h->group_rank == 0 ? 1 : 0;
   a.spos = h->spos;
   return a;
@@ -1128,7 +1158,7 @@
   StepArgs a;
   a.C = h->C; a.P = h->P; a.M = h->M;
   a.pt_start = h->pt_start; a.pt_obs = h->pt_obs; a.obs_pose = h->obs_pose; a.obs_point = h->obs_point;
-  a.Jpose = h->Jpose; a.Jpoint = h->Jpoint; a.r = h->r; a.Vinv = h->Vinv; a.vb = h->vb;
+  a.jac = BaJacobianRows(h); a.r = h->r; a.Vinv = h->Vinv; a.vb = h->vb;
   a.scale_c = h->scale_c; a.scale_p = h->scale_p; a.step_c = h->step_c; a.step_p = h->step_p; a.partials = h->partials + h->partials_stride;
   a.JkS = h->NI > 0 ? h->JkS_intr : nullptr; a.obs_cam = h->obs_cam; a.intr_off = h->intr_off; a.intr_nv = h->intr_nv;
   return a;
@@ -1179,8 +1209,8 @@
   hipStream_t s = h->stream;
   int rc = LaunchEval(h, 0, h->NI > 0 ? 1 : 0, true, h->poses, h->points, fold_cost ? nullptr : h->scal + kCost, true);
   if (rc) return rc;
-  hipLaunchKernelGGL(k_reduce, dim3(h->C + CeilDiv(4 * (int64_t)h->P, 256)), dim3(256), 0, s, h->C, h->P, h->pose_start, h->pose_obs, h->pt_start, h->pt_obs, h->Jpose,
-                     h->Jpoint, h->r, h->U, h->gc, h->V, h->gp);
+  hipLaunchKernelGGL(k_reduce, dim3(h->C + CeilDiv(4 * (int64_t)h->P, 256)), dim3(256), 0, s, h->C, h->P, h->pose_start, h->pose_obs, h->pt_start, h->pt_obs, BaJacobianRows(h),
+                     h->r, h->U, h->gc, h->V, h->gp);
   PP_HIP_TRY(hipGetLastError());
   if ((rc = IntrSumsAfterEval(h))) return rc;
   if (InGroup(h)) {
@@ -1247,7 +1277,7 @@
     const int point_blocks = CeilDiv(refresh_diagonal ? std::max(h->P, 6 * h->C) : h->P, 256);
     const dim3 grid(point_blocks + h->num_partials + zero_tiles);
     hipLaunchKernelGGL(refresh_diagonal ? k_prepare<true> : k_prepare<false>, grid, dim3(256), 0, s, point_blocks, h->P, h->V, h->gp, h->scale_p, h->diag_p, h->point_const,
-                       1.0 / radius, h->Vinv, h->vb, h->d_flag, h->C, h->U, h->scale_c, dmin, dmax, h->diag_c, h->M, h->obs_pose, h->obs_point, h->Jpose, h->Jpoint, h->JpS,
+                       1.0 / radius, h->Vinv, h->vb, h->d_flag, h->C, h->U, h->scale_c, dmin, dmax, h->diag_c, h->M, h->obs_pose, h->obs_point, BaJacobianRows(h), h->JpS,
                        h->num_partials, h->S, h->N, (const int32_t*)h->nz_tile_list);
   }
   SchurArgs a = MakeSchurArgs(h, radius);
```

Measured after the change: 1200 LM iterations/s. Within noise of the previous version (-0.5%).
